# collabora/WhisperLive

Measured on AMD Instinct MI355X. Metric: real-time factor (xRT), Whisper-small 30 s window (p50 chunk latency in p50_chunk_latency_ms), higher is better.
Workload: dtype f16 (MFMA operands; f32 accumulate, f32 residual stream, f32 log-mel); 1 GPU; configs[1]: Whisper-small.en, 1 stream per GPU, one 30 s window per stream per step (480000 samples 16 kHz f32 resident in HBM -> log-mel -> encoder -> beam-5 decode, 64 generated tokens forced by suppressing EOT), seeded random weights; streams_per_gpu=1, beam_size=5, decode_steps=64

## Files before the change

### whisperlive_amd/csrc/decoder.h

```cpp
#pragma once
#include "kernels.h"

namespace wlx {

#define WLX_MAX_MT 4
#define WLX_MAX_DEC_ROWS 320
#define WLX_XSPLIT 8
#define WLX_MAX_CAND 32
#define WLX_MAX_HYP 32

struct RowTables {
    const int* token; const int* pos; const int* cache; const int* ancrow;
    const short* anc;
    int* intok;
};

void launch_dec_embed(const half_t* tok_emb, const float* pos_emb, int d, const RowTables& rt, int rows,
                      float* x, const int* done, hipStream_t s);

enum GemvIn : int { GEMV_IN_LN = 0, GEMV_IN_F16 = 1, GEMV_IN_XATTN = 2 };
enum GemvOut : int { GEMV_OUT_F16 = 0, GEMV_OUT_GELU_F16 = 1, GEMV_OUT_F32 = 2, GEMV_OUT_RESID = 3, GEMV_OUT_QKV = 4,
                     GEMV_OUT_SLAB = 5 };
enum GemvXsrc : int { GEMV_X_PLAIN = 0, GEMV_X_SLABS = 1, GEMV_X_EMBED = 2 };
#ifndef WLX_CQ_GB_LDS
#define WLX_CQ_GB_LDS 1
#endif
#ifndef WLX_CQ_SWAP
#define WLX_CQ_SWAP 1
#endif
#ifndef WLX_STAGE_WAVE
#define WLX_STAGE_WAVE 1
#endif
#ifndef WLX_XCOMB_WAVE
#define WLX_XCOMB_WAVE 1
#endif
#ifndef WLX_FC2_KS
#define WLX_FC2_KS 2
#endif

struct GemvParams {
    int in_mode, out_mode;
    int M;
    int Mtot;
    int chunk;
    int busy_device;
    int rt_nz, rt_tiles, rt_magic;
    int K, KT, N;
    int KTW;
    int NCH;
    int nwm;
    int xstage;
    const half_t* Wp; const float* bias;
    const float* X; long ldx; const float* gamma; const float* beta;
    const half_t* Xh; long ldxh;
    const half_t* part_o; const float* part_ml; int H; int R;
    half_t* Yh; long ldyh;
    float* Y; long ldy;
    float* Xres; long ldxres;
    int d; float qscale; half_t* Kc; half_t* Vc; long cache_row_stride;
    const int* row_cache; const int* row_pos;
    const int* done;
    int xsrc;
    float* slab; long slab_stride;
    int KTS;
    const half_t* tok_emb; const float* pos_emb; const int* emb_token; int* intok;
    WLX_TR_FIELD
};
#ifdef WLX_TRACE
extern unsigned long long* g_trace_buf;
extern int g_trace_seq;
extern const char* g_trace_names[512];
static inline WlxTrace trace_next(const char* name) {
    WlxTrace t{g_trace_buf, g_trace_seq};
    if (g_trace_seq < 512) g_trace_names[g_trace_seq] = name;
    ++g_trace_seq;
    return t;
}
#define WLX_TR_ARG(name) , trace_next(name)
#else
#define WLX_TR_ARG(name)
#endif
void launch_dec_gemv(const GemvParams& p, hipStream_t s);
const char* dec_gemv_kernel_name(const GemvParams& p);
extern bool g_decode_v1;
bool dec_gemv_is_lean(const GemvParams& p);
int dec_gemv_slab_split(int M, int K, int N);

void launch_dec_self_attn(const half_t* q, long ldq, const half_t* Kc, const half_t* Vc, long cache_row_stride,
                          int d, int H, const RowTables& rt, int rows, half_t* out, long ldo,
                          const int* done, bool ident_ancestry, hipStream_t s);
void launch_dec_cross_attn(const half_t* q, long ldq, const half_t* Kp, const half_t* Vp, long item_stride, int H, int R,
                           int groups, int rows, const int* group_item, half_t* part_o, float* part_ml, hipStream_t s);

bool dec_cq_cross_attn_eligible(int d, int H, int R);
void launch_dec_cq_cross_attn(const float* X, long ldx, const float* gamma, const float* beta, const half_t* Wp, const float* bias,
                              float qscale, int d, const half_t* Kp, const half_t* Vp, long item_stride, int H, int R, int groups,
                              int rows, const int* group_item, half_t* part_o, float* part_ml, hipStream_t s);
void launch_dec_xattn_combine(const half_t* part_o, const float* part_ml, int M, int H, int R, half_t* out, long ldo, hipStream_t s);
void launch_dec_align_scores(const half_t* q, long ldq, const half_t* Kp_item, int h, int rows, float* out, hipStream_t s);

struct SearchState {
    int* step;
    int* done;
    int* done_host;
    int* n_finished;
    int* item_done;
    int* plen;
    float* cum;
    int* row_done;
    float* cand_score; int* cand_tok;
    int* samp_tok; float* samp_lp;
    int* hyp_tokens;
    int* hyp_len;
    float* hyp_score;
    int* n_hyp;
    int* n_hyp_host;
    float* no_speech;
    int* nsp_row;
    int* token; int* pos; short* anc; int* intok;
    float* scan_stats;
    float* scan_cv; int* scan_ci;
    int* rule;
};
#define SC_THREADS 256
#define SC_NPT 8
#define SC_CHUNK (SC_THREADS * SC_NPT)
#define SC_MAXCH 27
#define SC_NSTAT 8
struct SearchParams {
    int V; long ldl;
    int items, R, rows;
    int sampling;
    int beam, ncand, max_cand_hyp , num_hyp;
    int allow_early_exit;
    float length_penalty, rep_penalty, temperature;
    int no_repeat_ngram, topk;
    int suppress_blank, apply_ts_rules, max_initial_ts;
    int sot, eot, no_timestamps, ts_begin, no_speech, blank;
    int max_length;
    unsigned long long seed;
    const unsigned* suppress_mask;
};
void launch_search_rows(const float* logits, const SearchParams* sp_dev, int rows, const SearchState& st, hipStream_t s);
void launch_search_update(const SearchParams* sp_dev, int items, const SearchState& st, hipStream_t s);
void launch_search_scan3(const float* logits, long ldl, int V, const SearchParams* sp_dev, int rows, const SearchState& st,
                         hipStream_t s);
void launch_search_merge_update3(const float* logits, long ldl, int V, const SearchParams* sp_dev, int items, int R,
                                 const SearchState& st, hipStream_t s);
void launch_search_reset(const SearchState& st, int items, int rows, hipStream_t s);
void launch_token_prob_rows(const float* logits, long ldl, int vlim, int rows, const int* toks, float* out, hipStream_t s);
void launch_token_prob(const float* logits, long ldl, int V, int rows, int tok, float* out, hipStream_t s);
void launch_lang_probs(const float* logits, long ldl, int rows, const int* ids, int n, float* probs, hipStream_t s);

}
```

### whisperlive_amd/csrc/decoder.hip

```cpp
#include "decoder.h"
#include <algorithm>
#include <cstdlib>
#include <cstdio>
#include <atomic>

namespace wlx {

__global__ __launch_bounds__(256) void dec_embed_kernel(const half_t* __restrict__ tok_emb,
                                                        const float* __restrict__ pos_emb, int d,
                                                        const int* __restrict__ token,
                                                        const int* __restrict__ pos,
                                                        const int* __restrict__ cache, int* __restrict__ intok,
                                                        float* __restrict__ x, const int* __restrict__ done WLX_TR_PARAM) {
    if (done && *done) return;
    WLX_TR_BEGIN();
    const int r = blockIdx.x;
    const int tok = token[r], p = pos[r];
    if (threadIdx.x == 0) intok[(long)cache[r] * WLX_T_TEXT + p] = tok;
    const half_t* te = tok_emb + (long)tok * d;
    const float* pe = pos_emb + (long)p * d;
    for (int i = threadIdx.x * 4; i < d; i += 256 * 4) {
        f16x4 t = ld_f16x4(te + i);
        float4 pv = *reinterpret_cast<const float4*>(pe + i);
        *reinterpret_cast<float4*>(x + (long)r * d + i) =
            make_float4((float)t[0] + pv.x, (float)t[1] + pv.y, (float)t[2] + pv.z, (float)t[3] + pv.w);
    }
    WLX_TR_END(trc);
}

void launch_dec_embed(const half_t* tok_emb, const float* pos_emb, int d, const RowTables& rt, int rows,
                      float* x, const int* done, hipStream_t s) {
    hipLaunchKernelGGL(dec_embed_kernel, dim3(rows), dim3(256), 0, s, tok_emb, pos_emb, d, rt.token, rt.pos,
                       rt.cache, rt.intok, x, done WLX_TR_ARG("embed"));
}

#define GV_CH 6

template <int MT, int NTB, int IN>
__global__ __launch_bounds__(512) void dec_gemv_kernel(GemvParams p) {
    if (p.done && *p.done) return;
    extern __shared__ __attribute__((aligned(16))) float smem[];
    const int tid = threadIdx.x, wave = tid >> 6, lane = tid & 63, c = lane & 15, g = lane >> 4;
    const int nw = blockDim.x >> 6;
    const int KT = p.KT;
    const int KTW = (KT + nw - 1) / nw;
    const int kt0 = wave * KTW;
    const int kt1 = (kt0 + KTW < KT) ? kt0 + KTW : KT;
    const int NT_total = (p.N + 15) >> 4;

    const half_t* wbase[NTB];
#pragma unroll
    for (int i = 0; i < NTB; ++i) {
        int nt = blockIdx.x * NTB + i;
// ... 337 lines not shown
            int u = lane + 64 * q;
            if (u >= total) u = (q == 0) ? total - 1 : (lane + 64 * (q - 1) < total ? lane + 64 * (q - 1) : total - 1);
            m_[q] = u / kv8; k_[q] = u - m_[q] * kv8;
            v_[q] = ld_f16x8(X + (long)m_[q] * ldx + k_[q] * 8);
        }
        after_first_loads();
#pragma unroll
        for (int q = 0; q < P; ++q) *reinterpret_cast<f16x8*>(xs + m_[q] * ldxs + k_[q] * 8) = v_[q];
    }
#pragma unroll 1
    for (int u0 = lane + 64 * P; u0 < total; u0 += 128) {
        const int u1 = u0 + 64;
        const int m0 = u0 / kv8, k0 = u0 - m0 * kv8;
        const int uc = (u1 < total) ? u1 : u0;
        const int m1 = uc / kv8, k1 = uc - m1 * kv8;
        const f16x8 v0 = ld_f16x8(X + (long)m0 * ldx + k0 * 8);
        const f16x8 v1 = ld_f16x8(X + (long)m1 * ldx + k1 * 8);
        *reinterpret_cast<f16x8*>(xs + m0 * ldxs + k0 * 8) = v0;
        *reinterpret_cast<f16x8*>(xs + m1 * ldxs + k1 * 8) = v1;
    }
}


template <int CH, int LNV, int IN, int OUT, int NTB, int MT, int XS>
__global__ __launch_bounds__((IN == GEMV_IN_LN || OUT == GEMV_OUT_SLAB || MT > 1 || CH > 6 || (IN == GEMV_IN_XATTN && WLX_XCOMB_WAVE != 0)) ? 512 : 1024) void dec_gemv2_kernel(GemvParams p_in) {
    GemvParams p = p_in;
    int tile = blockIdx.x;
    if (p_in.Mtot > 0) {
        int zc = (int)blockIdx.z;
        if (p_in.rt_nz > 0) {
            const int lin = (int)blockIdx.x, t = lin >> 3;
            const int tq = (int)(((unsigned)t * (unsigned)p_in.rt_magic) >> 16);
            zc = t - tq * p_in.rt_nz;
            tile = tq * 8 + (lin & 7);
            if (tile >= p_in.rt_tiles) return;
        }
        const int CHK = p_in.chunk;
        const int r0 = zc * CHK;
        p.M = (p_in.Mtot - r0 < CHK) ? p_in.Mtot - r0 : CHK;
        if (p.emb_token) p.emb_token += r0;
        if (p.X) p.X += (long)r0 * p.ldx;
        if (p.Xh) p.Xh += (long)r0 * p.ldxh;
        if (p.Yh) p.Yh += (long)r0 * p.ldyh;
        if (p.Y) p.Y += (long)r0 * p.ldy;
        if (p.Xres) p.Xres += (long)r0 * p.ldxres;
        if (p.slab) p.slab += (long)r0 * ((IN == GEMV_IN_LN) ? p.ldx : p.ldxres);
        if (p.row_cache) p.row_cache += r0;
        if (p.row_pos) p.row_pos += r0;
    }
    static_assert(XS == GEMV_X_PLAIN || IN == GEMV_IN_LN || (IN == GEMV_IN_F16 && OUT == GEMV_OUT_RESID && NTB == 1),
                  "slab / embedding sources: LayerNorm prologue or residual epilogue only");
    static_assert(OUT != GEMV_OUT_SLAB || (IN == GEMV_IN_F16 && NTB == 1), "K-split form: fp16 rows in");
    extern __shared__ __attribute__((aligned(16))) float smem[];
    const int tid = threadIdx.x, lane = tid & 63, c = lane & 15, g = lane >> 4;
    const int wave = __builtin_amdgcn_readfirstlane(tid >> 6);
    const int nw = p.nwm;
    WLX_TR_BEGIN();
    constexpr int NP = NTB * MT;
    constexpr bool LNT = (LNV == 15);
    constexpr int NV = LNT ? 2 : LNV;
    const bool tail_on = !LNT || lane < 32;
    const int tback = LNT ? (tail_on ? 0 : lane) : 0;
    (void)tail_on; (void)tback;
    float* accred = smem;
    half_t* xs = reinterpret_cast<half_t*>(smem + nw * NP * 256);

    const bool streams = (IN != GEMV_IN_XATTN) || wave < nw;
    const int kx0 = (streams ? wave : 0) * p.KTW;
    const int ks0 = (OUT == GEMV_OUT_SLAB) ? (int)blockIdx.y * p.KTS : 0;
    const int kw0 = ks0 + kx0;
    const half_t* wp = p.Wp + ((long)(tile * NTB) * p.KT + kw0) * 512 + lane * 8;
    const long wstep = (long)p.KT * 512;
    f16x8 wf[CH][NTB];
    auto load_weights = [&]() {
        asm volatile("" ::: "memory");
        const half_t* wq = streams ? wp : p.Wp + ((long)(tile * NTB) * p.KT + ks0) * 512 + lane * 8;
        const long js = streams ? 512 : 0, is = streams ? wstep : 0;
#pragma unroll
        for (int j = 0; j < CH; ++j)
#pragma unroll
            for (int i = 0; i < NTB; ++i) wf[j][i] = ld_nt_f16x8(wq + i * is + j * js);
    };
#ifndef WLX_X_FIRST
#define WLX_X_FIRST 1
#endif
    if (!WLX_X_FIRST) load_weights();

    int crow[MT];
#pragma unroll
    for (int mt = 0; mt < MT; ++mt) crow[mt] = (mt * 16 + c < p.M) ? mt * 16 + c : p.M - 1;
    const int pair0 = (wave < NP) ? wave : 0;
    const int nt_e = tile * NTB + pair0 / MT;
    const int n_e = nt_e * 16 + g * 4;
    int row_e = (pair0 % MT) * 16 + c;
    if (row_e >= p.M) row_e = p.M - 1;
    float4 bias_e = make_float4(0.f, 0.f, 0.f, 0.f), res_e = bias_e;
    int rc_e = 0, rp_e = 0;
    if constexpr (OUT != GEMV_OUT_F32) bias_e = *reinterpret_cast<const float4*>(p.bias + n_e);
    if constexpr (OUT == GEMV_OUT_RESID) res_e = *reinterpret_cast<const float4*>(p.Xres + (long)row_e * p.ldxres + n_e);
    if constexpr (OUT == GEMV_OUT_QKV) { rc_e = p.row_cache[row_e]; rp_e = p.row_pos[row_e]; }
    float4 slab_e[(OUT == GEMV_OUT_RESID && XS == GEMV_X_SLABS) ? WLX_FC2_KS : 1];
    if constexpr (OUT == GEMV_OUT_RESID && XS == GEMV_X_SLABS) {
#pragma unroll
        for (int sl = 0; sl < WLX_FC2_KS; ++sl)
            slab_e[sl] = *reinterpret_cast<const float4*>(p.slab + sl * p.slab_stride + (long)row_e * p.ldxres + n_e);
    }
    if constexpr (OUT == GEMV_OUT_SLAB) { if (blockIdx.y != 0) bias_e = make_float4(0.f, 0.f, 0.f, 0.f); }

    f32x4 acc[NTB][MT];
#pragma unroll
    for (int i = 0; i < NTB; ++i)
#pragma unroll
        for (int mt = 0; mt < MT; ++mt) acc[i][mt] = (f32x4){0.f, 0.f, 0.f, 0.f};
    f16x8 xf[CH][MT];

    if constexpr (IN == GEMV_IN_F16) {
        const half_t* xr[MT];
        int xstep;
        if (MT == 1 && p.xstage) {
            const int Ks = (OUT == GEMV_OUT_SLAB) ? p.KTS * 32 : p.K;
            const int ldxs = Ks + 8;
            if constexpr (WLX_STAGE_WAVE != 0) {
                stage_rows_f16_wave<(CH * 4 * 5 + 63) / 64>(p.Xh + (ks0 + kx0) * 32, p.ldxh, p.M, p.KTW * 32, xs + kx0 * 32, ldxs, lane, [&]() { if (WLX_X_FIRST) load_weights(); });
                WLX_TR_MARK(1);
                __builtin_amdgcn_fence(__ATOMIC_RELEASE, "wavefront");
                __builtin_amdgcn_wave_barrier();
                __builtin_amdgcn_fence(__ATOMIC_ACQUIRE, "wavefront");
            } else {
            stage_rows_f16(p.Xh + ks0 * 32, p.ldxh, p.M, Ks, xs, ldxs, [&]() { if (WLX_X_FIRST) load_weights(); });
            WLX_TR_MARK(1);
            __syncthreads();
            }
            xr[0] = xs + crow[0] * ldxs + kx0 * 32 + g * 8;
            xstep = 32;
        } else {
#pragma unroll
            for (int mt = 0; mt < MT; ++mt) xr[mt] = p.Xh + (long)crow[mt] * p.ldxh + kw0 * 32 + g * 8;
            xstep = 32;
        }
#pragma unroll
        for (int j = 0; j < CH; ++j)
#pragma unroll
            for (int mt = 0; mt < MT; ++mt) xf[j][mt] = *reinterpret_cast<const f16x8*>(xr[mt] + j * xstep);
        if (WLX_X_FIRST && !(MT == 1 && p.xstage)) load_weights();
#pragma unroll 1
        for (int ch = 1; ch < p.NCH; ++ch) {
            f16x8 wn[CH][NTB], xn[CH][MT];
#pragma unroll
            for (int j = 0; j < CH; ++j) {
#pragma unroll
                for (int i = 0; i < NTB; ++i) wn[j][i] = ld_nt_f16x8(wp + i * wstep + (ch * CH + j) * 512);
#pragma unroll
                for (int mt = 0; mt < MT; ++mt) xn[j][mt] = *reinterpret_cast<const f16x8*>(xr[mt] + (ch * CH + j) * xstep);
            }
#pragma unroll
            for (int j = 0; j < CH; ++j) {
#pragma unroll
                for (int i = 0; i < NTB; ++i) {
#pragma unroll
                    for (int mt = 0; mt < MT; ++mt) acc[i][mt] = mfma16(wf[j][i], xf[j][mt], acc[i][mt]);
                    wf[j][i] = wn[j][i];
                }
#pragma unroll
                for (int mt = 0; mt < MT; ++mt) xf[j][mt] = xn[j][mt];
            }
        }
    } else if constexpr (IN == GEMV_IN_LN && XS != GEMV_X_PLAIN) {
        const int nwl = nw;
        constexpr int NSL = (XS == GEMV_X_SLABS) ? WLX_FC2_KS : 1;
        float4 x[NV], sl[NSL][NV];
        f16x4 te[NV];
        int tok0 = 0, pos0 = 0;
        auto request_row = [&](int r, float4 (&x)[NV], float4 (&sl)[NSL][NV], f16x4 (&te)[NV], int& tok, int& pos) {
            if constexpr (XS == GEMV_X_EMBED) {
                tok = p.emb_token[r];
                pos = p.row_pos[r] | (p.row_cache[r] << 16);
                const half_t* tp = p.tok_emb + (long)tok * p.K + lane * 4;
                const float4* pp = reinterpret_cast<const float4*>(p.pos_emb + (long)(pos & 0xffff) * p.K) + lane;
#pragma unroll
                for (int j = 0; j < NV; ++j) { const int tb = (j == NV - 1) ? tback : 0; te[j] = ld_f16x4(tp + 256 * j - 4 * tb); x[j] = pp[64 * j - tb]; }
            } else {
                const float4* x4 = reinterpret_cast<const float4*>(p.X + (long)r * p.ldx) + lane;
#pragma unroll
                for (int j = 0; j < NV; ++j) x[j] = x4[64 * j - ((j == NV - 1) ? tback : 0)];
                if constexpr (XS == GEMV_X_SLABS) {
#pragma unroll
                    for (int q = 0; q < NSL; ++q) {
                        const float4* s4 = reinterpret_cast<const float4*>(p.slab + q * p.slab_stride + (long)r * p.ldx) + lane;
#pragma unroll
                        for (int j = 0; j < NV; ++j) sl[q][j] = s4[64 * j - ((j == NV - 1) ? tback : 0)];
                    }
                }
            }
        };
        auto combine_row = [&](int r, bool keep, float4 (&x)[NV], const float4 (&sl)[NSL][NV], const f16x4 (&te)[NV], int tok, int pos) {
            if constexpr (XS == GEMV_X_SLABS) {
#pragma unroll
                for (int q = 0; q < NSL; ++q)
#pragma unroll
                    for (int j = 0; j < NV; ++j) { x[j].x += sl[q][j].x; x[j].y += sl[q][j].y; x[j].z += sl[q][j].z; x[j].w += sl[q][j].w; }
            }
            if constexpr (XS == GEMV_X_EMBED) {
#pragma unroll
                for (int j = 0; j < NV; ++j) { x[j].x += (float)te[j][0]; x[j].y += (float)te[j][1]; x[j].z += (float)te[j][2]; x[j].w += (float)te[j][3]; }
                if (tile == 0 && keep) {
                    float4* o4 = reinterpret_cast<float4*>(p.Xres + (long)r * p.ldxres) + lane;
#pragma unroll
                    for (int j = 0; j < NV; ++j) if (j < NV - 1 || tail_on) o4[64 * j] = x[j];
                    if (lane == 0) p.intok[(long)(pos >> 16) * WLX_T_TEXT + (pos & 0xffff)] = tok;
                }
            }
        };
        const int ra = (wave < p.M) ? wave : p.M - 1;
        request_row(ra, x, sl, te, tok0, pos0);
        constexpr bool PF2 = MT == 1 && ((CH == 6 && LNV == 3) || (CH == 8 && LNV == 4) || (CH == 10 && LNV == 5));
        float4 xb[NV], slb[NSL][NV];
        f16x4 teb[NV];
        int tokb = 0, posb = 0;
        const int rb = (wave + nwl < p.M) ? wave + nwl : p.M - 1;
        if constexpr (PF2) request_row(rb, xb, slb, teb, tokb, posb);
        const float4* g4 = reinterpret_cast<const float4*>(p.gamma) + lane;
        const float4* b4 = reinterpret_cast<const float4*>(p.beta) + lane;
        float4 gq[NV], bq[NV];
#pragma unroll
        for (int j = 0; j < NV; ++j) { const int tb = (j == NV - 1) ? tback : 0; gq[j] = g4[64 * j - tb]; bq[j] = b4[64 * j - tb]; }
        if (WLX_X_FIRST) load_weights();
        const int ldxs = p.K + 8;
        constexpr float invK = LNT ? (1.0f / 384.0f) : 1.0f / (256.0f * NV);
        auto ln_row = [&](float4 (&x)[NV], int r, bool keep) {
            if constexpr (LNT) { if (!tail_on) x[NV - 1] = make_float4(0.f, 0.f, 0.f, 0.f); }
            float sm = 0.f;
#pragma unroll
            for (int j = 0; j < NV; ++j) sm += (x[j].x + x[j].y) + (x[j].z + x[j].w);
            const float mean = wave_sum_dpp(sm) * invK;
            float q = 0.f;
#pragma unroll
            for (int j = 0; j < NV; ++j) {
                x[j].x -= mean; x[j].y -= mean; x[j].z -= mean; x[j].w -= mean;
                if constexpr (LNT) { if (j == NV - 1 && !tail_on) x[j] = make_float4(0.f, 0.f, 0.f, 0.f); }
                q += (x[j].x * x[j].x + x[j].y * x[j].y) + (x[j].z * x[j].z + x[j].w * x[j].w);
            }
            const float rstd = rsqrtf(wave_sum_dpp(q) * invK + 1e-5f);
            half_t* dst = xs + (long)r * ldxs + lane * 4;
#pragma unroll
            for (int j = 0; j < NV; ++j) {
                const f16x4 hv = {(half_t)(x[j].x * rstd * gq[j].x + bq[j].x), (half_t)(x[j].y * rstd * gq[j].y + bq[j].y),
                                  (half_t)(x[j].z * rstd * gq[j].z + bq[j].z), (half_t)(x[j].w * rstd * gq[j].w + bq[j].w)};
                if (keep && (j < NV - 1 || tail_on)) *reinterpret_cast<f16x4*>(dst + 256 * j) = hv;
            }
        };
        combine_row(ra, wave < p.M, x, sl, te, tok0, pos0);
        ln_row(x, ra, wave < p.M);
        if constexpr (PF2) {
            combine_row(rb, wave + nwl < p.M, xb, slb, teb, tokb, posb);
            ln_row(xb, rb, wave + nwl < p.M);
        }
        if constexpr (MT == 1) {
#pragma unroll 1
            for (int r = wave + (PF2 ? 2 : 1) * nwl; r < p.M; r += nwl) {
                float4 x2[NV], sl2[NSL][NV];
                f16x4 te2[NV];
                int tok2 = 0, pos2 = 0;
                request_row(r, x2, sl2, te2, tok2, pos2);
                combine_row(r, true, x2, sl2, te2, tok2, pos2);
                ln_row(x2, r, true);
            }
        } else {
#pragma unroll 1
            for (int r = wave + nwl; r < p.M; r += 2 * nwl) {
                const int r1 = r + nwl;
                const bool has1 = r1 < p.M;
                float4 x2[NV], sl2[NSL][NV], x3[NV], sl3[NSL][NV];
                f16x4 te2[NV], te3[NV];
                int tok2 = 0, pos2 = 0, tok3 = 0, pos3 = 0;
                request_row(r, x2, sl2, te2, tok2, pos2);
                request_row(has1 ? r1 : r, x3, sl3, te3, tok3, pos3);
                combine_row(r, true, x2, sl2, te2, tok2, pos2);
                ln_row(x2, r, true);
                combine_row(has1 ? r1 : r, has1, x3, sl3, te3, tok3, pos3);
// ... 379 lines not shown
    const size_t xs_bytes = (size_t)p.M * (KTf * 32 + 8) * sizeof(half_t);
    if (c.NTB == 2 && p.out_mode == GEMV_OUT_GELU_F16 && c.shm + xs_bytes > WLX_G2_LDS_MAX) {
        c.NTB = 1;
        c.shm = sizeof(float) * (size_t)c.nw * c.NTB * c.MT * 256;
    }
    c.xstage = true;
    const size_t xstage_max = (p.Mtot > 0 && p.rt_nz > 0) ? (size_t)WLX_G2_LDS_MAX : (size_t)64 * 1024;
    if (p.in_mode == GEMV_IN_F16 && (c.MT > 1 || c.shm + xs_bytes > xstage_max)) c.xstage = false;
    if (c.xstage) c.shm += xs_bytes;
    if (c.shm > WLX_G2_LDS_MAX) return false;
    if (c.shm > 64 * 1024 && g_lds_optin_refused.load(std::memory_order_relaxed)) return false;
    return true;
}
static Gemv2Cfg gemv2_cfg(const GemvParams& p) {
    Gemv2Cfg c{};
    if (g_decode_v1 || p.M > 48 || p.M < 1) return c;
    if (p.bias ? (p.N & 15) != 0 : p.out_mode != GEMV_OUT_F32) return c;
    const bool combo = (p.in_mode == GEMV_IN_LN && (p.out_mode == GEMV_OUT_QKV || p.out_mode == GEMV_OUT_F16 ||
                                                    p.out_mode == GEMV_OUT_GELU_F16 || p.out_mode == GEMV_OUT_F32)) ||
                       (p.in_mode != GEMV_IN_LN && p.out_mode == GEMV_OUT_RESID) ||
                       (p.in_mode == GEMV_IN_F16 && p.out_mode == GEMV_OUT_SLAB);
    if (!combo || p.K != p.KT * 32) return c;
    if (p.xsrc != GEMV_X_PLAIN) {
        const bool ln_ok = p.in_mode == GEMV_IN_LN && p.out_mode == GEMV_OUT_QKV;
        const bool res_ok = p.in_mode == GEMV_IN_F16 && p.out_mode == GEMV_OUT_RESID && p.xsrc == GEMV_X_SLABS;
        if (!(ln_ok || res_ok)) return c;
    }
    int KTf = p.KT;
    if (p.out_mode == GEMV_OUT_SLAB) {
        if (p.KTS < 1 || p.KT % p.KTS || p.KT / p.KTS != WLX_FC2_KS) return c;
        KTf = p.KTS;
    }
    if (!gemv2_cfg_waves(p, KTf, c)) return c;
    c.NTB = gemv2_cfg_tiles(p);
    c.ok = gemv2_cfg_staging(p, KTf, c);
    return c;
}

template <int CH_, int LNV_, int IN_, int OUT_, int NTB_, int MT_, int XS_>
struct G2Args { static constexpr int CH = CH_, LNV = LNV_, IN = IN_, OUT = OUT_, NTB = NTB_, MT = MT_, XS = XS_; };
enum G2Rows { G2_LN_XS, G2_LN_PLAIN, G2_NO_LN };
template <int CH, int LNV, int OUT, int MT, int NTBMAX, class Leaf>
static bool gemv2_dispatch_ntb(const Gemv2Cfg& c, Leaf& leaf) {
    if (c.NTB == 1) return leaf(G2Args<CH, LNV, GEMV_IN_LN, OUT, 1, MT, GEMV_X_PLAIN>{});
    if constexpr (NTBMAX >= 2) { if (c.NTB == 2) return leaf(G2Args<CH, LNV, GEMV_IN_LN, OUT, 2, MT, GEMV_X_PLAIN>{}); }
    if constexpr (NTBMAX >= 4 && MT == 1) { if (c.NTB == 4) return leaf(G2Args<CH, LNV, GEMV_IN_LN, OUT, 4, 1, GEMV_X_PLAIN>{}); }
    return false;
}
template <int ROWS, int CH, int LNV, int MT, class Leaf>
static bool gemv2_dispatch_modes(const GemvParams& p, const Gemv2Cfg& c, Leaf& leaf) {
    if constexpr (ROWS == G2_LN_XS) {
        if (p.out_mode != GEMV_OUT_QKV || c.NTB != 1) return false;
        if (p.xsrc == GEMV_X_SLABS) return leaf(G2Args<CH, LNV, GEMV_IN_LN, GEMV_OUT_QKV, 1, MT, GEMV_X_SLABS>{});
        return p.xsrc == GEMV_X_EMBED && leaf(G2Args<CH, LNV, GEMV_IN_LN, GEMV_OUT_QKV, 1, MT, GEMV_X_EMBED>{});
    } else if constexpr (ROWS == G2_LN_PLAIN) {
        switch (p.out_mode) {
            case GEMV_OUT_QKV: return gemv2_dispatch_ntb<CH, LNV, GEMV_OUT_QKV, MT, 4>(c, leaf);
            case GEMV_OUT_F16: return gemv2_dispatch_ntb<CH, LNV, GEMV_OUT_F16, MT, 1>(c, leaf);
            case GEMV_OUT_GELU_F16: return gemv2_dispatch_ntb<CH, LNV, GEMV_OUT_GELU_F16, MT, 4>(c, leaf);
            case GEMV_OUT_F32: return gemv2_dispatch_ntb<CH, LNV, GEMV_OUT_F32, MT, 2>(c, leaf);
            default: return false;
        }
    } else {
        if (p.in_mode == GEMV_IN_XATTN) {
            if constexpr (CH <= 6) { if (p.out_mode == GEMV_OUT_RESID && p.xsrc == GEMV_X_PLAIN && c.NTB == 1) return leaf(G2Args<CH, 1, GEMV_IN_XATTN, GEMV_OUT_RESID, 1, MT, GEMV_X_PLAIN>{}); }
            return false;
        }
        if (p.in_mode != GEMV_IN_F16) return false;
        if (p.out_mode == GEMV_OUT_SLAB) return p.xsrc == GEMV_X_PLAIN && c.NTB == 1 && leaf(G2Args<CH, 1, GEMV_IN_F16, GEMV_OUT_SLAB, 1, MT, GEMV_X_PLAIN>{});
        if (p.out_mode != GEMV_OUT_RESID) return false;
        if (p.xsrc == GEMV_X_SLABS) return c.NTB == 1 && leaf(G2Args<CH, 1, GEMV_IN_F16, GEMV_OUT_RESID, 1, MT, GEMV_X_SLABS>{});
        if (p.xsrc != GEMV_X_PLAIN) return false;
        if (c.NTB == 1) return leaf(G2Args<CH, 1, GEMV_IN_F16, GEMV_OUT_RESID, 1, MT, GEMV_X_PLAIN>{});
        if constexpr (MT == 1) { if (c.NTB == 2) return leaf(G2Args<CH, 1, GEMV_IN_F16, GEMV_OUT_RESID, 2, 1, GEMV_X_PLAIN>{}); }
        return false;
    }
}
template <int ROWS, int CH, int LNV, int MTMAX, class Leaf>
static bool gemv2_dispatch_pair(const GemvParams& p, const Gemv2Cfg& c, Leaf& leaf) {
    if (c.CH != CH || c.LNV != LNV) return false;
    if (c.MT == 1) return gemv2_dispatch_modes<ROWS, CH, LNV, 1>(p, c, leaf);
    if constexpr (MTMAX == 3) return c.MT == 2 ? gemv2_dispatch_modes<ROWS, CH, LNV, 2>(p, c, leaf) : c.MT == 3 && gemv2_dispatch_modes<ROWS, CH, LNV, 3>(p, c, leaf);
    return false;
}
template <class Leaf>
static bool gemv2_dispatch(const GemvParams& p, const Gemv2Cfg& c, Leaf leaf) {
    if (p.in_mode == GEMV_IN_LN && p.xsrc != GEMV_X_PLAIN)
        return gemv2_dispatch_pair<G2_LN_XS, 4, 3, 3>(p, c, leaf) || gemv2_dispatch_pair<G2_LN_XS, 3, 3, 3>(p, c, leaf) || gemv2_dispatch_pair<G2_LN_XS, 2, 2, 3>(p, c, leaf) ||
               gemv2_dispatch_pair<G2_LN_XS, 4, 4, 3>(p, c, leaf) || gemv2_dispatch_pair<G2_LN_XS, 5, 5, 3>(p, c, leaf) || gemv2_dispatch_pair<G2_LN_XS, 2, 15, 1>(p, c, leaf) ||
               gemv2_dispatch_pair<G2_LN_XS, 6, 3, 1>(p, c, leaf) || gemv2_dispatch_pair<G2_LN_XS, 8, 4, 1>(p, c, leaf) || gemv2_dispatch_pair<G2_LN_XS, 10, 5, 1>(p, c, leaf);
    if (p.in_mode == GEMV_IN_LN)
        return gemv2_dispatch_pair<G2_LN_PLAIN, 6, 3, 3>(p, c, leaf) || gemv2_dispatch_pair<G2_LN_PLAIN, 5, 5, 3>(p, c, leaf) || gemv2_dispatch_pair<G2_LN_PLAIN, 4, 2, 3>(p, c, leaf) ||
               gemv2_dispatch_pair<G2_LN_PLAIN, 4, 4, 3>(p, c, leaf) || gemv2_dispatch_pair<G2_LN_PLAIN, 10, 5, 1>(p, c, leaf) || gemv2_dispatch_pair<G2_LN_PLAIN, 8, 4, 1>(p, c, leaf) ||
               gemv2_dispatch_pair<G2_LN_PLAIN, 2, 15, 1>(p, c, leaf);
    return gemv2_dispatch_pair<G2_NO_LN, 12, 1, 1>(p, c, leaf) || gemv2_dispatch_pair<G2_NO_LN, 10, 1, 1>(p, c, leaf) || gemv2_dispatch_pair<G2_NO_LN, 8, 1, 1>(p, c, leaf) ||
           gemv2_dispatch_pair<G2_NO_LN, 6, 1, 3>(p, c, leaf) || gemv2_dispatch_pair<G2_NO_LN, 5, 1, 3>(p, c, leaf) || gemv2_dispatch_pair<G2_NO_LN, 4, 1, 3>(p, c, leaf);
}
template __global__ void dec_gemv2_kernel<12, 1, GEMV_IN_XATTN, GEMV_OUT_RESID, 1, 1, GEMV_X_PLAIN>(GemvParams);
template __global__ void dec_gemv2_kernel<10, 1, GEMV_IN_XATTN, GEMV_OUT_RESID, 1, 1, GEMV_X_PLAIN>(GemvParams);
template __global__ void dec_gemv2_kernel<8, 1, GEMV_IN_XATTN, GEMV_OUT_RESID, 1, 1, GEMV_X_PLAIN>(GemvParams);

static bool gemv2_ok(const GemvParams& p, Gemv2Cfg* out) {
    const Gemv2Cfg c = gemv2_cfg(p);
    if (!c.ok || !gemv2_dispatch(p, c, [](auto) { return true; })) return false;
    if (out) *out = c;
    return true;
}
static void gemv2_launch(const GemvParams& p0, const Gemv2Cfg& c, hipStream_t s) {
    GemvParams p = p0;
    p.KTW = c.CH * c.NCH; p.NCH = c.NCH; p.xstage = c.xstage ? 1 : 0; p.nwm = c.nw;
#ifdef WLX_TRACE
    { static thread_local char nm[512][48]; const int q = g_trace_seq < 512 ? g_trace_seq : 511;
      snprintf(nm[q], 48, "gemv2<%d,%d,%d> N%d K%d", p.in_mode, p.out_mode, p.xsrc, p.N, p.K); p.trc = trace_next(nm[q]); }
#endif
    const int NT_total = (p.N + 15) / 16;
    if (p.Mtot > 0 && p.chunk <= 0) p.chunk = 48;
    dim3 grid((NT_total + c.NTB - 1) / c.NTB, p.out_mode == GEMV_OUT_SLAB ? p.KT / p.KTS : 1, p.Mtot > 0 ? (p.Mtot + p.chunk - 1) / p.chunk : 1), block(c.nw * 64);
    if (p.Mtot > 0 && p.rt_nz > 0) {
        p.rt_tiles = (int)grid.x;
        p.rt_magic = 65536 / p.rt_nz + 1;
        grid.x = ((grid.x + 7) / 8) * 8 * p.rt_nz;
        grid.z = 1;
    }
    if (p.in_mode == GEMV_IN_XATTN && !(WLX_XCOMB_WAVE != 0 && c.MT == 1)) {
        const int want = (p.M * p.H * 8 + 63) / 64;
        block.x = 64 * std::max(c.nw, std::min(c.MT > 1 ? 8 : 16, want));
    }
    const bool launched = gemv2_dispatch(p, c, [&](auto a) { using A = decltype(a); g2_launch<A::CH, A::LNV, A::IN, A::OUT, A::NTB, A::MT, A::XS>(grid, block, c.shm, s, p); return true; });
    if (!launched) dispatch_bug("dec_gemv2_kernel", s);
}
static GemvParams gemv_chunked(const GemvParams& p) {
    static const bool rt_on = [] { const char* e = wlx_ab("WLX_ROWTILE"); return !(e && e[0] == '0'); }();
    constexpr int rt_max = WLX_MAX_DEC_ROWS;
    static const int rt_chunk_env = [] { const char* e = wlx_ab("WLX_ROWTILE_CHUNK"); const int v = e ? atoi(e) : 0; return (v == 16 || v == 32 || v == 48) ? v : 0; }();
    int rt_chunk = 16;
    if (p.in_mode == GEMV_IN_F16 && p.out_mode == GEMV_OUT_RESID && p.xsrc == GEMV_X_PLAIN && !p.busy_device && p.M > 64) {
        static const int n_cu = [] { int dev = 0, n = 256; (void)hipGetDevice(&dev); hipDeviceProp_t pr; if (hipGetDeviceProperties(&pr, dev) == hipSuccess && pr.multiProcessorCount > 0) n = pr.multiProcessorCount; return n; }();
        const int tiles = (p.N + 15) / 16;
        double best = 1e300;
        for (int mt = 1; mt <= 3; ++mt) {
            const long wgs = (long)tiles * ((p.M + 16 * mt - 1) / (16 * mt));
            const double cost = (double)((wgs + n_cu - 1) / n_cu) * (1.0 + 0.35 * (mt - 1));
            if (cost < best - 1e-9) { best = cost; rt_chunk = 16 * mt; }
        }
    }
    if (rt_chunk_env) rt_chunk = rt_chunk_env;
    GemvParams q = p;
    if (p.Mtot != 0 || p.in_mode == GEMV_IN_XATTN) return q;
    const bool ln_wide4 = rt_chunk == 16 && p.M > 32 && p.in_mode == GEMV_IN_LN && p.xsrc == GEMV_X_PLAIN && (p.out_mode == GEMV_OUT_QKV || p.out_mode == GEMV_OUT_GELU_F16) &&
                          (p.N & 15) == 0 && ((p.N >> 4) & 3) == 0;
    const bool rt_shape = p.N <= 1536 || (long)p.N * p.K <= 3200000L || ln_wide4;
    if (rt_on && !g_decode_v1 && p.M > rt_chunk && p.M <= rt_max && rt_shape) { q.Mtot = p.M; q.M = rt_chunk; q.chunk = rt_chunk; q.rt_nz = (p.M + rt_chunk - 1) / rt_chunk; }
    else if (p.M > 48 && p.xsrc != GEMV_X_EMBED) { q.Mtot = p.M; q.M = 48; q.chunk = 48; }
    return q;
}

int dec_gemv_slab_split(int M, int K, int N) {
    if (WLX_FC2_KS < 2) return 0;
    if (g_decode_v1 || M < 1 || K % 32 || (K / 32) % WLX_FC2_KS || K < 2048) return 0;
    GemvParams p0{};
    p0.in_mode = GEMV_IN_F16; p0.out_mode = GEMV_OUT_SLAB; p0.M = M; p0.K = K; p0.KT = K / 32; p0.N = N; p0.KTS = p0.KT / WLX_FC2_KS;
    static const float dummy_bias = 0.f;
    p0.bias = &dummy_bias;
    const GemvParams p = gemv_chunked(p0);
    Gemv2Cfg c;
    if (!gemv2_ok(p, &c) || (p.M <= 16 && !c.xstage)) return 0;
    return WLX_FC2_KS;
}

struct VocabParams {
    const float* X; long ldx; const float* gamma; const float* beta;
    const half_t* Wp; int M, N, NT;
    float* Y; long ldy;
    const float* slab; long slab_stride;
    WLX_TR_FIELD
};
template <int KT, int KC, int MT, bool SLABS>
__global__ __launch_bounds__(512) void dec_vocab_kernel(VocabParams p) {
    static_assert(!SLABS || MT == 1, "slab rows: decode steps of one row tile");
    constexpr int K = KT * 32, LNV = (K + 255) / 256, NC = KT / KC, LDXS = K + 8;
    constexpr bool LNT = (K % 256) != 0;
    static_assert((K % 256 == 0 || K == 384) && KT % KC == 0 && NC % 2 == 0, "d_model a multiple of 256 (or 384); an even number of K chunks");
    constexpr int RPT = (MT == 1) ? 2 : 4;
    constexpr int NTRIP = (MT * 16 + 8 * RPT - 1) / (8 * RPT);
    extern __shared__ __attribute__((aligned(16))) half_t vxs[];
    const int tid = threadIdx.x, lane = tid & 63, c = lane & 15, g = lane >> 4;
    const int wave = __builtin_amdgcn_readfirstlane(tid >> 6);
    WLX_TR_BEGIN();
    const int pair = blockIdx.x * 8 + wave;
    const int t0 = (2 * pair < p.NT) ? 2 * pair : p.NT - 1, t1 = (2 * pair + 1 < p.NT) ? 2 * pair + 1 : p.NT - 1;
    const bool tail_on = !LNT || lane < 32;
    const int tback = LNT ? (tail_on ? 0 : lane) : 0;
    float4 x[RPT][LNV];
#pragma unroll
    for (int i = 0; i < RPT; ++i) {
        const int r = (wave + 8 * i < p.M) ? wave + 8 * i : p.M - 1;
        const float4* x4 = reinterpret_cast<const float4*>(p.X + (long)r * p.ldx) + lane;
#pragma unroll
        for (int j = 0; j < LNV; ++j) x[i][j] = x4[64 * j - ((j == LNV - 1) ? tback : 0)];
    }
    float4 xsl[SLABS ? WLX_FC2_KS : 1][RPT][LNV];
    if constexpr (SLABS) {
#pragma unroll
        for (int q = 0; q < WLX_FC2_KS; ++q)
#pragma unroll
            for (int i = 0; i < RPT; ++i) {
// ... 772 lines not shown
```

### whisperlive_amd/csrc/engine.h

```cpp
#pragma once
#include <hip/hip_runtime.h>
#include <map>
#include <mutex>
#include <string>
#include <vector>
#include "../../include/wlx.h"
#include "decoder.h"
#include "host.h"

namespace wlx {

struct StepGraphKey {
    int rows, R, groups;
    bool operator<(const StepGraphKey& o) const {
        if (rows != o.rows) return rows < o.rows;
        if (R != o.R) return R < o.R;
        return groups < o.groups;
    }
};

struct ProfRec { std::string name; double bytes; };
struct Prof { std::vector<ProfRec> recs; bool list_only = true; std::string only; int t = 0; };

struct Slot {
    std::mutex call_mu;
    int B = 0, R = 0, rows_cap = 0, cache_rows = 0, groups_cap = 0;
    hipStream_t stream = nullptr;
    bool dedicated_queue = false;
    int device_of = -1;
    bool counted = false;
    unsigned promote_epoch = 0;
    hipEvent_t ev0 = nullptr, ev1 = nullptr;
    hipEvent_t ev_lm0 = nullptr, ev_lm1 = nullptr;
    hipEvent_t ev_en0 = nullptr, ev_en1 = nullptr;
    bool en_pending = false;
    bool lm_pending = false;
    bool gen_pending = false;
    std::vector<int> lm_items;
    bool busy_variant = false;
    std::vector<void*> allocs, host_allocs;
    float* pcm = nullptr; size_t pcm_cap = 0;
    float* feats = nullptr; long feat_ld = 0;
    std::vector<int> nframes;
    std::vector<int64_t> npcm;
    unsigned* gmax = nullptr;
    ResampleStage rs{};
    bool rs_ready = false;
    long long* d_rng = nullptr;
    half_t *featT = nullptr, *h1 = nullptr, *ln = nullptr, *q = nullptr, *k = nullptr, *vt = nullptr,
           *attn = nullptr, *h2 = nullptr, *enc16 = nullptr;
    float *x = nullptr, *enc32 = nullptr;
    long featT_stride = 0, h1_stride = 0;
    half_t *ck = nullptr, *cvt = nullptr;
    int enc_batch = 0;
    half_t *kc = nullptr, *vc = nullptr;
    float* xd = nullptr; half_t *qd = nullptr, *attnd = nullptr, *hd = nullptr;
    float* slab = nullptr;
    half_t* part_o = nullptr;
    float *part_ml = nullptr, *logits = nullptr;
    long ldl = 0;
    int *d_token = nullptr, *d_pos = nullptr, *d_cache = nullptr, *d_ancrow = nullptr, *d_group_item = nullptr;
    struct DecBufs {
        float* xd; half_t *qd, *attnd, *hd; float* slab; int slab_rows; half_t* part_o; float* part_ml;
        int *d_token, *d_pos, *d_cache, *d_ancrow, *d_group_item;
    };
    DecBufs pf{};
    bool pf_one_pass = false;
    bool pf_ok = false;
    short* d_anc = nullptr; int* d_intok = nullptr;
    bool anc_ident = false;
    SearchState st{};
    SearchParams* d_sp = nullptr;
    unsigned* d_suppress = nullptr;
    int* d_lang_ids = nullptr; float* d_probs = nullptr; float* d_tokprob = nullptr;
    int* h_stage = nullptr; size_t h_stage_ints = 0;
    unsigned char* h_gen = nullptr; size_t h_gen_bytes = 0;
    int* h_pf = nullptr; bool h_pf_used = false;
    int* h_hyp = nullptr;
    int max_items = 0;
    std::vector<int> last_suppress; bool suppress_valid = false;
    std::map<StepGraphKey, hipGraphExec_t> graphs;
    wlx_timings tm{};
    Prof* prof = nullptr;
    struct AlignCapture { float* scores; const int32_t* heads; int n_heads, n_tok, row0, item; }* align = nullptr;
    float* align_scores = nullptr; size_t align_cap = 0;
    int* d_align_tgt = nullptr; float* d_align_prob = nullptr;
};

struct Ring {
    std::mutex mu;
    int device = 0;
    float* buf = nullptr; size_t cap = 0;
    int64_t base = 0, resident = 0;
    hipStream_t stream = nullptr;
    hipEvent_t last_read = nullptr; bool read_pending = false; hipStream_t last_read_stream = nullptr;
};

struct Engine {
    wlx_spec spec{};
    int device = 0;
    int H = 0;
    std::vector<void*> allocs;
    LogmelConsts lm{};
    half_t *conv1_w = nullptr, *conv2_w = nullptr;
    float *conv1_b = nullptr, *conv2_b = nullptr, *enc_pos = nullptr, *enc_ln_g = nullptr, *enc_ln_b = nullptr;
    int conv1_KT = 0;
    std::vector<LayerW> enc;
    half_t* Wckv = nullptr; float* bckv = nullptr;
    half_t *tok_emb16 = nullptr, *Wvocab = nullptr;
    float *dec_pos = nullptr, *dec_ln_g = nullptr, *dec_ln_b = nullptr;
    std::vector<LayerW> dec;
    std::mutex mu;
    std::vector<Slot*> slots;
    bool use_graph = true;
};

}

struct wlx_engine : public wlx::Engine {};
struct wlx_ring : public wlx::Ring {};
```

### whisperlive_amd/csrc/engine.hip

```cpp
#include "engine.h"
#include <sched.h>
#include <atomic>
#include <limits>
#include <algorithm>
#include <cmath>
#include <cstdio>
#include <cstdlib>
#include <cstring>
#include <chrono>
#include <thread>

using namespace wlx;

static inline void cpu_relax() {
#if defined(__x86_64__) || defined(__i386__)
    __builtin_ia32_pause();
#elif defined(__aarch64__)
    asm volatile("yield" ::: "memory");
#else
    asm volatile("" ::: "memory");
#endif
}
extern "C" int32_t wlx_abi_version(void) { return WLX_ABI_VERSION; }

// ... 74 lines not shown
    CKR(conv("model.encoder.conv2.weight", d, &e->conv2_w, &KT));
    CKR(ws.alloc_vec(A, "model.encoder.conv1.bias", d, &e->conv1_b, true));
    CKR(ws.alloc_vec(A, "model.encoder.conv2.bias", d, &e->conv2_b, true));
    CKR(positions("model.encoder.embed_positions.weight", sp.n_audio_ctx, &e->enc_pos));
    LayerOpts o{false, 1.f, true};
    e->enc.resize(sp.enc_layers);
    for (int l = 0; l < sp.enc_layers; ++l)
        CKR(load_layer(ws, A, "model.encoder.layers." + std::to_string(l) + ".", d, F, o, e->enc[l]));
    CKR(ws.alloc_vec(A, "model.encoder.layer_norm.weight", d, &e->enc_ln_g, true));
    CKR(ws.alloc_vec(A, "model.encoder.layer_norm.bias", d, &e->enc_ln_b, true));
    CKR(ws.need("model.decoder.embed_tokens.weight", {V, d}, &t));
    CKR(dalloc(A, &e->tok_emb16, (size_t)V * d, true));
    CKR(ws.device_f32(t, &src));
    launch_f32_to_f16(src, e->tok_emb16, (long)V * d, ws.st);
    CKR(alloc_packed(A, V, d, &e->Wvocab, &KT, true));
    launch_pack_linear(src, V, d, d, e->Wvocab, KT, 0, ws.st);
    CKR(positions("model.decoder.embed_positions.weight", sp.n_text_ctx, &e->dec_pos));
    CKR(alloc_packed(A, (int64_t)sp.dec_layers * 2 * d, d, &e->Wckv, nullptr, true));
    CKR(dalloc(A, &e->bckv, (size_t)sp.dec_layers * 2 * d, true));
    o.Wckv = e->Wckv; o.bckv = e->bckv;
    e->dec.resize(sp.dec_layers);
    for (o.l = 0; o.l < sp.dec_layers; ++o.l)
        CKR(load_layer(ws, A, "model.decoder.layers." + std::to_string(o.l) + ".", d, F, o, e->dec[o.l]));
    CKR(ws.alloc_vec(A, "model.decoder.layer_norm.weight", d, &e->dec_ln_g, true));
    CKR(ws.alloc_vec(A, "model.decoder.layer_norm.bias", d, &e->dec_ln_b, true));
    return ws.finish();
}

static std::atomic<bool> g_embedded_device_memory{false};
extern "C" int32_t wlx_engine_create(const wlx_spec* spec, const wlx_tensor* weights, int32_t n_weights,
                                     int32_t device, wlx_engine** out) {
    if (!spec || !weights || !out) return set_error(WLX_ERR_ARG, "null argument");
    if (spec->d_model % 64 || spec->d_model / 64 != spec->n_heads)
        return set_error(WLX_ERR_ARG, "d_model must be 64*n_heads");
    if (spec->d_model % 128 || spec->d_model > 1536) return set_error(WLX_ERR_ARG, "d_model must be a multiple of 128, <= 1536");
    if (spec->ffn % 128) return set_error(WLX_ERR_ARG, "ffn must be a multiple of 128");
    if (spec->n_mels != 80 && spec->n_mels != 128) return set_error(WLX_ERR_ARG, "n_mels must be 80 or 128");
    if (spec->n_audio_ctx != WLX_T_AUDIO || spec->n_text_ctx != WLX_T_TEXT)
        return set_error(WLX_ERR_ARG, "n_audio_ctx/n_text_ctx must be 1500/448");
    if (spec->vocab > 1024 * 52) return set_error(WLX_ERR_ARG, "vocab too large");
    int ndev = 0;
    CK(hipGetDeviceCount(&ndev));
    if (device < 0 || device >= ndev) return set_error(WLX_ERR_ARG, "device %d out of range (%d)", device, ndev);
    CK(hipSetDevice(device));
    if (int pe = gemm_prepare_device()) return set_error(WLX_ERR_HIP, "GEMM kernel set-up failed on device %d (hip error %d)", device, pe);
    wlx_engine* e = new wlx_engine();
    e->spec = *spec;
    e->device = device;
    e->H = spec->n_heads;
    for (int i = 0; i < n_weights; ++i)
        if (weights[i].on_device) { g_embedded_device_memory.store(true); break; }
    const char* ng = getenv("WLX_NO_GRAPH");
    e->use_graph = !(ng && ng[0] == '1');
    const char* v1 = wlx_ab("WLX_DECODE_V1");
    g_decode_v1 = (v1 && v1[0] == '1');
    int rc = engine_load(e, weights, n_weights);
    if (rc != WLX_OK) {
        for (void* p : e->allocs) (void)hipFree(p);
        delete e;
        return rc;
    }
    *out = e;
    return WLX_OK;
}

static int max_dedicated_queues() {
    static const int v = [] { const char* e = getenv("WLX_DEDICATED_QUEUES"); return e ? atoi(e) : 4; }();
    return v;
}
static std::atomic<int> g_dedicated_live[64];
static std::atomic<int> g_slots_live[64];
static std::atomic<bool> g_demote[64];
static std::atomic<unsigned> g_promote_epoch[64];
static void slot_free(Slot* s) {
    if (!s) return;
    if (s->device_of >= 0 && s->device_of < 64) {
        if (s->dedicated_queue) g_dedicated_live[s->device_of].fetch_sub(1);
        if (s->counted && g_slots_live[s->device_of].fetch_sub(1) - 1 <= max_dedicated_queues()) {
            if (g_demote[s->device_of].exchange(false)) g_promote_epoch[s->device_of].fetch_add(1);
        }
    }
    if (s->align_scores) (void)hipFree(s->align_scores);
    for (auto& kv : s->graphs) (void)hipGraphExecDestroy(kv.second);
    for (void* p : s->allocs) (void)hipFree(p);
    for (void* p : s->host_allocs) (void)hipHostFree(p);
    if (s->ev0) (void)hipEventDestroy(s->ev0);
    if (s->ev1) (void)hipEventDestroy(s->ev1);
    if (s->ev_lm0) (void)hipEventDestroy(s->ev_lm0);
    if (s->ev_lm1) (void)hipEventDestroy(s->ev_lm1);
    if (s->ev_en0) (void)hipEventDestroy(s->ev_en0);
    if (s->ev_en1) (void)hipEventDestroy(s->ev_en1);
    for (hipEvent_t ev : s->rs.copied) if (ev) (void)hipEventDestroy(ev);
    if (s->stream) (void)hipStreamDestroy(s->stream);
    delete s;
}

extern "C" void wlx_engine_destroy(wlx_engine* e) {
    if (!e) return;
    (void)hipSetDevice(e->device);
    (void)hipDeviceSynchronize();
    for (Slot* s : e->slots) slot_free(s);
    for (void* p : e->allocs) (void)hipFree(p);
    delete e;
}

extern "C" int32_t wlx_engine_spec(const wlx_engine* e, wlx_spec* out) {
// ... 201 lines not shown
            b.slab_rows = (int)PR;
            CKR(dalloc(s->allocs, &b.xd, PR * d, true)); CKR(dalloc(s->allocs, &b.qd, PR * d, true)); CKR(dalloc(s->allocs, &b.attnd, PR * d, true));
            CKR(dalloc(s->allocs, &b.hd, PR * F, true)); CKR(dalloc(s->allocs, &b.slab, (size_t)WLX_FC2_KS * PR * d, true));
            CKR(dalloc(s->allocs, &b.part_o, PG * e->H * WLX_XSPLIT * 16 * 64, true));
            CKR(dalloc(s->allocs, &b.part_ml, PG * e->H * WLX_XSPLIT * 16 * 2, true));
            CKR(dalloc(s->allocs, &b.d_token, PR, true)); CKR(dalloc(s->allocs, &b.d_pos, PR, true)); CKR(dalloc(s->allocs, &b.d_cache, PR, true));
            CKR(dalloc(s->allocs, &b.d_ancrow, PR, true)); CKR(dalloc(s->allocs, &b.d_group_item, PG, true));
            GemvParams q{};
            static const float dummy_bias = 0.f;
            q.M = 96; q.bias = &dummy_bias; q.xsrc = GEMV_X_PLAIN;
            auto lean = [&](int in, int out, int N, int K) { q.in_mode = in; q.out_mode = out; q.N = N; q.K = K; q.KT = K / 32; return dec_gemv_is_lean(q); };
            s->pf_ok = lean(GEMV_IN_LN, GEMV_OUT_QKV, 3 * d, d) && lean(GEMV_IN_F16, GEMV_OUT_RESID, d, d) && lean(GEMV_IN_LN, GEMV_OUT_F16, d, d) &&
                       lean(GEMV_IN_LN, GEMV_OUT_GELU_F16, F, d) && lean(GEMV_IN_F16, GEMV_OUT_RESID, d, F);
        }
        s->ldl = ((sp.vocab + 15) / 16) * 16;
        CKR(dalloc(s->allocs, &s->logits, (size_t)RC * s->ldl, true));
        CKR(dalloc(s->allocs, &s->d_token, (size_t)RC, true));
        CKR(dalloc(s->allocs, &s->d_pos, (size_t)RC, true));
        CKR(dalloc(s->allocs, &s->d_cache, (size_t)RC, true));
        CKR(dalloc(s->allocs, &s->d_ancrow, (size_t)RC, true));
        CKR(dalloc(s->allocs, &s->d_group_item, (size_t)RC, true));
        const int CR = std::max(s->cache_rows, RC);
        CKR(dalloc(s->allocs, &s->d_anc, (size_t)CR * WLX_T_TEXT, true));
        CKR(dalloc(s->allocs, &s->d_intok, (size_t)CR * WLX_T_TEXT, true));
        SearchState& st = s->st;
        CKR(dalloc(s->allocs, &st.step, 1, true)); CKR(dalloc(s->allocs, &st.done, 1, true)); CKR(dalloc(s->allocs, &st.n_finished, 1, true));
        CKR(dalloc(s->allocs, &st.item_done, (size_t)B, true)); CKR(dalloc(s->allocs, &st.plen, (size_t)B, true));
        CKR(dalloc(s->allocs, &st.cum, (size_t)RC, true)); CKR(dalloc(s->allocs, &st.row_done, (size_t)RC, true));
        CKR(dalloc(s->allocs, &st.cand_score, (size_t)RC * WLX_MAX_CAND, true));
        CKR(dalloc(s->allocs, &st.cand_tok, (size_t)RC * WLX_MAX_CAND, true));
        CKR(dalloc(s->allocs, &st.samp_tok, (size_t)RC, true)); CKR(dalloc(s->allocs, &st.samp_lp, (size_t)RC, true));
        {
            const size_t ints = (size_t)B * (2 + 2 * WLX_MAX_HYP + (size_t)WLX_MAX_HYP * WLX_T_TEXT);
            CKR(halloc(s->host_allocs, &s->h_hyp, ints));
            memset(s->h_hyp, 0, ints * sizeof(int));
            s->max_items = B;
            CKR(halloc(s->host_allocs, &s->h_pf, (size_t)(5 * WLX_T_TEXT + 64)));
            st.n_hyp_host = s->h_hyp;
            st.hyp_len = st.n_hyp_host + B;
            st.hyp_score = reinterpret_cast<float*>(st.hyp_len + (size_t)B * WLX_MAX_HYP);
            st.no_speech = st.hyp_score + (size_t)B * WLX_MAX_HYP;
            st.hyp_tokens = reinterpret_cast<int*>(st.no_speech + B);
        }
        CKR(dalloc(s->allocs, &st.n_hyp, (size_t)B, true));
        CKR(dalloc(s->allocs, &st.nsp_row, (size_t)RC, true));
        st.token = s->d_token; st.pos = s->d_pos; st.anc = s->d_anc; st.intok = s->d_intok;
        CKR(dalloc(s->allocs, &st.scan_stats, (size_t)RC * SC_MAXCH * SC_NSTAT, true));
        CKR(dalloc(s->allocs, &st.scan_cv, (size_t)RC * (SC_MAXCH + 1) * WLX_MAX_CAND, true));
        CKR(dalloc(s->allocs, &st.scan_ci, (size_t)RC * (SC_MAXCH + 1) * WLX_MAX_CAND, true));
        CKR(dalloc(s->allocs, &st.rule, (size_t)RC * 4, true));
        CKR(dalloc(s->allocs, &s->d_align_tgt, (size_t)WLX_T_TEXT, true));
        CKR(dalloc(s->allocs, &s->d_align_prob, (size_t)WLX_T_TEXT, true));
        CKR(dalloc(s->allocs, &s->d_sp, 1, true));
        CKR(dalloc(s->allocs, &s->d_suppress, (size_t)(1024 * 52 / 32), true));
        CKR(dalloc(s->allocs, &s->d_lang_ids, 256, true));
        CKR(dalloc(s->allocs, &s->d_probs, (size_t)B * 256, true));
        CKR(dalloc(s->allocs, &s->d_tokprob, (size_t)RC, true));
        s->h_stage_ints = 1 << 16;
        CKR(halloc(s->host_allocs, &s->h_stage, s->h_stage_ints));
        s->st.done_host = s->h_stage + (s->h_stage_ints - 4);
        s->h_gen_bytes = 4096 + (size_t)RC * (4 + 16 + 4) + (size_t)B * 4 + (size_t)RC * WLX_T_TEXT * 2 + 256 + ((size_t)RC * 4 + B) * 4 + 128 +
                         (size_t)B * (4 + WLX_MAX_HYP * 8 + 4) + 64 + (size_t)B * WLX_MAX_HYP * WLX_T_TEXT * 4;
        CKR(halloc(s->host_allocs, &s->h_gen, s->h_gen_bytes));
        CK(hipStreamSynchronize(s->stream));
        return WLX_OK;
    }();
    if (rc != WLX_OK) { slot_free(s); return rc; }
    std::lock_guard<std::mutex> g(e->mu);
    e->slots.push_back(s);
    const int id = (int)e->slots.size() - 1;
    *slot_out = id;
    return WLX_OK;
}

extern "C" int32_t wlx_slot_destroy(wlx_engine* e, int32_t slot) {
    if (!e) return set_error(WLX_ERR_ARG, "null engine");
    Slot* s = nullptr;
    for (;;) {
        {
            std::lock_guard<std::mutex> g(e->mu);
            if (slot < 0 || slot >= (int)e->slots.size() || !e->slots[slot]) return set_error(WLX_ERR_ARG, "bad slot %d", slot);
            if (e->slots[slot]->call_mu.try_lock()) {
                s = e->slots[slot];
                e->slots[slot] = nullptr;
                break;
            }
        }
        std::this_thread::sleep_for(std::chrono::milliseconds(1));
    }
    s->call_mu.unlock();
    (void)hipSetDevice(e->device);
    (void)hipStreamSynchronize(s->stream);
    slot_free(s);
    return WLX_OK;
}

static int flush_logmel(Engine* e, Slot* s) {
    if (s->lm_items.empty()) return WLX_OK;
    CK(hipSetDevice(e->device));
    CK(hipEventRecord(s->ev_lm0, s->stream));
    for (size_t i0 = 0; i0 < s->lm_items.size(); i0 += WLX_LM_MAXB) {
        LogmelBatch lb{};
        for (size_t i = i0; i < s->lm_items.size() && i < i0 + WLX_LM_MAXB; ++i) {
            const int item = s->lm_items[i], k = lb.n_items++;
            const int64_t n = s->npcm[item];
            lb.pcm[k] = s->pcm + (size_t)item * s->pcm_cap; lb.n[k] = (long)n;
// ... 341 lines not shown
        g.A = s->ln; g.lda = d; g.Wp = w.Wqkv; g.KT = d / 32; g.M = M; g.N = 3 * d; g.mode = GEMM_QKV; g.bias = w.bqkv;
        g.C = s->q; g.ldc = d; g.d = d; g.qscale = 0.125f; g.Kout = s->k; g.ldk = d; g.Vt = s->vt; g.ldvt = WLX_T_AUDIO_PAD;
        g.rows_per_item = T; g.kv_item_stride_k = (long)WLX_T_AUDIO_PAD * d; g.kv_item_stride_v = (long)d * WLX_T_AUDIO_PAD;
        launch_gemm(g, 1, st);
        launch_attn_encoder(s->q, d, s->k, d, s->vt, WLX_T_AUDIO_PAD, s->attn, d, T, H, batch, (long)T * d,
                            (long)WLX_T_AUDIO_PAD * d, (long)d * WLX_T_AUDIO_PAD, (long)T * d, st);
        g = GemmParams{};
        g.A = s->attn; g.lda = d; g.Wp = w.Wo; g.KT = d / 32; g.M = M; g.N = d; g.mode = GEMM_RESID_F32; g.bias = w.bo;
        g.X = s->x; g.ldx = d;
        launch_gemm(g, 1, st);
        launch_layernorm_f16(s->x, d, w.ln3_g, w.ln3_b, s->ln, d, M, d, st);
        g = GemmParams{};
        g.A = s->ln; g.lda = d; g.Wp = w.W1; g.KT = d / 32; g.M = M; g.N = F; g.mode = GEMM_GELU_F16; g.bias = w.b1;
        g.C = s->h2; g.ldc = F;
        launch_gemm(g, 1, st);
        g = GemmParams{};
        g.A = s->h2; g.lda = F; g.Wp = w.W2; g.KT = F / 32; g.M = M; g.N = d; g.mode = GEMM_RESID_F32; g.bias = w.b2;
        g.X = s->x; g.ldx = d;
        launch_gemm(g, 1, st);
    }
    launch_layernorm_f16_f32(s->x, d, e->enc_ln_g, e->enc_ln_b, s->enc16, s->enc32, d, M, d, st);
    g = GemmParams{};
    g.A = s->enc16; g.lda = d; g.Wp = e->Wckv; g.KT = d / 32; g.M = M; g.N = sp.dec_layers * 2 * d; g.mode = GEMM_CROSS_KV;
    g.bias = e->bckv; g.d = d; g.Kout = s->ck; g.ldk = d; g.Vt = s->cvt; g.ldvt = WLX_T_AUDIO_PAD; g.rows_per_item = T;
    g.kv_item_stride_k = (long)WLX_T_AUDIO_PAD * d; g.kv_item_stride_v = (long)d * WLX_T_AUDIO_PAD;
    g.kv_layer_stride_k = (long)s->B * WLX_T_AUDIO_PAD * d; g.kv_layer_stride_v = (long)s->B * d * WLX_T_AUDIO_PAD;
    launch_gemm(g, 1, st);
    CK(hipGetLastError());
    CK(hipEventRecord(s->ev_en1, st));
    s->en_pending = true;
    s->enc_batch = batch;
    return WLX_OK;
}

extern "C" int32_t wlx_encoder_output_get(wlx_engine* e, int32_t slot, int32_t item, float* out, int64_t cap_floats) {
    SlotGuard sg_;
    CKR(slot_acquire(e, slot, sg_));
    Slot* s = sg_.s;
    if (item < 0 || item >= s->enc_batch) return set_error(WLX_ERR_STATE, "item %d not encoded", item);
    const size_t n = (size_t)WLX_T_AUDIO * e->spec.d_model;
    if (!out || (int64_t)n > cap_floats) return set_error(WLX_ERR_ARG, "output buffer too small");
    CK(hipSetDevice(e->device));
    CK(hipMemcpyAsync(out, s->enc32 + (size_t)item * n, n * 4, hipMemcpyDeviceToHost, s->stream));
    CK(hipStreamSynchronize(s->stream));
    return WLX_OK;
}

template <class F>
static inline void plaunch(Slot* s, const char* name, double bytes, F&& f) {
    if (!s->prof) { f(); return; }
    if (s->prof->list_only) { s->prof->recs.push_back(ProfRec{name, bytes}); return; }
    if (s->prof->only == name) f();
}
static double gemv_bytes(const GemvParams& p) { return 2.0 * (double)p.N * (double)p.K + (p.bias ? 4.0 * p.N : 0.0); }
static bool device_is_busy(const Slot* s) {
    return s->device_of >= 0 && s->device_of < 64 && g_slots_live[s->device_of].load(std::memory_order_relaxed) >= 3;
}
static void pgemv(Slot* s, const GemvParams& p0) {
    GemvParams p = p0;
    p.busy_device = s->busy_variant ? 1 : 0;
    if (!s->prof) { launch_dec_gemv(p, s->stream); return; }
    const std::string nm = dec_gemv_kernel_name(p);
    plaunch(s, nm.c_str(), gemv_bytes(p), [&] { launch_dec_gemv(p, s->stream); });
}

static void decoder_pass(Engine* e, Slot* s_, int rows, int R, int groups, bool with_logits, bool check_done, const Slot::DecBufs* alt = nullptr) {
    const wlx_spec& sp = e->spec;
    const int d = sp.d_model, F = sp.ffn, H = e->H;
    struct View {
        Slot* base; float* xd; half_t *qd, *attnd, *hd; float* slab; long slab_rows; half_t* part_o; float* part_ml;
        int *d_token, *d_pos, *d_cache, *d_ancrow, *d_group_item;
        Slot* operator->() const { return base; }
    } s{s_, alt ? alt->xd : s_->xd, alt ? alt->qd : s_->qd, alt ? alt->attnd : s_->attnd, alt ? alt->hd : s_->hd,
        alt ? alt->slab : s_->slab, alt ? (long)alt->slab_rows : (long)s_->rows_cap, alt ? alt->part_o : s_->part_o, alt ? alt->part_ml : s_->part_ml,
        alt ? alt->d_token : s_->d_token, alt ? alt->d_pos : s_->d_pos, alt ? alt->d_cache : s_->d_cache,
        alt ? alt->d_ancrow : s_->d_ancrow, alt ? alt->d_group_item : s_->d_group_item};
    hipStream_t st = s->stream;
    const int* done = (check_done && g_decode_v1) ? s->st.done : nullptr;
    RowTables rt{s.d_token, s.d_pos, s.d_cache, s.d_ancrow, s->d_anc, s->d_intok};
    const long crs = (long)WLX_T_TEXT * d;
    auto qkv_params = [&](int l, int xsrc) {
        const LayerW& w = e->dec[l];
        GemvParams p{};
        p.in_mode = GEMV_IN_LN; p.out_mode = GEMV_OUT_QKV; p.M = rows; p.K = d; p.KT = d / 32; p.N = 3 * d;
        p.Wp = w.Wqkv; p.bias = w.bqkv; p.X = s.xd; p.ldx = d; p.gamma = w.ln1_g; p.beta = w.ln1_b;
        p.Yh = s.qd; p.ldyh = d; p.d = d; p.qscale = 0.125f;
        p.Kc = s->kc + (size_t)l * s->cache_rows * crs; p.Vc = s->vc + (size_t)l * s->cache_rows * crs; p.cache_row_stride = crs;
        p.row_cache = s.d_cache; p.row_pos = s.d_pos; p.done = done;
        p.xsrc = xsrc; p.slab = s.slab; p.slab_stride = s.slab_rows * d;
        if (xsrc == GEMV_X_EMBED) {
            p.tok_emb = e->tok_emb16; p.pos_emb = e->dec_pos; p.emb_token = s.d_token; p.intok = s->d_intok;
            p.Xres = s.xd; p.ldxres = d;
        }
        return p;
    };
    auto oproj_params = [&](int l, int xsrc) {
        const LayerW& w = e->dec[l];
        GemvParams p{};
        p.in_mode = GEMV_IN_F16; p.out_mode = GEMV_OUT_RESID; p.M = rows; p.K = d; p.KT = d / 32; p.N = d;
        p.Wp = w.Wo; p.bias = w.bo; p.Xh = s.attnd; p.ldxh = d; p.Xres = s.xd; p.ldxres = d; p.qscale = 1.f; p.done = done;
        p.xsrc = xsrc; p.slab = s.slab; p.slab_stride = s.slab_rows * d;
        return p;
    };
    auto vocab_params = [&](int xsrc) {
        GemvParams p{};
        p.in_mode = GEMV_IN_LN; p.out_mode = GEMV_OUT_F32; p.M = rows; p.K = d; p.KT = d / 32; p.N = sp.vocab;
        p.Wp = e->Wvocab; p.bias = nullptr; p.X = s.xd; p.ldx = d; p.gamma = e->dec_ln_g; p.beta = e->dec_ln_b;
        p.Y = s->logits; p.ldy = s->ldl; p.qscale = 1.f; p.done = done;
        p.xsrc = xsrc; p.slab = s.slab; p.slab_stride = s.slab_rows * d;
        return p;
    };
    int KS = dec_gemv_slab_split(rows, F, d);
    if (rows > s.slab_rows) KS = 0;
    if (rows > 16 && !alt) KS = 0;
    if (alt && s->pf_one_pass) KS = 0;
    if (KS && !(dec_gemv_is_lean(qkv_params(0, GEMV_X_SLABS)) && dec_gemv_is_lean(oproj_params(0, GEMV_X_SLABS)))) KS = 0;
    const bool fold_embed = (rows <= 16 || (alt != nullptr && rows <= 64)) && dec_gemv_is_lean(qkv_params(0, GEMV_X_EMBED));
    if (!fold_embed)
        plaunch(s.base, "dec_embed_kernel", (double)rows * d * (2 + 4), [&] { launch_dec_embed(e->tok_emb16, e->dec_pos, d, rt, rows, s.xd, done, st); });
    bool slabs_pending = false;
    for (int l = 0; l < sp.dec_layers; ++l) {
        const LayerW& w = e->dec[l];
        half_t* kc = s->kc + (size_t)l * s->cache_rows * crs;
        half_t* vc = s->vc + (size_t)l * s->cache_rows * crs;
        {
            GemvParams pq = qkv_params(l, (l == 0 && fold_embed) ? GEMV_X_EMBED : (slabs_pending ? GEMV_X_SLABS : GEMV_X_PLAIN));
            pgemv(s.base, pq);
        }
        plaunch(s.base, "dec_self_attn2_kernel", 4.0 * rows * d * (s->prof ? s->prof->t + 1 : 1), [&] { launch_dec_self_attn(s.qd, d, kc, vc, crs, d, H, rt, rows, s.attnd, d, done, s->anc_ident, st); });
        pgemv(s.base, oproj_params(l, slabs_pending ? GEMV_X_SLABS : GEMV_X_PLAIN));
        slabs_pending = false;
        GemvParams p{};
        const half_t* ckl = s->ck + (size_t)l * s->B * WLX_T_AUDIO_PAD * d;
        const half_t* cvl = s->cvt + (size_t)l * s->B * d * WLX_T_AUDIO_PAD;
        const bool fused = !s->align && rows <= 48 && dec_cq_cross_attn_eligible(d, H, R);
        if (fused)
            plaunch(s.base, "dec_cq_cross_attn_kernel", 2.0 * d * d + 4.0 * groups * WLX_T_AUDIO * d, [&] {
                launch_dec_cq_cross_attn(s.xd, d, w.ln2_g, w.ln2_b, w.Wcq, w.bcq, 0.125f, d, ckl, cvl, (long)WLX_T_AUDIO_PAD * d, H, R,
                                         groups, rows, s.d_group_item, s.part_o, s.part_ml, st);
            });
        if (!fused) {
            p = GemvParams{};
            p.in_mode = GEMV_IN_LN; p.out_mode = GEMV_OUT_F16; p.M = rows; p.K = d; p.KT = d / 32; p.N = d;
            p.Wp = w.Wcq; p.bias = w.bcq; p.X = s.xd; p.ldx = d; p.gamma = w.ln2_g; p.beta = w.ln2_b;
            p.Yh = s.qd; p.ldyh = d; p.qscale = 0.125f; p.done = done;
            pgemv(s.base, p);
            if (s->align) {
                const Slot::AlignCapture& a = *s->align;
                for (int hi = 0; hi < a.n_heads; ++hi)
                    if (a.heads[2 * hi] == l)
                        launch_dec_align_scores(s.qd, d, s->ck + ((size_t)l * s->B + a.item) * WLX_T_AUDIO_PAD * d, a.heads[2 * hi + 1], rows,
                                                a.scores + ((size_t)hi * a.n_tok + a.row0) * WLX_T_AUDIO_PAD, st);
            }
            plaunch(s.base, "dec_cross_attn_kernel", 4.0 * groups * WLX_T_AUDIO * d, [&] {
                launch_dec_cross_attn(s.qd, d, ckl, cvl, (long)WLX_T_AUDIO_PAD * d, H, R, groups, rows, s.d_group_item, s.part_o, s.part_ml, st);
            });
        }
        p = GemvParams{};
        p.in_mode = GEMV_IN_XATTN; p.out_mode = GEMV_OUT_RESID; p.M = rows; p.K = d; p.KT = d / 32; p.N = d;
        p.Wp = w.Wco; p.bias = w.bco; p.part_o = s.part_o; p.part_ml = s.part_ml; p.H = H; p.R = R;
        p.Xres = s.xd; p.ldxres = d; p.qscale = 1.f; p.done = done;
        if (rows > 16) {
            plaunch(s.base, "dec_xattn_combine_kernel", 0.0, [&] { launch_dec_xattn_combine(s.part_o, s.part_ml, rows, H, R, s.attnd, d, st); });
            p.in_mode = GEMV_IN_F16; p.Xh = s.attnd; p.ldxh = d;
        }
        pgemv(s.base, p);
        p = GemvParams{};
        p.in_mode = GEMV_IN_LN; p.out_mode = GEMV_OUT_GELU_F16; p.M = rows; p.K = d; p.KT = d / 32; p.N = F;
        p.Wp = w.W1; p.bias = w.b1; p.X = s.xd; p.ldx = d; p.gamma = w.ln3_g; p.beta = w.ln3_b;
        p.Yh = s.hd; p.ldyh = F; p.qscale = 1.f; p.done = done;
        pgemv(s.base, p);
        p = GemvParams{};
        p.in_mode = GEMV_IN_F16; p.out_mode = GEMV_OUT_RESID; p.M = rows; p.K = F; p.KT = F / 32; p.N = d;
        p.Wp = w.W2; p.bias = w.b2; p.Xh = s.hd; p.ldxh = F; p.Xres = s.xd; p.ldxres = d; p.qscale = 1.f; p.done = done;
        const bool last_split = with_logits && dec_gemv_is_lean(vocab_params(GEMV_X_SLABS));
        if (KS && (l + 1 < sp.dec_layers || last_split)) {
            p.out_mode = GEMV_OUT_SLAB; p.KTS = p.KT / KS; p.slab = s.slab; p.slab_stride = s.slab_rows * d;
            slabs_pending = true;
        }
// ... 37 lines not shown
        CK(hipMemcpyAsync(b.d_pos, h + rows, rows * 4, hipMemcpyHostToDevice, s->stream));
        CK(hipMemcpyAsync(b.d_cache, h + 2 * rows, rows * 4, hipMemcpyHostToDevice, s->stream));
        CK(hipMemcpyAsync(b.d_ancrow, h + 3 * rows, rows * 4, hipMemcpyHostToDevice, s->stream));
        CK(hipMemcpyAsync(b.d_group_item, h + 4 * rows, groups * 4, hipMemcpyHostToDevice, s->stream));
        s->anc_ident = false;
        s->pf_one_pass = true;
        decoder_pass(e, s, rows, 16, groups, false, false, &b);
        s->pf_one_pass = false;
        CK(hipGetLastError());
        if (nsp_index >= 0 && nsp_index < rows) {
            const int d = e->spec.d_model;
            GemvParams p{};
            p.in_mode = GEMV_IN_LN; p.out_mode = GEMV_OUT_F32; p.M = 1; p.K = d; p.KT = d / 32; p.N = e->spec.vocab;
            p.Wp = e->Wvocab; p.bias = nullptr; p.X = b.xd + (size_t)nsp_index * d; p.ldx = d; p.gamma = e->dec_ln_g; p.beta = e->dec_ln_b;
            p.Y = s->logits; p.ldy = s->ldl; p.qscale = 1.f; p.xsrc = GEMV_X_PLAIN;
            launch_dec_gemv(p, s->stream);
            launch_token_prob(s->logits, s->ldl, e->spec.vocab, 1, nsp_token, s->d_tokprob, s->stream);
            CK(hipMemcpyAsync(nsp_out, s->d_tokprob, 4, hipMemcpyDefault, s->stream));
            CK(hipGetLastError());
        }
        return WLX_OK;
    }
    const int chunk = std::min(s->rows_cap, [] { const char* v = getenv("WLX_PREFILL_ROWS"); const int c = v ? atoi(v) : 48; return (c >= 16 && c <= WLX_MAX_DEC_ROWS) ? c : 48; }());
    for (int c0 = 0; c0 < n; c0 += chunk) {
        const int rows = std::min(chunk, n - c0);
        const int groups = (rows + 15) / 16;
        std::vector<int> tk(rows), ps(rows), ca(rows, crow), an(rows, crow), gi(groups, item);
        for (int i = 0; i < rows; ++i) { tk[i] = tokens[c0 + i]; ps[i] = pos0 + c0 + i; }
        CKR(upload_rows(s, tk, ps, ca, an, gi));
        const bool want_nsp = nsp_index >= c0 && nsp_index < c0 + rows;
        const bool lg = (logits_host != nullptr) || want_nsp;
        decoder_pass(e, s, rows, 16, groups, lg, false);
        CK(hipGetLastError());
        if (logits_host) {
            CK(hipMemcpy2DAsync(logits_host + (size_t)c0 * e->spec.vocab, (size_t)e->spec.vocab * 4, s->logits,
                                (size_t)s->ldl * 4, (size_t)e->spec.vocab * 4, rows, hipMemcpyDeviceToHost, s->stream));
        }
        if (want_nsp) {
            launch_token_prob(s->logits + (size_t)(nsp_index - c0) * s->ldl, s->ldl, e->spec.vocab, 1, nsp_token,
                              s->d_tokprob, s->stream);
            CK(hipMemcpyAsync(nsp_out, s->d_tokprob, 4, hipMemcpyDeviceToDevice, s->stream));
        }
    }
    return WLX_OK;
}

static int set_anc_rows(Slot* s, const std::vector<short>& anc_host, int first_row, int nrows) {
    CK(hipMemcpyAsync(s->d_anc + (size_t)first_row * WLX_T_TEXT, anc_host.data(), (size_t)nrows * WLX_T_TEXT * sizeof(short),
                      hipMemcpyHostToDevice, s->stream));
    CK(hipStreamSynchronize(s->stream));
    return WLX_OK;
}

static void launch_search(Engine* e, Slot* s, int rows, int R, int groups, bool sampling) {
    if (sampling || g_decode_v1) {
        launch_search_rows(s->logits, s->d_sp, rows, s->st, s->stream);
        launch_search_update(s->d_sp, groups, s->st, s->stream);
    } else {
        launch_search_scan3(s->logits, s->ldl, e->spec.vocab, s->d_sp, rows, s->st, s->stream);
        launch_search_merge_update3(s->logits, s->ldl, e->spec.vocab, s->d_sp, groups, R, s->st, s->stream);
    }
}

static int graph_steps_for(const Slot* s, int rows) {
    static const int env = [] { const char* v = wlx_ab("WLX_GRAPH_STEPS"); const int n = v ? atoi(v) : 2; return (n == 1 || n == 2) ? n : 2; }();
    if (env == 1 || rows > 16) return 1;
    const bool alone = s->device_of >= 0 && s->device_of < 64 && g_slots_live[s->device_of].load(std::memory_order_relaxed) <= 1;
    return alone ? 2 : 1;
}

static int get_step_graph(Engine* e, Slot* s, int rows, int R, int groups, bool sampling, int nsteps, hipGraphExec_t* out) {
    s->busy_variant = device_is_busy(s);
    StepGraphKey key{rows, R, groups * 8 + (nsteps == 2 ? 4 : 0) + (s->busy_variant ? 2 : 0) + (sampling ? 1 : 0)};
    auto it = s->graphs.find(key);
    if (it != s->graphs.end()) { *out = it->second; return WLX_OK; }
    hipGraph_t graph;
    decoder_pass(e, s, rows, R, groups, true, true);
    CK(hipGetLastError());
    CK(hipStreamBeginCapture(s->stream, hipStreamCaptureModeThreadLocal));
    for (int k = 0; k < nsteps; ++k) {
        decoder_pass(e, s, rows, R, groups, true, true);
        launch_search(e, s, rows, R, groups, sampling);
    }
    const hipError_t ce = hipStreamEndCapture(s->stream, &graph);
    if (ce != hipSuccess) {
        (void)hipGetLastError();
        hipStream_t ns = nullptr;
        bool ded = false;
        if (s->dedicated_queue) { g_dedicated_live[e->device].fetch_sub(1); s->dedicated_queue = false; }
        if (create_slot_stream(e->device, &ns, &ded) == WLX_OK) {
            s->dedicated_queue = ded;
            (void)hipStreamDestroy(s->stream);
            s->stream = ns;
        }
        return set_error(WLX_ERR_HIP, "decode-step graph capture failed: %s (slot stream replaced)", hipGetErrorString(ce));
    }
    hipGraphExec_t exec;
    CK(hipGraphInstantiate(&exec, graph, nullptr, nullptr, 0));
    CK(hipGraphDestroy(graph));
    s->graphs[key] = exec;
    *out = exec;
    return WLX_OK;
}

static int run_step(Engine* e, Slot* s, int rows, int R, int groups, bool sampling, int nsteps = 1) {
    if (e->use_graph) {
        hipGraphExec_t exec;
        CKR(get_step_graph(e, s, rows, R, groups, sampling, nsteps, &exec));
        CK(hipGraphLaunch(exec, s->stream));
    } else {
        s->busy_variant = device_is_busy(s);
        for (int k = 0; k < nsteps; ++k) {
            decoder_pass(e, s, rows, R, groups, true, true);
            launch_search(e, s, rows, R, groups, sampling);
        }
        CK(hipGetLastError());
    }
    return WLX_OK;
}

static int fill_search_params(Engine* e, Slot* s, int batch, int R, const wlx_gen_opts* o, bool apply_ts, SearchParams* sp) {
    memset(sp, 0, sizeof(*sp));
    sp->V = e->spec.vocab; sp->ldl = s->ldl; sp->items = batch; sp->R = R; sp->rows = batch * R;
    sp->sampling = (o->sampling_temperature > 0.f || o->beam_size <= 1) ? 1 : 0;
    sp->beam = sp->sampling ? 1 : o->beam_size;
    sp->ncand = sp->sampling ? 1 : 2 * o->beam_size;
    sp->max_cand_hyp = std::max(1, (int)std::lround((double)o->beam_size * (double)o->patience));
    sp->num_hyp = std::max(1, o->num_hypotheses);
    sp->allow_early_exit = (o->length_penalty == 0.f) ? 1 : 0;
    sp->length_penalty = o->length_penalty; sp->rep_penalty = (o->repetition_penalty > 0.f) ? o->repetition_penalty : 1.f;
    sp->temperature = o->sampling_temperature; sp->no_repeat_ngram = o->no_repeat_ngram_size;
    sp->topk = (o->sampling_temperature > 0.f) ? o->sampling_topk : 1;
    sp->suppress_blank = o->suppress_blank; sp->apply_ts_rules = apply_ts ? 1 : 0;
    sp->max_initial_ts = o->max_initial_timestamp_index;
    sp->sot = o->ids.sot; sp->eot = o->ids.eot; sp->no_timestamps = o->ids.no_timestamps; sp->ts_begin = o->ids.timestamp_begin;
    sp->no_speech = o->ids.no_speech; sp->blank = o->ids.blank;
    sp->max_length = o->max_length; sp->seed = o->seed; sp->suppress_mask = s->d_suppress;
    return WLX_OK;
}

static int validate_opts(Engine* e, Slot* s, int batch, const wlx_gen_opts* o) {
    if (!o) return set_error(WLX_ERR_ARG, "null opts");
    const int V = e->spec.vocab;
    auto bad = [&](int id) { return id < 0 || id >= V; };
    if (bad(o->ids.sot) || bad(o->ids.eot) || bad(o->ids.no_timestamps) || bad(o->ids.timestamp_begin) || bad(o->ids.no_speech))
        return set_error(WLX_ERR_ARG, "token ids out of vocabulary");
    if (o->max_length < 2 || o->max_length > WLX_T_TEXT) return set_error(WLX_ERR_ARG, "max_length must be 2..448");
    const bool sampling = (o->sampling_temperature > 0.f || o->beam_size <= 1);
    const int R = sampling ? std::max(1, o->num_hypotheses) : o->beam_size;
    if (R < 1 || R > s->R) return set_error(WLX_ERR_ARG, "beam_size/num_hypotheses %d exceeds slot rows per item %d", R, s->R);
    if (!sampling && o->num_hypotheses > o->beam_size) return set_error(WLX_ERR_ARG, "num_hypotheses > beam_size");
    if (!sampling && 2 * o->beam_size > WLX_MAX_CAND) return set_error(WLX_ERR_ARG, "beam_size too large");
    if (batch * R > s->rows_cap) return set_error(WLX_ERR_ARG, "too many decoder rows");
    if (o->n_suppress_tokens < 0 || (o->n_suppress_tokens > 0 && !o->suppress_tokens)) return set_error(WLX_ERR_ARG, "bad suppress_tokens");
    return WLX_OK;
}

static int upload_suppress(Engine* e, Slot* s, const wlx_gen_opts* o) {
    const int V = e->spec.vocab, words = (V + 31) / 32;
    if (s->suppress_valid && (int)s->last_suppress.size() == o->n_suppress_tokens &&
        (o->n_suppress_tokens == 0 || memcmp(s->last_suppress.data(), o->suppress_tokens, (size_t)o->n_suppress_tokens * 4) == 0))
        return WLX_OK;
    s->suppress_valid = false;
    std::vector<unsigned> mask(words, 0u);
    for (int i = 0; i < o->n_suppress_tokens; ++i) {
        const int id = o->suppress_tokens[i];
        if (id >= 0 && id < V) mask[id >> 5] |= 1u << (id & 31);
// ... 89 lines not shown
                for (int bi = 0; bi < nb; ++bi) {
                    const int b = b0 + bi;
                    const int32_t* pr = prompts + (size_t)b * pstride;
                    const int np_ = pl[b] - 1;
                    for (int i = 0; i < 16; ++i) {
                        const int j = np_ > 0 ? std::min(i, np_ - 1) : 0;
                        h[bi * 16 + i] = pr[j]; h[prow + bi * 16 + i] = j; h[2 * prow + bi * 16 + i] = b * R; h[3 * prow + bi * 16 + i] = b * R;
                    }
                    h[4 * prow + bi] = enc_items ? enc_items[b] : b;
                }
                CK(hipMemcpyAsync(pb.d_token, h, prow * 4, hipMemcpyHostToDevice, st));
                CK(hipMemcpyAsync(pb.d_pos, h + prow, prow * 4, hipMemcpyHostToDevice, st));
                CK(hipMemcpyAsync(pb.d_cache, h + 2 * prow, prow * 4, hipMemcpyHostToDevice, st));
                CK(hipMemcpyAsync(pb.d_ancrow, h + 3 * prow, prow * 4, hipMemcpyHostToDevice, st));
                CK(hipMemcpyAsync(pb.d_group_item, h + 4 * prow, nb * 4, hipMemcpyHostToDevice, st));
                s->anc_ident = false;
                decoder_pass(e, s, prow, 16, nb, false, false, &pb);
                CK(hipGetLastError());
                for (int bi = 0; bi < nb; ++bi) {
                    const int b = b0 + bi;
                    if (!(sot_at[b] >= 0 && sot_at[b] < pl[b] - 1)) continue;
                    GemvParams p{};
                    p.in_mode = GEMV_IN_LN; p.out_mode = GEMV_OUT_F32; p.M = 1; p.K = d; p.KT = d / 32; p.N = V;
                    p.Wp = e->Wvocab; p.bias = nullptr; p.X = pb.xd + (size_t)(bi * 16 + sot_at[b]) * d; p.ldx = d; p.gamma = e->dec_ln_g; p.beta = e->dec_ln_b;
                    p.Y = s->logits; p.ldy = s->ldl; p.qscale = 1.f; p.xsrc = GEMV_X_PLAIN;
                    launch_dec_gemv(p, st);
                    launch_token_prob(s->logits, s->ldl, V, 1, o->ids.no_speech, s->d_tokprob, st);
                    CK(hipMemcpyAsync(S.no_speech + b, s->d_tokprob, 4, hipMemcpyDefault, st));
                }
                CK(hipGetLastError());
            }
        } else {
            for (int b = 0; b < batch; ++b) {
                const int32_t* pr = prompts + (size_t)b * pstride;
                if (pl[b] > 1)
                    CKR(prefill_tokens(e, s, enc_items ? enc_items[b] : b, b * R, pr, 0, pl[b] - 1, nullptr, (sot_at[b] >= 0 && sot_at[b] < pl[b] - 1) ? sot_at[b] : -1,
                                       o->ids.no_speech, S.no_speech + b));
            }
        }
    }
    {
        std::vector<int> tk(rows), ps(rows), ca(rows), an(rows), gi(batch);
        for (int b = 0; b < batch; ++b) {
            gi[b] = enc_items ? enc_items[b] : b;
            for (int r = 0; r < R; ++r) {
                const int row = b * R + r;
                tk[row] = prompts[(size_t)b * pstride + pl[b] - 1]; ps[row] = pl[b] - 1; ca[row] = row; an[row] = row;
            }
        }
        CKR(upload_rows(s, tk, ps, ca, an, gi, h_rows));
        memcpy(h_nsp, nsp.data(), (size_t)rows * 4);
        CK(hipMemcpyAsync(S.nsp_row, h_nsp, rows * 4, hipMemcpyHostToDevice, st));
    }
    volatile int* h_done = s->h_stage + (s->h_stage_ints - 4);
    h_done[0] = 0;
    h_done[1] = 0;
    const double tg1 = now_us();
    int steps_run = 0;
    bool finished = false;
    const int gsteps = (injected_logits || !e->use_graph) ? 1 : graph_steps_for(s, rows);
    for (int step = 0; step < max_steps && !finished;) {
        int n_this = 1;
        if (injected_logits) {
            if (step >= inj_steps) break;
            RowTables rt{s->d_token, s->d_pos, s->d_cache, s->d_ancrow, s->d_anc, s->d_intok};
            launch_dec_embed(e->tok_emb16, e->dec_pos, e->spec.d_model, rt, rows, s->xd, nullptr, st);
            CK(hipMemcpy2DAsync(s->logits, (size_t)s->ldl * 4, inj + (size_t)step * rows * V, (size_t)V * 4, (size_t)V * 4, rows,
                                hipMemcpyHostToDevice, st));
            launch_search(e, s, rows, R, batch, sampling);
            CK(hipGetLastError());
        } else {
            const double ta = gen_trace ? now_us() : 0.0;
            n_this = std::min(gsteps, max_steps - step);
            CKR(run_step(e, s, rows, R, batch, sampling, n_this));
            if (gen_trace) tg_launch += now_us() - ta;
        }
        steps_run += n_this;
        step += n_this;
        if (injected_logits) {
            CK(hipStreamSynchronize(st));
            finished = h_done[0] != 0;
        } else if (step >= 2) {
            const double ta = gen_trace ? now_us() : 0.0;
            int spins = 0, rounds = 0;
            while (h_done[1] < step - 1 && h_done[0] == 0) {
                if (rounds == 0 && spins < 4096) cpu_relax(); else sched_yield();
                if (++spins >= (1 << 16)) {
                    spins = 0; ++rounds;
                    const hipError_t q = hipStreamQuery(st);
                    if (q == hipSuccess) break;
                    if (q != hipErrorNotReady) return set_error(WLX_ERR_HIP, "decode loop: %s", hipGetErrorString(q));
                }
            }
            if (gen_trace) tg_wait += now_us() - ta;
            finished = h_done[0] != 0;
        }
    }
    const double tg2 = now_us();
    if (gen_trace) CK(hipStreamSynchronize(st));
    const double tg3 = now_us();
    CK(hipEventRecord(s->ev1, st));
    s->gen_pending = true;
    if (h_done[0] == 0 || gen_trace) CK(hipStreamSynchronize(st));
    std::atomic_thread_fence(std::memory_order_acquire);
    const int MB = s->max_items;
    const int* n_hyp = S.n_hyp_host;
    const int* hyp_len = S.hyp_len;
    const float* hyp_score = S.hyp_score;
    const float* nspv = S.no_speech;
    const int* hyp_tok = S.hyp_tokens;
    (void)MB; (void)h_res;
    const int NH = std::max(1, o->num_hypotheses);
    for (int b = 0; b < batch; ++b) {
        std::vector<int> order(std::min(n_hyp[b], WLX_MAX_HYP));
        for (size_t i = 0; i < order.size(); ++i) order[i] = (int)i;
        std::stable_sort(order.begin(), order.end(), [&](int a, int c) {
            return hyp_score[(size_t)b * WLX_MAX_HYP + a] > hyp_score[(size_t)b * WLX_MAX_HYP + c];
        });
        for (int h = 0; h < NH; ++h) {
            int32_t* dst = tokens_out + ((size_t)b * NH + h) * tstride;
            if (h < (int)order.size()) {
                const int src = order[h];
                int len = hyp_len[(size_t)b * WLX_MAX_HYP + src];
                if (len > tstride) len = tstride;
                memcpy(dst, &hyp_tok[((size_t)b * WLX_MAX_HYP + src) * WLX_T_TEXT], (size_t)len * 4);
                n_tokens_out[b * NH + h] = len;
                scores_out[b * NH + h] = hyp_score[(size_t)b * WLX_MAX_HYP + src];
            } else {
                n_tokens_out[b * NH + h] = 0;
                scores_out[b * NH + h] = -INFINITY;
            }
        }
        if (nsp_out) nsp_out[b] = nspv[b];
    }
    if (gen_trace) {
        float gms = 0.f;
        CK(hipEventElapsedTime(&gms, s->ev0, s->ev1));
        fprintf(stderr, "[wlx gen] steps %d: setup %.0f us | loop %.0f us (graph launch calls %.0f, event waits %.0f) | drain %.0f us | readback %.0f us | device %.0f us\n",
                steps_run, tg1 - tg0, tg2 - tg1, tg_launch, tg_wait, tg3 - tg2, now_us() - tg3, 1e3 * gms);
    }
    return WLX_OK;
}

extern "C" int32_t wlx_generate_ex(wlx_engine* e, int32_t slot, int32_t batch, const int32_t* enc_items,
                                   const int32_t* prompts, const int32_t* prompt_lens, int32_t prompt_stride,
                                   const wlx_gen_opts* opts, int32_t* tokens_out, int32_t tokens_stride,
                                   int32_t* n_tokens_out, float* scores_out, float* no_speech_prob_out) {
    SlotGuard sg_;
    CKR(slot_acquire(e, slot, sg_));
// ... 406 lines not shown
```

### whisperlive_amd/csrc/search.hip

```cpp
#include "decoder.h"

namespace wlx {

#define SR_THREADS 1024
#define SR_NPT 52

__device__ __forceinline__ float block_max(float v, float* scratch) {
    v = wave_max(v);
    __syncthreads();
    if ((threadIdx.x & 63) == 0) scratch[threadIdx.x >> 6] = v;
    __syncthreads();
    float r = scratch[0];
#pragma unroll
    for (int w = 1; w < SR_THREADS / 64; ++w) r = fmaxf(r, scratch[w]);
    return r;
}
__device__ __forceinline__ float block_sum(float v, float* scratch) {
    v = wave_sum(v);
    __syncthreads();
    if ((threadIdx.x & 63) == 0) scratch[threadIdx.x >> 6] = v;
    __syncthreads();
    float r = 0.f;
#pragma unroll
    for (int w = 0; w < SR_THREADS / 64; ++w) r += scratch[w];
    return r;
}

__device__ __forceinline__ unsigned long long splitmix64(unsigned long long x) {
    x += 0x9E3779B97F4A7C15ull;
    x = (x ^ (x >> 30)) * 0xBF58476D1CE4E5B9ull;
    x = (x ^ (x >> 27)) * 0x94D049BB133111EBull;
    return x ^ (x >> 31);
}

__global__ __launch_bounds__(SR_THREADS) void search_rows_kernel(const float* __restrict__ logits,
                                                                 const SearchParams* __restrict__ spp, SearchState st) {
    if (*st.done) return;
    const SearchParams sp = *spp;
    const int r = blockIdx.x;
    const int item = r / sp.R;
    const int rb = r - item * sp.R;
    if (st.item_done[item]) return;
    if (sp.sampling) { if (rb >= sp.num_hyp || st.row_done[r]) return; }
    else if (rb >= sp.beam) return;

    __shared__ int hist[WLX_T_TEXT];
    __shared__ unsigned seen[(SR_THREADS * SR_NPT + 31) / 32];
    __shared__ float fs[16];
    __shared__ int is_[16];
    __shared__ int last_ts_idx;
    __shared__ float chunk_sum[SR_THREADS];

    const int tid = threadIdx.x;
// ... 194 lines not shown
            float gv = fs[0]; int gi = is_[0];
#pragma unroll
            for (int w = 1; w < SR_THREADS / 64; ++w)
                if (fs[w] > gv || (fs[w] == gv && is_[w] < gi)) { gv = fs[w]; gi = is_[w]; }
            chosen = gi;
            if (tid == 0) { st.samp_tok[r] = gi; st.samp_lp[r] = gv - lse_sel; }
        } else {
            float* wrow = const_cast<float*>(lrow);
#pragma unroll
            for (int i = 0; i < SR_NPT; ++i) {
                const int id = tid + i * SR_THREADS;
                if (id < V) wrow[id] = v[i];
            }
            __syncthreads();
            const float invT = 1.0f / sp.temperature;
            float cs = 0.f;
            for (int q = 0; q < SR_NPT; ++q) {
                const int id = tid * SR_NPT + q;
                if (id < V) cs += __expf((wrow[id] - mx_sel) * invT);
            }
            chunk_sum[tid] = cs;
            __syncthreads();
            if (tid == 0) {
                float total = 0.f;
                for (int t2 = 0; t2 < SR_THREADS; ++t2) total += chunk_sum[t2];
                const unsigned long long h = splitmix64(sp.seed ^ splitmix64(((unsigned long long)r << 32) | (unsigned)p));
                const float u = (float)(h >> 40) * (1.0f / 16777216.0f);
                const float target = u * total;
                float run = 0.f; int ch = 0;
                for (; ch < SR_THREADS - 1; ++ch) { if (run + chunk_sum[ch] > target) break; run += chunk_sum[ch]; }
                int pick = -1, lastvalid = -1;
                for (int q = 0; q < SR_NPT; ++q) {
                    const int id = ch * SR_NPT + q;
                    if (id >= V) break;
                    const float e = __expf((wrow[id] - mx_sel) * invT);
                    if (e > 0.f) lastvalid = id;
                    run += e;
                    if (run > target && e > 0.f) { pick = id; break; }
                }
                if (pick < 0) pick = (lastvalid >= 0) ? lastvalid : sp.eot;
                st.samp_tok[r] = pick;
                st.samp_lp[r] = wrow[pick] - lse_sel;
                is_[0] = pick;
            }
            __syncthreads();
            chosen = is_[0];
        }
        (void)chosen;
    }
}

void launch_search_rows(const float* logits, const SearchParams* sp_dev, int rows, const SearchState& st, hipStream_t s) {
    hipLaunchKernelGGL(search_rows_kernel, dim3(rows), dim3(SR_THREADS), 0, s, logits, sp_dev, st);
}

__device__ __forceinline__ void step_mirror(const SearchState& st, int step_no) {
    __hip_atomic_store(st.done_host + 1, step_no, __ATOMIC_RELEASE, __HIP_MEMORY_SCOPE_SYSTEM);
}
__device__ __forceinline__ void finish_item(const SearchState& st, int item, int items) {
    st.item_done[item] = 1;
    __threadfence_system();
    const int nf = atomicAdd(st.n_finished, 1) + 1;
    if (nf >= items) {
        __threadfence_system();
        *st.done = 1;
        __hip_atomic_store(st.done_host, 1, __ATOMIC_RELEASE, __HIP_MEMORY_SCOPE_SYSTEM);
    }
}

__global__ __launch_bounds__(256) void search_update_kernel(const SearchParams* __restrict__ spp, SearchState st) {
    if (*st.done) return;
    const SearchParams sp = *spp;
    const int item = blockIdx.x;
    const int tid = threadIdx.x;
    int step_no = 0;
    if (item == 0 && tid == 0) step_no = atomicAdd(st.step, 1) + 1;
    if (st.item_done[item]) { if (step_no) step_mirror(st, step_no); return; }
    const int r0 = item * sp.R;
    const int plen = st.plen[item];

    __shared__ short anc_s[16 * WLX_T_TEXT];
    __shared__ int parent[16], newtok[16];
    __shared__ float newcum[16];
    __shared__ int hyp_src[16], hyp_extra[16], hyp_slot[16], hyp_n;
    __shared__ int n_active_s, finished_s;

    if (!sp.sampling) {
        const int p = st.pos[r0];
        const int ngen = p + 1 - plen;
        const int max_new = sp.max_length - plen;
        const bool is_last = (ngen + 1 >= max_new);
        if (tid == 0) {
            bool used[16 * WLX_MAX_CAND];
            for (int i = 0; i < sp.beam * sp.ncand; ++i) used[i] = false;
            int n_active = 0, nh_new = 0, n_hyp = st.n_hyp[item];
            bool top_beam_finished = false;
            for (int k = 0; k < sp.ncand; ++k) {
                float bs = WLX_NEG_INF; int bb = -1, bj = -1;
                for (int b = 0; b < sp.beam; ++b)
                    for (int j = 0; j < sp.ncand; ++j) {
                        if (used[b * sp.ncand + j]) continue;
                        const float sc = st.cand_score[(long)(r0 + b) * WLX_MAX_CAND + j];
                        if (bb < 0 || sc > bs) { bs = sc; bb = b; bj = j; }
                        break;
                    }
                if (bb < 0) break;
                used[bb * sp.ncand + bj] = true;
                const int tok = st.cand_tok[(long)(r0 + bb) * WLX_MAX_CAND + bj];
                if (tok == sp.eot || is_last) {
                    if (k >= sp.beam) continue;
                    if (n_hyp + nh_new < WLX_MAX_HYP && nh_new < 16) {
                        const int len = ngen + ((tok == sp.eot) ? 0 : 1);
                        const int slot = n_hyp + nh_new;
                        hyp_src[nh_new] = bb;
                        hyp_extra[nh_new] = (tok == sp.eot) ? -1 : tok;
                        hyp_slot[nh_new] = slot;
                        st.hyp_len[item * WLX_MAX_HYP + slot] = len;
                        const float denom = powf((float)(len > 0 ? len : 1), sp.length_penalty);
                        st.hyp_score[item * WLX_MAX_HYP + slot] = bs / denom;
                        ++nh_new;
// ... 52 lines not shown
            }
            st.pos[r0 + j] = p + 1;
            st.nsp_row[r0 + j] = 0;
        }
    } else {
        __shared__ int alive;
        if (tid == 0) alive = 0;
        __syncthreads();
        for (int b = 0; b < sp.num_hyp; ++b) {
            const int r = r0 + b;
            if (st.row_done[r]) continue;
            const int p = st.pos[r];
            const int ngen = p + 1 - plen;
            const bool is_last = (ngen + 1 >= sp.max_length - plen);
            const int tok = st.samp_tok[r];
            const float cum = st.cum[r] + st.samp_lp[r];
            const bool fin = (tok == sp.eot) || is_last;
            if (fin) {
                int* dst = st.hyp_tokens + ((long)item * WLX_MAX_HYP + b) * WLX_T_TEXT;
                const short* ar = st.anc + (long)r * WLX_T_TEXT;
                for (int j = tid; j < ngen; j += 256) dst[j] = st.intok[(long)ar[plen + j] * WLX_T_TEXT + plen + j];
                if (tid == 0) {
                    const int len = ngen + ((tok == sp.eot) ? 0 : 1);
                    if (tok != sp.eot) dst[ngen] = tok;
                    st.hyp_len[item * WLX_MAX_HYP + b] = len;
                    st.hyp_score[item * WLX_MAX_HYP + b] = cum / powf((float)(len > 0 ? len : 1), sp.length_penalty);
                    st.row_done[r] = 1;
                    st.cum[r] = cum;
                }
            } else if (tid == 0) {
                st.cum[r] = cum;
                st.token[r] = tok;
                st.pos[r] = p + 1;
                st.anc[(long)r * WLX_T_TEXT + p + 1] = (short)r;
                st.nsp_row[r] = 0;
                alive = 1;
            }
            __syncthreads();
        }
        __syncthreads();
        if (tid == 0 && !alive) {
            st.n_hyp[item] = sp.num_hyp; st.n_hyp_host[item] = sp.num_hyp;
            finish_item(st, item, sp.items);
        }
    }
    if (step_no) step_mirror(st, step_no);
}

void launch_search_update(const SearchParams* sp_dev, int items, const SearchState& st, hipStream_t s) {
    hipLaunchKernelGGL(search_update_kernel, dim3(items), dim3(256), 0, s, sp_dev, st);
}


__device__ __forceinline__ float s3_wave_sum(float v) { return dpp_wave_sum(v); }
__device__ __forceinline__ float s3_wave_max(float v) { return dpp_wave_max(v); }
__device__ __forceinline__ void s3_wave_argmax(float& v, int& i) {
    const float m = dpp_wave_max(v);
    const unsigned long long hit = __ballot(v == m);
    int id;
    if (__builtin_popcountll(hit) == 1) id = __builtin_amdgcn_readlane(i, (int)__builtin_ctzll(hit));
    else id = dpp_wave_min_i32((v == m) ? i : 0x7fffffff);
    i = id;
    v = m;
}
__device__ __forceinline__ void s3_row_argmax(float& v, int& i) {
    float m = v;
    WLX_DPP_REDUCE_ROW("v_max_f32_dpp", m);
    int t = (v == m) ? i : 0x7fffffff;
    WLX_DPP_REDUCE_ROW("v_min_i32_dpp", t);
    v = m; i = t;
}

__device__ __forceinline__ void s3_chunk(int chunk, int ts_begin, int V, int& id0, int& lim, int& nct, int& nch) {
    nct = (ts_begin + SC_CHUNK - 1) / SC_CHUNK;
    nch = nct + (V - ts_begin + SC_CHUNK - 1) / SC_CHUNK;
    const bool is_ts = chunk >= nct;
    id0 = is_ts ? ts_begin + (chunk - nct) * SC_CHUNK : chunk * SC_CHUNK;
    lim = is_ts ? V : ts_begin;
}

__global__ __launch_bounds__(SC_THREADS) void search_scan3_kernel(const float* __restrict__ logits, long ldl, int V,
                                                                  const SearchParams* __restrict__ spp, SearchState st WLX_TR_PARAM) {
    const int chunk = blockIdx.x, r = blockIdx.y, tid = threadIdx.x, lane = tid & 63;
    const int wave = __builtin_amdgcn_readfirstlane(tid >> 6);
    WLX_TR_BEGIN();
    const SearchParams sp = *spp;
    int id0, lim, nct, nch_;
    s3_chunk(chunk, sp.ts_begin, V, id0, lim, nct, nch_);
    if (chunk >= nch_) return;
    const float* lrow = logits + (long)r * ldl + id0 + tid;
    float v[SC_NPT];
#pragma unroll
    for (int i = 0; i < SC_NPT; ++i) v[i] = (id0 + i * SC_THREADS + tid < lim) ? lrow[i * SC_THREADS] : WLX_NEG_INF;
    const int item = r / sp.R;
    const int rb = r - item * sp.R;
    const int4 rule = *reinterpret_cast<const int4*>(st.rule + 4 * r);
    const int p = st.pos[r], plen = st.plen[item], nsp = st.nsp_row[r];
    if (st.item_done[item] || rb >= sp.beam) return;
    const int ngen = p + 1 - plen;

    __shared__ float fs[6][4];
    __shared__ float wv_s[4][WLX_MAX_CAND];
    __shared__ int wi_s[4][WLX_MAX_CAND];

    if (sp.rep_penalty != 1.0f || sp.no_repeat_ngram > 0) {
        __shared__ int hist[WLX_T_TEXT];
        const short* ar = st.anc + (long)r * WLX_T_TEXT;
        for (int j = tid; j < ngen; j += SC_THREADS) hist[j] = st.intok[(long)ar[plen + j] * WLX_T_TEXT + plen + j];
        __syncthreads();
        if (sp.rep_penalty != 1.0f) {
#pragma unroll
            for (int i = 0; i < SC_NPT; ++i) {
                const int id = id0 + i * SC_THREADS + tid;
                bool hit = false;
                for (int j = 0; j < ngen; ++j) hit = hit || (hist[j] == id);
                if (hit && id < lim) v[i] = (v[i] < 0.f) ? v[i] * sp.rep_penalty : v[i] / sp.rep_penalty;
            }
        }
        if (sp.no_repeat_ngram > 0 && ngen >= sp.no_repeat_ngram - 1) {
            const int n = sp.no_repeat_ngram;
            for (int j = 0; j + n - 1 < ngen; ++j) {
                bool match = true;
                for (int q = 0; q < n - 1; ++q) match = match && (hist[j + q] == hist[ngen - (n - 1) + q]);
                if (match) {
                    const int banned = hist[j + n - 1];
#pragma unroll
                    for (int i = 0; i < SC_NPT; ++i)
                        if (id0 + i * SC_THREADS + tid == banned) v[i] = WLX_NEG_INF;
                }
            }
        }
    }
// ... 91 lines not shown
#pragma unroll
                        for (int i = 0; i + stp < SC_NPT; i += 2 * stp)
                            if (tv[i + stp] > tv[i]) { tv[i] = tv[i + stp]; ti_[i] = ti_[i + stp]; }
                    bv = tv[0]; bi = ti_[0];
                }
                ++won;
            }
        }
        WLX_TR_MARK(3);
        __syncthreads();
        WLX_TR_MARK(4);
        if (wave == 0) {
            if (lane == 0) {
                float* so = st.scan_stats + ((long)r * SC_MAXCH + chunk) * SC_NSTAT;
                const float ssum = fs[3][0] + fs[3][1] + fs[3][2] + fs[3][3];
                so[0] = ts_chunk ? WLX_NEG_INF : mx; so[1] = ts_chunk ? 0.f : ssum;
                so[2] = ts_chunk ? mx : WLX_NEG_INF; so[3] = ts_chunk ? ssum : 0.f;
                so[4] = raw_m;   so[5] = fs[5][0] + fs[5][1] + fs[5][2] + fs[5][3];
            }
            const int nc = sp.ncand;
            const int e0 = lane, e1 = lane + 64;
            float x0 = WLX_NEG_INF, x1 = WLX_NEG_INF; int i0 = 0x7fffffff, i1 = 0x7fffffff;
            if (e0 < 4 * nc) { const int q = e0 / nc, k = e0 - q * nc; x0 = wv_s[q][k]; i0 = wi_s[q][k]; }
            if (e1 < 4 * nc) { const int q = e1 / nc, k = e1 - q * nc; x1 = wv_s[q][k]; i1 = wi_s[q][k]; }
#pragma unroll 1
            for (int k = 0; k < nc; ++k) {
                const bool f1 = (x1 > x0) || (x1 == x0 && i1 < i0);
                float gv = f1 ? x1 : x0; int gi = f1 ? i1 : i0;
                s3_wave_argmax(gv, gi);
                if (lane == 0) { cv[k] = gv; ci[k] = gi; }
                if (gi != 0x7fffffff) {
                    if (i0 == gi) { x0 = WLX_NEG_INF; i0 = 0x7fffffff; }
                    if (i1 == gi) { x1 = WLX_NEG_INF; i1 = 0x7fffffff; }
                }
            }
        }
    }
    WLX_TR_MARK(5);
    WLX_TR_END(trc);
}

void launch_search_scan3(const float* logits, long ldl, int V, const SearchParams* sp_dev, int rows, const SearchState& st,
                         hipStream_t s) {
    hipLaunchKernelGGL(search_scan3_kernel, dim3(SC_MAXCH, rows), dim3(SC_THREADS), 0, s, logits, ldl, V, sp_dev, st WLX_TR_ARG("search_scan3"));
}

#define MU3_THREADS 384
__global__ __launch_bounds__(MU3_THREADS) void search_merge_update3_kernel(const float* __restrict__ logits, long ldl, int V,
                                                                           const SearchParams* __restrict__ spp, SearchState st, int R WLX_TR_PARAM) {
    const int item = blockIdx.x;
    const int tid = threadIdx.x, lane = tid & 63;
    const int wave = __builtin_amdgcn_readfirstlane(tid >> 6);
    constexpr int NW = MU3_THREADS / 64;
    constexpr int PQ = 3;
    const int r0 = item * R;
    const int done_v = *st.done;
    const int idone = st.item_done[item];
    const int plen = st.plen[item];
    const int p = st.pos[r0];
    const int n_hyp0 = st.n_hyp[item];
    const int rp = r0 + (wave < R ? wave : R - 1);
    const int lc = lane < SC_MAXCH ? lane : SC_MAXCH - 1;
    const float4* pso = reinterpret_cast<const float4*>(st.scan_stats + ((long)rp * SC_MAXCH + lc) * SC_NSTAT);
    const float4 ps0 = pso[0], ps1 = pso[1];
    const float4* pcv = reinterpret_cast<const float4*>(st.scan_cv + ((long)rp * (SC_MAXCH + 1) + lc) * WLX_MAX_CAND);
    const int4* pci = reinterpret_cast<const int4*>(st.scan_ci + ((long)rp * (SC_MAXCH + 1) + lc) * WLX_MAX_CAND);
    float4 pa[PQ]; int4 pb[PQ];
#pragma unroll
    for (int k = 0; k < PQ; ++k) { pa[k] = pcv[k]; pb[k] = pci[k]; }
    const float pcum = st.cum[rp];
    const int pnsp = st.nsp_row[rp];
    const SearchParams sp = *spp;
    if (done_v) return;
    WLX_TR_BEGIN();
    int step_no = 0;
    if (item == 0 && tid == 0) step_no = atomicAdd(st.step, 1) + 1;
    if (idone) { if (step_no) step_mirror(st, step_no); return; }
    int id0_, lim_, nct, nch;
    s3_chunk(0, sp.ts_begin, V, id0_, lim_, nct, nch);

    __shared__ float cand_s[16][WLX_MAX_CAND];
    __shared__ int cand_t[16][WLX_MAX_CAND];
    __shared__ float lv[NW][SC_MAXCH + 1][WLX_MAX_CAND];
    __shared__ int li[NW][SC_MAXCH + 1][WLX_MAX_CAND];
    __shared__ short anc_s[16 * WLX_T_TEXT];
    __shared__ int parent[16], newtok[16];
    __shared__ float newcum[16];
    __shared__ int hyp_src[16], hyp_extra[16], hyp_slot[16], hyp_n;
    __shared__ int n_active_s, finished_s;
    __shared__ int ord_b[WLX_MAX_CAND], ord_t[WLX_MAX_CAND];
    __shared__ float ord_s[WLX_MAX_CAND];
    __shared__ int4 rule_old[16];

    for (int i = tid; i < sp.beam * (p + 1); i += MU3_THREADS) {
        const int b = i / (p + 1), q = i - b * (p + 1);
        anc_s[b * WLX_T_TEXT + q] = st.anc[(long)(r0 + b) * WLX_T_TEXT + q];
    }
    if (tid < sp.beam) rule_old[tid] = *reinterpret_cast<const int4*>(st.rule + 4 * (r0 + tid));

    const bool ts = sp.apply_ts_rules != 0;
    const int nc4 = (sp.ncand + 3) >> 2;
#pragma unroll 1
    for (int rb = wave; rb < sp.beam; rb += NW) {
        const int r = r0 + rb;
        const bool first = rb == wave;
        const bool have = lane < nch;
        float4 s0 = make_float4(WLX_NEG_INF, 0.f, WLX_NEG_INF, 0.f), s1 = make_float4(WLX_NEG_INF, 0.f, 0.f, 0.f);
        float cum_r; int nsp_r;
        {
            const float4* cv = reinterpret_cast<const float4*>(st.scan_cv + ((long)r * (SC_MAXCH + 1) + lc) * WLX_MAX_CAND);
            const int4* ci = reinterpret_cast<const int4*>(st.scan_ci + ((long)r * (SC_MAXCH + 1) + lc) * WLX_MAX_CAND);
            float4 a[WLX_MAX_CAND / 4]; int4 b[WLX_MAX_CAND / 4];
            if (first) {
#pragma unroll
                for (int k = 0; k < PQ; ++k) { a[k] = pa[k]; b[k] = pb[k]; }
#pragma unroll
                for (int k = PQ; k < WLX_MAX_CAND / 4; ++k)
                    if (k < nc4) { a[k] = cv[k]; b[k] = ci[k]; }
                if (have) { s0 = ps0; s1 = ps1; }
                cum_r = pcum; nsp_r = pnsp;
            } else {
#pragma unroll
                for (int k = 0; k < WLX_MAX_CAND / 4; ++k)
                    if (k < nc4) { a[k] = cv[k]; b[k] = ci[k]; }
                const float4* so = reinterpret_cast<const float4*>(st.scan_stats + ((long)r * SC_MAXCH + lc) * SC_NSTAT);
                const float4 t0 = so[0], t1 = so[1];
                if (have) { s0 = t0; s1 = t1; }
                cum_r = st.cum[r]; nsp_r = st.nsp_row[r];
            }
#pragma unroll
            for (int k = 0; k < WLX_MAX_CAND / 4; ++k)
                if (k < nc4 && have) {
                    *reinterpret_cast<float4*>(&lv[wave][lane][4 * k]) = have ? a[k] : make_float4(WLX_NEG_INF, WLX_NEG_INF, WLX_NEG_INF, WLX_NEG_INF);
                    *reinterpret_cast<int4*>(&li[wave][lane][4 * k]) = have ? b[k] : make_int4(0x7fffffff, 0x7fffffff, 0x7fffffff, 0x7fffffff);
                }
        }
        const float mt = s0.x, st_ = s0.y, mts = s0.z, sts = s0.w, rm = s1.x, rs = s1.y;
        const float Mtext = s3_wave_max(mt), Mts = s3_wave_max(mts);
        if (nsp_r > 0) {
            const float RM = s3_wave_max(rm);
            const float RS = s3_wave_sum((rm > WLX_NEG_INF) ? rs * __expf(rm - RM) : 0.f);
            if (lane == 0) st.no_speech[item] = __expf(logits[(long)r * ldl + sp.no_speech] - RM) / RS;
        }
        const float S_ts = s3_wave_sum((mts > WLX_NEG_INF) ? sts * __expf(mts - Mts) : 0.f);
        const float lse_ts = (Mts > WLX_NEG_INF) ? Mts + __logf(S_ts) : WLX_NEG_INF;
        const bool text_masked = ts && (lse_ts > Mtext);
        float lse_sel;
        if (text_masked) {
            lse_sel = lse_ts;
        } else {
            const float mx_all = fmaxf(Mtext, Mts);
            const float a = ((mt > WLX_NEG_INF) ? st_ * __expf(mt - mx_all) : 0.f) +
                            ((mts > WLX_NEG_INF) ? sts * __expf(mts - mx_all) : 0.f);
            lse_sel = mx_all + __logf(s3_wave_sum(a));
        }
        const bool usable = (lane < nch) && (!text_masked || lane >= nct);
        const float base = cum_r - lse_sel;
        int hp = 0;
        float hv = usable ? lv[wave][lane][0] : WLX_NEG_INF;
        int hi = usable ? li[wave][lane][0] : 0x7fffffff;
#pragma unroll 1
        for (int k = 0; k < sp.ncand; ++k) {
            float gv = hv; int gi = hi;
            s3_wave_argmax(gv, gi);
            if (lane == 0) {
                cand_s[rb][k] = (gi < V) ? gv + base : WLX_NEG_INF;
                cand_t[rb][k] = (gi < V) ? gi : sp.eot;
            }
            if (usable && gi != 0x7fffffff && hi == gi) {
                ++hp;
                hv = (hp < sp.ncand) ? lv[wave][lane][hp] : WLX_NEG_INF;
                hi = (hp < sp.ncand) ? li[wave][lane][hp] : 0x7fffffff;
            }
        }
    }
    __syncthreads();
    WLX_TR_MARK(1);

    const int ngen = p + 1 - plen;
    const int max_new = sp.max_length - plen;
    const bool is_last = (ngen + 1 >= max_new);
    if (wave == 0) {
        const int b = lane;
        const bool own = b < sp.beam;
        int hp = 0;
#pragma unroll 1
        for (int k = 0; k < sp.ncand; ++k) {
            const bool alive = own && hp < sp.ncand;
            float kv = alive ? cand_s[b][hp] : WLX_NEG_INF;
            int kb = alive ? b : 0x7fffffff;
            s3_row_argmax(kv, kb);
            if (lane == 0) ord_b[k] = (kb == 0x7fffffff) ? -1 : kb;
            if (alive && b == kb) { ord_s[k] = cand_s[b][hp]; ord_t[k] = cand_t[b][hp]; ++hp; }
        }
        const int k = lane;
        const bool in_list = k < sp.ncand;
        const int bb = in_list ? ord_b[k] : -1;
        const float bs = in_list ? ord_s[k] : 0.f;
        const int tok = in_list ? ord_t[k] : 0;
        const unsigned long long stop = __ballot(!in_list || bb < 0);
        const bool live = k < (int)__builtin_ctzll(stop);
        const bool fin_k = live && (tok == sp.eot || is_last);
        const bool act_k = live && !fin_k;
        const unsigned long long below = (1ull << k) - 1ull;
        const unsigned long long finm = __ballot(fin_k && k < sp.beam);
        const unsigned long long actm = __ballot(act_k);
        int cap = WLX_MAX_HYP - n_hyp0; cap = cap < 16 ? cap : 16; cap = cap > 0 ? cap : 0;
        const int hidx = __builtin_popcountll(finm & below), aidx = __builtin_popcountll(actm & below);
        if (fin_k && k < sp.beam && hidx < cap) {
            const int len = ngen + ((tok == sp.eot) ? 0 : 1);
            const int slot = n_hyp0 + hidx;
            hyp_src[hidx] = bb;
            hyp_extra[hidx] = (tok == sp.eot) ? -1 : tok;
            hyp_slot[hidx] = slot;
            st.hyp_len[item * WLX_MAX_HYP + slot] = len;
            const float flen = (float)(len > 0 ? len : 1);
            const float denom = (sp.length_penalty == 1.0f) ? flen : powf(flen, sp.length_penalty);
            st.hyp_score[item * WLX_MAX_HYP + slot] = bs / denom;
        }
        if (act_k && aidx < sp.beam) { parent[aidx] = bb; newtok[aidx] = tok; newcum[aidx] = bs; }
        if (lane == 0) {
            int nh_new = __builtin_popcountll(finm); nh_new = nh_new < cap ? nh_new : cap;
            int n_active = __builtin_popcountll(actm); n_active = n_active < sp.beam ? n_active : sp.beam;
            const bool top_beam_finished = fin_k;
            const int n_hyp = n_hyp0 + nh_new;
            st.n_hyp[item] = n_hyp; st.n_hyp_host[item] = n_hyp;
            hyp_n = nh_new;
            n_active_s = n_active;
            bool fin = is_last || n_active == 0;
            if (sp.allow_early_exit) fin = fin || (top_beam_finished && n_hyp >= sp.num_hyp);
            else fin = fin || (n_hyp >= sp.max_cand_hyp);
            finished_s = fin ? 1 : 0;
        }
    }
    __syncthreads();
    WLX_TR_MARK(2);
    for (int hh = 0; hh < hyp_n; ++hh) {
        const int b = hyp_src[hh];
        int* dst = st.hyp_tokens + ((long)item * WLX_MAX_HYP + hyp_slot[hh]) * WLX_T_TEXT;
        for (int j = tid; j < ngen; j += MU3_THREADS)
            dst[j] = st.intok[(long)anc_s[b * WLX_T_TEXT + plen + j] * WLX_T_TEXT + plen + j];
        if (tid == 0 && hyp_extra[hh] >= 0) dst[ngen] = hyp_extra[hh];
    }
    if (finished_s) {
        __syncthreads();
        if (tid == 0) {
            if (step_no) step_mirror(st, step_no);
            finish_item(st, item, sp.items);
        }
        return;
    }
    const int na = n_active_s;
    for (int i = tid; i < na * (p + 1); i += MU3_THREADS) {
        const int j = i / (p + 1), q = i - j * (p + 1);
        st.anc[(long)(r0 + j) * WLX_T_TEXT + q] = anc_s[parent[j] * WLX_T_TEXT + q];
    }
    if (tid < sp.beam) {
        const int j = tid;
        st.anc[(long)(r0 + j) * WLX_T_TEXT + p + 1] = (short)(r0 + j);
        int4 ru = make_int4(0, 1, -1, 0);
        if (j < na) {
            const int tok = newtok[j];
            const int4 po = rule_old[parent[j]];
            const int is_ts = tok >= sp.ts_begin ? 1 : 0;
            ru.x = is_ts;
            ru.y = (ngen + 1 < 2) ? 1 : po.x;
            ru.z = is_ts ? tok : po.z;
            st.token[r0 + j] = tok; st.cum[r0 + j] = newcum[j];
        } else { st.token[r0 + j] = sp.eot; st.cum[r0 + j] = WLX_NEG_INF; }
        *reinterpret_cast<int4*>(st.rule + 4 * (r0 + j)) = ru;
        st.pos[r0 + j] = p + 1;
        st.nsp_row[r0 + j] = 0;
    }
    if (step_no) step_mirror(st, step_no);
    WLX_TR_END(trc);
}

void launch_search_merge_update3(const float* logits, long ldl, int V, const SearchParams* sp_dev, int items, int R,
                                 const SearchState& st, hipStream_t s) {
    hipLaunchKernelGGL(search_merge_update3_kernel, dim3(items), dim3(MU3_THREADS), 0, s, logits, ldl, V, sp_dev, st, R WLX_TR_ARG("search_merge_update3"));
}

__global__ __launch_bounds__(256) void search_reset_kernel(SearchState st, int items, int rows) {
    const int t = threadIdx.x;
    if (t == 0) { *st.step = 0; *st.done = 0; *st.n_finished = 0; step_mirror(st, 0); }
    for (int i = t; i < items; i += 256) { st.item_done[i] = 0; st.n_hyp[i] = 0; st.n_hyp_host[i] = 0; st.no_speech[i] = 0.f; }
    for (int i = t; i < rows; i += 256) st.row_done[i] = 0;
    for (int i = t; i < items * WLX_MAX_HYP; i += 256) st.hyp_len[i] = 0;
}
void launch_search_reset(const SearchState& st, int items, int rows, hipStream_t s) {
    hipLaunchKernelGGL(search_reset_kernel, dim3(1), dim3(256), 0, s, st, items, rows);
}

__global__ __launch_bounds__(SR_THREADS) void token_prob_kernel(const float* __restrict__ logits, long ldl, int V,
                                                               int tok, float* __restrict__ out) {
    __shared__ float fs[16];
    const float* lrow = logits + (long)blockIdx.x * ldl;
    float mx = WLX_NEG_INF;
    for (int i = threadIdx.x; i < V; i += SR_THREADS) mx = fmaxf(mx, lrow[i]);
    mx = block_max(mx, fs);
    float sm = 0.f;
    for (int i = threadIdx.x; i < V; i += SR_THREADS) sm += __expf(lrow[i] - mx);
    sm = block_sum(sm, fs);
    if (threadIdx.x == 0) out[blockIdx.x] = __expf(lrow[tok] - mx) / sm;
}
__global__ __launch_bounds__(SR_THREADS) void token_prob_rows_kernel(const float* __restrict__ logits, long ldl, int vlim,
                                                                     const int* __restrict__ toks, float* __restrict__ out) {
    __shared__ float fs[16];
    const int r = blockIdx.x, tid = threadIdx.x;
    const float* lrow = logits + (long)r * ldl;
    float mx = WLX_NEG_INF;
    for (int i = tid; i < vlim; i += SR_THREADS) mx = fmaxf(mx, lrow[i]);
    mx = block_max(mx, fs);
    float sm = 0.f;
    for (int i = tid; i < vlim; i += SR_THREADS) sm += __expf(lrow[i] - mx);
    sm = block_sum(sm, fs);
    if (tid == 0) { const int t = toks[r]; out[r] = (t >= 0 && t < vlim) ? __expf(lrow[t] - mx) / sm : 0.f; }
}
void launch_token_prob_rows(const float* logits, long ldl, int vlim, int rows, const int* toks, float* out, hipStream_t s) {
    hipLaunchKernelGGL(token_prob_rows_kernel, dim3(rows), dim3(SR_THREADS), 0, s, logits, ldl, vlim, toks, out);
}

void launch_token_prob(const float* logits, long ldl, int V, int rows, int tok, float* out, hipStream_t s) {
    hipLaunchKernelGGL(token_prob_kernel, dim3(rows), dim3(SR_THREADS), 0, s, logits, ldl, V, tok, out);
}

__global__ __launch_bounds__(256) void lang_probs_kernel(const float* __restrict__ logits, long ldl,
                                                         const int* __restrict__ ids, int n, float* __restrict__ probs) {
    __shared__ float red[4];
    const float* lrow = logits + (long)blockIdx.x * ldl;
    float mx = WLX_NEG_INF;
    for (int i = threadIdx.x; i < n; i += 256) mx = fmaxf(mx, lrow[ids[i]]);
    mx = wave_max(mx);
// ... 18 lines not shown
```

Before: 1154 xRT (audio s / wall s).

## Fold beam-search merge/update into next step's first-layer QKV GEMV kernel

Removes the separate search_merge_update3 launch in the greedy/beam path by folding the merge work into the layer-0 embed+LN+QKV GEMV kernel. An extra block 0 does the bookkeeping (hypothesis commit, ancestry, rule state), while every other block redundantly recomputes the beam winners from the scan partials so it knows which tokens to embed. Winner state is passed between steps through a double-buffered fold scratch array. This saves one kernel launch and one serial dependency per decode step. In exchange, each GEMV block does extra merge work, and the change adds new graph variants and a single-item, rows-at-most-16 restriction.

```diff
diff --git a/whisperlive_amd/csrc/decoder.h b/whisperlive_amd/csrc/decoder.h
--- a/whisperlive_amd/csrc/decoder.h
+++ b/whisperlive_amd/csrc/decoder.h
@@ -21,7 +21,31 @@
 enum GemvIn : int { GEMV_IN_LN = 0, GEMV_IN_F16 = 1, GEMV_IN_XATTN = 2 };
 enum GemvOut : int { GEMV_OUT_F16 = 0, GEMV_OUT_GELU_F16 = 1, GEMV_OUT_F32 = 2, GEMV_OUT_RESID = 3, GEMV_OUT_QKV = 4,
                      GEMV_OUT_SLAB = 5 };
-enum GemvXsrc : int { GEMV_X_PLAIN = 0, GEMV_X_SLABS = 1, GEMV_X_EMBED = 2 };
+enum GemvXsrc : int { GEMV_X_PLAIN = 0, GEMV_X_SLABS = 1, GEMV_X_EMBED = 2, GEMV_X_FOLD = 3 };
+struct SearchParams;
+struct SearchState {
+    int* step;
+    int* done;
+    int* done_host;
+    int* n_finished;
+    int* item_done;
+    int* plen;
+    float* cum;
+    int* row_done;
+    float* cand_score; int* cand_tok;
+    int* samp_tok; float* samp_lp;
+    int* hyp_tokens;
+    int* hyp_len;
+    float* hyp_score;
+    int* n_hyp;
+    int* n_hyp_host;
+    float* no_speech;
+    int* nsp_row;
+    int* token; int* pos; short* anc; int* intok;
+    float* scan_stats;
+    float* scan_cv; int* scan_ci;
+    int* rule;
+};
 #ifndef WLX_CQ_GB_LDS
 #define WLX_CQ_GB_LDS 1
 #endif
@@ -64,6 +88,9 @@
     float* slab; long slab_stride;
     int KTS;
     const half_t* tok_emb; const float* pos_emb; const int* emb_token; int* intok;
+    const SearchParams* fold_sp; SearchState fold_st;
+    const int* fold_in; int* fold_out;
+    const float* fold_logits; long fold_ldl; int fold_V;
     WLX_TR_FIELD
 };
 #ifdef WLX_TRACE
@@ -99,29 +126,6 @@
 void launch_dec_xattn_combine(const half_t* part_o, const float* part_ml, int M, int H, int R, half_t* out, long ldo, hipStream_t s);
 void launch_dec_align_scores(const half_t* q, long ldq, const half_t* Kp_item, int h, int rows, float* out, hipStream_t s);
 
-struct SearchState {
-    int* step;
-    int* done;
-    int* done_host;
-    int* n_finished;
-    int* item_done;
-    int* plen;
-    float* cum;
-    int* row_done;
-    float* cand_score; int* cand_tok;
-    int* samp_tok; float* samp_lp;
-    int* hyp_tokens;
-    int* hyp_len;
-    float* hyp_score;
-    int* n_hyp;
-    int* n_hyp_host;
-    float* no_speech;
-    int* nsp_row;
-    int* token; int* pos; short* anc; int* intok;
-    float* scan_stats;
-    float* scan_cv; int* scan_ci;
-    int* rule;
-};
 #define SC_THREADS 256
 #define SC_NPT 8
 #define SC_CHUNK (SC_THREADS * SC_NPT)
@@ -147,6 +151,8 @@
                          hipStream_t s);
 void launch_search_merge_update3(const float* logits, long ldl, int V, const SearchParams* sp_dev, int items, int R,
                                  const SearchState& st, hipStream_t s);
+void launch_search_fold_seed(const SearchState& st, int* fold, int rows, hipStream_t s);
+#define WLX_FOLD_WORDS 64
 void launch_search_reset(const SearchState& st, int items, int rows, hipStream_t s);
 void launch_token_prob_rows(const float* logits, long ldl, int vlim, int rows, const int* toks, float* out, hipStream_t s);
 void launch_token_prob(const float* logits, long ldl, int V, int rows, int tok, float* out, hipStream_t s);
diff --git a/whisperlive_amd/csrc/decoder.hip b/whisperlive_amd/csrc/decoder.hip
--- a/whisperlive_amd/csrc/decoder.hip
+++ b/whisperlive_amd/csrc/decoder.hip
@@ -1,4 +1,5 @@
 #include "decoder.h"
+#include "search_merge.h"
 #include <algorithm>
 #include <cstdlib>
 #include <cstdio>
@@ -442,6 +443,14 @@
                   "slab / embedding sources: LayerNorm prologue or residual epilogue only");
     static_assert(OUT != GEMV_OUT_SLAB || (IN == GEMV_IN_F16 && NTB == 1), "K-split form: fp16 rows in");
     extern __shared__ __attribute__((aligned(16))) float smem[];
+    if constexpr (XS == GEMV_X_FOLD) {
+        if (blockIdx.x == 0) {
+            s3_fold_bookkeep(p.fold_logits, p.fold_ldl, p.fold_V, p.fold_sp, p.fold_st, p.M, p.fold_in, p.fold_out, (int)threadIdx.x, (int)blockDim.x,
+                             *reinterpret_cast<S3FoldLds*>(smem));
+            return;
+        }
+        tile -= 1;
+    }
     const int tid = threadIdx.x, lane = tid & 63, c = lane & 15, g = lane >> 4;
     const int wave = __builtin_amdgcn_readfirstlane(tid >> 6);
     const int nw = p.nwm;
@@ -475,6 +484,14 @@
 #define WLX_X_FIRST 1
 #endif
     if (!WLX_X_FIRST) load_weights();
+    __shared__ int fold_tok_s[XS == GEMV_X_FOLD ? 16 : 1];
+    __shared__ int fold_pos_s;
+    int fold_pos = 0;
+    if constexpr (XS == GEMV_X_FOLD) {
+        s3_fold_winners(p.fold_sp, p.fold_st, p.fold_in, p.fold_V, p.M, tid, (int)(blockDim.x >> 6), reinterpret_cast<S3FoldLds*>(smem)->L, fold_tok_s, &fold_pos_s,
+                        [&]() { if (WLX_X_FIRST) load_weights(); });
+        fold_pos = __builtin_amdgcn_readfirstlane(fold_pos_s);
+    }
 
     int crow[MT];
 #pragma unroll
@@ -488,7 +505,7 @@
     int rc_e = 0, rp_e = 0;
     if constexpr (OUT != GEMV_OUT_F32) bias_e = *reinterpret_cast<const float4*>(p.bias + n_e);
     if constexpr (OUT == GEMV_OUT_RESID) res_e = *reinterpret_cast<const float4*>(p.Xres + (long)row_e * p.ldxres + n_e);
-    if constexpr (OUT == GEMV_OUT_QKV) { rc_e = p.row_cache[row_e]; rp_e = p.row_pos[row_e]; }
+    if constexpr (OUT == GEMV_OUT_QKV) { rc_e = p.row_cache[row_e]; rp_e = (XS == GEMV_X_FOLD) ? fold_pos : p.row_pos[row_e]; }
     float4 slab_e[(OUT == GEMV_OUT_RESID && XS == GEMV_X_SLABS) ? WLX_FC2_KS : 1];
     if constexpr (OUT == GEMV_OUT_RESID && XS == GEMV_X_SLABS) {
 #pragma unroll
@@ -562,9 +579,14 @@
         f16x4 te[NV];
         int tok0 = 0, pos0 = 0;
         auto request_row = [&](int r, float4 (&x)[NV], float4 (&sl)[NSL][NV], f16x4 (&te)[NV], int& tok, int& pos) {
-            if constexpr (XS == GEMV_X_EMBED) {
+            if constexpr (XS == GEMV_X_FOLD) {
+                tok = __builtin_amdgcn_readfirstlane(fold_tok_s[r]);
+                pos = fold_pos | (p.row_cache[r] << 16);
+            } else if constexpr (XS == GEMV_X_EMBED) {
                 tok = p.emb_token[r];
                 pos = p.row_pos[r] | (p.row_cache[r] << 16);
+            }
+            if constexpr (XS == GEMV_X_EMBED || XS == GEMV_X_FOLD) {
                 const half_t* tp = p.tok_emb + (long)tok * p.K + lane * 4;
                 const float4* pp = reinterpret_cast<const float4*>(p.pos_emb + (long)(pos & 0xffff) * p.K) + lane;
 #pragma unroll
@@ -590,7 +612,7 @@
 #pragma unroll
                     for (int j = 0; j < NV; ++j) { x[j].x += sl[q][j].x; x[j].y += sl[q][j].y; x[j].z += sl[q][j].z; x[j].w += sl[q][j].w; }
             }
-            if constexpr (XS == GEMV_X_EMBED) {
+            if constexpr (XS == GEMV_X_EMBED || XS == GEMV_X_FOLD) {
 #pragma unroll
                 for (int j = 0; j < NV; ++j) { x[j].x += (float)te[j][0]; x[j].y += (float)te[j][1]; x[j].z += (float)te[j][2]; x[j].w += (float)te[j][3]; }
                 if (tile == 0 && keep) {
@@ -614,7 +636,7 @@
         float4 gq[NV], bq[NV];
 #pragma unroll
         for (int j = 0; j < NV; ++j) { const int tb = (j == NV - 1) ? tback : 0; gq[j] = g4[64 * j - tb]; bq[j] = b4[64 * j - tb]; }
-        if (WLX_X_FIRST) load_weights();
+        if (WLX_X_FIRST && XS != GEMV_X_FOLD) load_weights();
         const int ldxs = p.K + 8;
         constexpr float invK = LNT ? (1.0f / 384.0f) : 1.0f / (256.0f * NV);
         auto ln_row = [&](float4 (&x)[NV], int r, bool keep) {
@@ -1100,6 +1122,7 @@
     if constexpr (ROWS == G2_LN_XS) {
         if (p.out_mode != GEMV_OUT_QKV || c.NTB != 1) return false;
         if (p.xsrc == GEMV_X_SLABS) return leaf(G2Args<CH, LNV, GEMV_IN_LN, GEMV_OUT_QKV, 1, MT, GEMV_X_SLABS>{});
+        if constexpr (MT == 1) { if (p.xsrc == GEMV_X_FOLD) return p.M <= 16 && p.Mtot == 0 && leaf(G2Args<CH, LNV, GEMV_IN_LN, GEMV_OUT_QKV, 1, 1, GEMV_X_FOLD>{}); }
         return p.xsrc == GEMV_X_EMBED && leaf(G2Args<CH, LNV, GEMV_IN_LN, GEMV_OUT_QKV, 1, MT, GEMV_X_EMBED>{});
     } else if constexpr (ROWS == G2_LN_PLAIN) {
         switch (p.out_mode) {
@@ -1174,7 +1197,9 @@
         const int want = (p.M * p.H * 8 + 63) / 64;
         block.x = 64 * std::max(c.nw, std::min(c.MT > 1 ? 8 : 16, want));
     }
-    const bool launched = gemv2_dispatch(p, c, [&](auto a) { using A = decltype(a); g2_launch<A::CH, A::LNV, A::IN, A::OUT, A::NTB, A::MT, A::XS>(grid, block, c.shm, s, p); return true; });
+    size_t shm = c.shm;
+    if (p.xsrc == GEMV_X_FOLD) { grid.x += 1; shm = std::max(shm, sizeof(S3FoldLds)); }
+    const bool launched = gemv2_dispatch(p, c, [&](auto a) { using A = decltype(a); g2_launch<A::CH, A::LNV, A::IN, A::OUT, A::NTB, A::MT, A::XS>(grid, block, shm, s, p); return true; });
     if (!launched) dispatch_bug("dec_gemv2_kernel", s);
 }
 static GemvParams gemv_chunked(const GemvParams& p) {
@@ -1199,7 +1224,7 @@
                           (p.N & 15) == 0 && ((p.N >> 4) & 3) == 0;
     const bool rt_shape = p.N <= 1536 || (long)p.N * p.K <= 3200000L || ln_wide4;
     if (rt_on && !g_decode_v1 && p.M > rt_chunk && p.M <= rt_max && rt_shape) { q.Mtot = p.M; q.M = rt_chunk; q.chunk = rt_chunk; q.rt_nz = (p.M + rt_chunk - 1) / rt_chunk; }
-    else if (p.M > 48 && p.xsrc != GEMV_X_EMBED) { q.Mtot = p.M; q.M = 48; q.chunk = 48; }
+    else if (p.M > 48 && p.xsrc != GEMV_X_EMBED && p.xsrc != GEMV_X_FOLD) { q.Mtot = p.M; q.M = 48; q.chunk = 48; }
     return q;
 }
 
diff --git a/whisperlive_amd/csrc/engine.h b/whisperlive_amd/csrc/engine.h
--- a/whisperlive_amd/csrc/engine.h
+++ b/whisperlive_amd/csrc/engine.h
@@ -71,6 +71,7 @@
     bool anc_ident = false;
     SearchState st{};
     SearchParams* d_sp = nullptr;
+    int* d_fold = nullptr;
     unsigned* d_suppress = nullptr;
     int* d_lang_ids = nullptr; float* d_probs = nullptr; float* d_tokprob = nullptr;
     int* h_stage = nullptr; size_t h_stage_ints = 0;
@@ -113,6 +114,7 @@
     std::mutex mu;
     std::vector<Slot*> slots;
     bool use_graph = true;
+    bool merge_fold = true;
 };
 
 }
diff --git a/whisperlive_amd/csrc/engine.hip b/whisperlive_amd/csrc/engine.hip
--- a/whisperlive_amd/csrc/engine.hip
+++ b/whisperlive_amd/csrc/engine.hip
@@ -150,6 +150,8 @@
         if (weights[i].on_device) { g_embedded_device_memory.store(true); break; }
     const char* ng = getenv("WLX_NO_GRAPH");
     e->use_graph = !(ng && ng[0] == '1');
+    const char* mf = getenv("WLX_MERGE_FOLD");
+    e->merge_fold = !(mf && mf[0] == '0');
     const char* v1 = wlx_ab("WLX_DECODE_V1");
     g_decode_v1 = (v1 && v1[0] == '1');
     int rc = engine_load(e, weights, n_weights);
@@ -457,6 +459,7 @@
         CKR(dalloc(s->allocs, &s->d_align_tgt, (size_t)WLX_T_TEXT, true));
         CKR(dalloc(s->allocs, &s->d_align_prob, (size_t)WLX_T_TEXT, true));
         CKR(dalloc(s->allocs, &s->d_sp, 1, true));
+        CKR(dalloc(s->allocs, &s->d_fold, (size_t)2 * WLX_FOLD_WORDS, true));
         CKR(dalloc(s->allocs, &s->d_suppress, (size_t)(1024 * 52 / 32), true));
         CKR(dalloc(s->allocs, &s->d_lang_ids, 256, true));
         CKR(dalloc(s->allocs, &s->d_probs, (size_t)B * 256, true));
@@ -904,7 +907,11 @@
     if (s->prof->list_only) { s->prof->recs.push_back(ProfRec{name, bytes}); return; }
     if (s->prof->only == name) f();
 }
-static double gemv_bytes(const GemvParams& p) { return 2.0 * (double)p.N * (double)p.K + (p.bias ? 4.0 * p.N : 0.0); }
+static double gemv_bytes(const GemvParams& p) {
+    double b = 2.0 * (double)p.N * (double)p.K + (p.bias ? 4.0 * p.N : 0.0);
+    if (p.xsrc == GEMV_X_FOLD) b += (double)p.M * SC_MAXCH * (SC_NSTAT * 4.0 + 2.0 * WLX_MAX_CAND * 4.0);
+    return b;
+}
 static bool device_is_busy(const Slot* s) {
     return s->device_of >= 0 && s->device_of < 64 && g_slots_live[s->device_of].load(std::memory_order_relaxed) >= 3;
 }
@@ -916,7 +923,7 @@
     plaunch(s, nm.c_str(), gemv_bytes(p), [&] { launch_dec_gemv(p, s->stream); });
 }
 
-static void decoder_pass(Engine* e, Slot* s_, int rows, int R, int groups, bool with_logits, bool check_done, const Slot::DecBufs* alt = nullptr) {
+static void decoder_pass(Engine* e, Slot* s_, int rows, int R, int groups, bool with_logits, bool check_done, const Slot::DecBufs* alt = nullptr, int fold_copy = -1) {
     const wlx_spec& sp = e->spec;
     const int d = sp.d_model, F = sp.ffn, H = e->H;
     struct View {
@@ -940,9 +947,15 @@
         p.Kc = s->kc + (size_t)l * s->cache_rows * crs; p.Vc = s->vc + (size_t)l * s->cache_rows * crs; p.cache_row_stride = crs;
         p.row_cache = s.d_cache; p.row_pos = s.d_pos; p.done = done;
         p.xsrc = xsrc; p.slab = s.slab; p.slab_stride = s.slab_rows * d;
-        if (xsrc == GEMV_X_EMBED) {
+        if (xsrc == GEMV_X_EMBED || xsrc == GEMV_X_FOLD) {
             p.tok_emb = e->tok_emb16; p.pos_emb = e->dec_pos; p.emb_token = s.d_token; p.intok = s->d_intok;
             p.Xres = s.xd; p.ldxres = d;
+        }
+        if (xsrc == GEMV_X_FOLD) {
+            const SearchState& S = s->st;
+            p.fold_sp = s->d_sp; p.fold_st = S;
+            p.fold_in = s->d_fold + (size_t)(fold_copy & 1) * WLX_FOLD_WORDS; p.fold_out = s->d_fold + (size_t)((fold_copy & 1) ^ 1) * WLX_FOLD_WORDS;
+            p.fold_logits = s->logits; p.fold_ldl = s->ldl; p.fold_V = sp.vocab;
         }
         return p;
     };
@@ -976,7 +989,7 @@
         half_t* kc = s->kc + (size_t)l * s->cache_rows * crs;
         half_t* vc = s->vc + (size_t)l * s->cache_rows * crs;
         {
-            GemvParams pq = qkv_params(l, (l == 0 && fold_embed) ? GEMV_X_EMBED : (slabs_pending ? GEMV_X_SLABS : GEMV_X_PLAIN));
+            GemvParams pq = qkv_params(l, (l == 0 && fold_embed) ? (fold_copy >= 0 ? GEMV_X_FOLD : GEMV_X_EMBED) : (slabs_pending ? GEMV_X_SLABS : GEMV_X_PLAIN));
             pgemv(s.base, pq);
         }
         plaunch(s.base, "dec_self_attn2_kernel", 4.0 * rows * d * (s->prof ? s->prof->t + 1 : 1), [&] { launch_dec_self_attn(s.qd, d, kc, vc, crs, d, H, rt, rows, s.attnd, d, done, s->anc_ident, st); });
@@ -1120,14 +1133,22 @@
     return WLX_OK;
 }
 
-static void launch_search(Engine* e, Slot* s, int rows, int R, int groups, bool sampling) {
+static void launch_search(Engine* e, Slot* s, int rows, int R, int groups, bool sampling, bool merge = true) {
     if (sampling || g_decode_v1) {
         launch_search_rows(s->logits, s->d_sp, rows, s->st, s->stream);
         launch_search_update(s->d_sp, groups, s->st, s->stream);
     } else {
         launch_search_scan3(s->logits, s->ldl, e->spec.vocab, s->d_sp, rows, s->st, s->stream);
-        launch_search_merge_update3(s->logits, s->ldl, e->spec.vocab, s->d_sp, groups, R, s->st, s->stream);
-    }
+        if (merge) launch_search_merge_update3(s->logits, s->ldl, e->spec.vocab, s->d_sp, groups, R, s->st, s->stream);
+    }
+}
+static int fold_copy_of(int fold_step0, int k) { return (fold_step0 < 0 || fold_step0 + k == 0) ? -1 : ((fold_step0 + k - 1) & 1); }
+static bool fold_form_ok(Engine* e, int rows) {
+    static const float dummy_bias = 0.f;
+    const int d = e->spec.d_model;
+    GemvParams p{};
+    p.in_mode = GEMV_IN_LN; p.out_mode = GEMV_OUT_QKV; p.M = rows; p.K = d; p.KT = d / 32; p.N = 3 * d; p.bias = &dummy_bias; p.xsrc = GEMV_X_FOLD;
+    return rows <= 16 && dec_gemv_is_lean(p);
 }
 
 static int graph_steps_for(const Slot* s, int rows) {
@@ -1137,9 +1158,10 @@
     return alone ? 2 : 1;
 }
 
-static int get_step_graph(Engine* e, Slot* s, int rows, int R, int groups, bool sampling, int nsteps, hipGraphExec_t* out) {
+static int get_step_graph(Engine* e, Slot* s, int rows, int R, int groups, bool sampling, int nsteps, int fold_step0, hipGraphExec_t* out) {
     s->busy_variant = device_is_busy(s);
-    StepGraphKey key{rows, R, groups * 8 + (nsteps == 2 ? 4 : 0) + (s->busy_variant ? 2 : 0) + (sampling ? 1 : 0)};
+    const int fold_mode = fold_step0 < 0 ? 0 : (fold_step0 == 0 ? 1 : 2 + ((fold_step0 - 1) & 1));
+    StepGraphKey key{rows, R, groups * 32 + fold_mode * 8 + (nsteps == 2 ? 4 : 0) + (s->busy_variant ? 2 : 0) + (sampling ? 1 : 0)};
     auto it = s->graphs.find(key);
     if (it != s->graphs.end()) { *out = it->second; return WLX_OK; }
     hipGraph_t graph;
@@ -1147,8 +1169,8 @@
     CK(hipGetLastError());
     CK(hipStreamBeginCapture(s->stream, hipStreamCaptureModeThreadLocal));
     for (int k = 0; k < nsteps; ++k) {
-        decoder_pass(e, s, rows, R, groups, true, true);
-        launch_search(e, s, rows, R, groups, sampling);
+        decoder_pass(e, s, rows, R, groups, true, true, nullptr, fold_copy_of(fold_step0, k));
+        launch_search(e, s, rows, R, groups, sampling, fold_step0 < 0);
     }
     const hipError_t ce = hipStreamEndCapture(s->stream, &graph);
     if (ce != hipSuccess) {
@@ -1171,16 +1193,16 @@
     return WLX_OK;
 }
 
-static int run_step(Engine* e, Slot* s, int rows, int R, int groups, bool sampling, int nsteps = 1) {
+static int run_step(Engine* e, Slot* s, int rows, int R, int groups, bool sampling, int nsteps = 1, int fold_step0 = -1) {
     if (e->use_graph) {
         hipGraphExec_t exec;
-        CKR(get_step_graph(e, s, rows, R, groups, sampling, nsteps, &exec));
+        CKR(get_step_graph(e, s, rows, R, groups, sampling, nsteps, fold_step0, &exec));
         CK(hipGraphLaunch(exec, s->stream));
     } else {
         s->busy_variant = device_is_busy(s);
         for (int k = 0; k < nsteps; ++k) {
-            decoder_pass(e, s, rows, R, groups, true, true);
-            launch_search(e, s, rows, R, groups, sampling);
+            decoder_pass(e, s, rows, R, groups, true, true, nullptr, fold_copy_of(fold_step0, k));
+            launch_search(e, s, rows, R, groups, sampling, fold_step0 < 0);
         }
         CK(hipGetLastError());
     }
@@ -1376,6 +1398,9 @@
         memcpy(h_nsp, nsp.data(), (size_t)rows * 4);
         CK(hipMemcpyAsync(S.nsp_row, h_nsp, rows * 4, hipMemcpyHostToDevice, st));
     }
+    const bool fold = e->merge_fold && !sampling && !injected_logits && batch == 1 && !g_decode_v1 && !s->prof && !s->align &&
+                      h_sp->rep_penalty == 1.f && h_sp->no_repeat_ngram <= 0 && fold_form_ok(e, rows);
+    if (fold) launch_search_fold_seed(S, s->d_fold, rows, st);
     volatile int* h_done = s->h_stage + (s->h_stage_ints - 4);
     h_done[0] = 0;
     h_done[1] = 0;
@@ -1396,7 +1421,7 @@
         } else {
             const double ta = gen_trace ? now_us() : 0.0;
             n_this = std::min(gsteps, max_steps - step);
-            CKR(run_step(e, s, rows, R, batch, sampling, n_this));
+            CKR(run_step(e, s, rows, R, batch, sampling, n_this, fold ? step : -1));
             if (gen_trace) tg_launch += now_us() - ta;
         }
         steps_run += n_this;
@@ -1419,6 +1444,10 @@
             if (gen_trace) tg_wait += now_us() - ta;
             finished = h_done[0] != 0;
         }
+    }
+    if (fold && steps_run > 0 && !finished) {
+        launch_search_merge_update3(s->logits, s->ldl, V, s->d_sp, batch, R, S, st);
+        CK(hipGetLastError());
     }
     const double tg2 = now_us();
     if (gen_trace) CK(hipStreamSynchronize(st));
diff --git a/whisperlive_amd/csrc/search.hip b/whisperlive_amd/csrc/search.hip
--- a/whisperlive_amd/csrc/search.hip
+++ b/whisperlive_amd/csrc/search.hip
@@ -1,4 +1,5 @@
 #include "decoder.h"
+#include "search_merge.h"
 
 namespace wlx {
 
@@ -299,20 +300,6 @@
 
 void launch_search_rows(const float* logits, const SearchParams* sp_dev, int rows, const SearchState& st, hipStream_t s) {
     hipLaunchKernelGGL(search_rows_kernel, dim3(rows), dim3(SR_THREADS), 0, s, logits, sp_dev, st);
-}
-
-__device__ __forceinline__ void step_mirror(const SearchState& st, int step_no) {
-    __hip_atomic_store(st.done_host + 1, step_no, __ATOMIC_RELEASE, __HIP_MEMORY_SCOPE_SYSTEM);
-}
-__device__ __forceinline__ void finish_item(const SearchState& st, int item, int items) {
-    st.item_done[item] = 1;
-    __threadfence_system();
-    const int nf = atomicAdd(st.n_finished, 1) + 1;
-    if (nf >= items) {
-        __threadfence_system();
-        *st.done = 1;
-        __hip_atomic_store(st.done_host, 1, __ATOMIC_RELEASE, __HIP_MEMORY_SCOPE_SYSTEM);
-    }
 }
 
 __global__ __launch_bounds__(256) void search_update_kernel(const SearchParams* __restrict__ spp, SearchState st) {
@@ -471,32 +458,6 @@
 }
 
 
-__device__ __forceinline__ float s3_wave_sum(float v) { return dpp_wave_sum(v); }
-__device__ __forceinline__ float s3_wave_max(float v) { return dpp_wave_max(v); }
-__device__ __forceinline__ void s3_wave_argmax(float& v, int& i) {
-    const float m = dpp_wave_max(v);
-    const unsigned long long hit = __ballot(v == m);
-    int id;
-    if (__builtin_popcountll(hit) == 1) id = __builtin_amdgcn_readlane(i, (int)__builtin_ctzll(hit));
-    else id = dpp_wave_min_i32((v == m) ? i : 0x7fffffff);
-    i = id;
-    v = m;
-}
-__device__ __forceinline__ void s3_row_argmax(float& v, int& i) {
-    float m = v;
-    WLX_DPP_REDUCE_ROW("v_max_f32_dpp", m);
-    int t = (v == m) ? i : 0x7fffffff;
-    WLX_DPP_REDUCE_ROW("v_min_i32_dpp", t);
-    v = m; i = t;
-}
-
-__device__ __forceinline__ void s3_chunk(int chunk, int ts_begin, int V, int& id0, int& lim, int& nct, int& nch) {
-    nct = (ts_begin + SC_CHUNK - 1) / SC_CHUNK;
-    nch = nct + (V - ts_begin + SC_CHUNK - 1) / SC_CHUNK;
-    const bool is_ts = chunk >= nct;
-    id0 = is_ts ? ts_begin + (chunk - nct) * SC_CHUNK : chunk * SC_CHUNK;
-    lim = is_ts ? V : ts_begin;
-}
 
 __global__ __launch_bounds__(SC_THREADS) void search_scan3_kernel(const float* __restrict__ logits, long ldl, int V,
                                                                   const SearchParams* __restrict__ spp, SearchState st WLX_TR_PARAM) {
@@ -694,7 +655,6 @@
     const int tid = threadIdx.x, lane = tid & 63;
     const int wave = __builtin_amdgcn_readfirstlane(tid >> 6);
     constexpr int NW = MU3_THREADS / 64;
-    constexpr int PQ = 3;
     const int r0 = item * R;
     const int done_v = *st.done;
     const int idone = st.item_done[item];
@@ -703,15 +663,8 @@
     const int n_hyp0 = st.n_hyp[item];
     const int rp = r0 + (wave < R ? wave : R - 1);
     const int lc = lane < SC_MAXCH ? lane : SC_MAXCH - 1;
-    const float4* pso = reinterpret_cast<const float4*>(st.scan_stats + ((long)rp * SC_MAXCH + lc) * SC_NSTAT);
-    const float4 ps0 = pso[0], ps1 = pso[1];
-    const float4* pcv = reinterpret_cast<const float4*>(st.scan_cv + ((long)rp * (SC_MAXCH + 1) + lc) * WLX_MAX_CAND);
-    const int4* pci = reinterpret_cast<const int4*>(st.scan_ci + ((long)rp * (SC_MAXCH + 1) + lc) * WLX_MAX_CAND);
-    float4 pa[PQ]; int4 pb[PQ];
-#pragma unroll
-    for (int k = 0; k < PQ; ++k) { pa[k] = pcv[k]; pb[k] = pci[k]; }
-    const float pcum = st.cum[rp];
-    const int pnsp = st.nsp_row[rp];
+    S3RowFetch pf;
+    s3_merge_request(st, st.cum, true, rp, lc, pf);
     const SearchParams sp = *spp;
     if (done_v) return;
     WLX_TR_BEGIN();
@@ -721,101 +674,12 @@
     int id0_, lim_, nct, nch;
     s3_chunk(0, sp.ts_begin, V, id0_, lim_, nct, nch);
 
-    __shared__ float cand_s[16][WLX_MAX_CAND];
-    __shared__ int cand_t[16][WLX_MAX_CAND];
-    __shared__ float lv[NW][SC_MAXCH + 1][WLX_MAX_CAND];
-    __shared__ int li[NW][SC_MAXCH + 1][WLX_MAX_CAND];
-    __shared__ short anc_s[16 * WLX_T_TEXT];
-    __shared__ int parent[16], newtok[16];
-    __shared__ float newcum[16];
-    __shared__ int hyp_src[16], hyp_extra[16], hyp_slot[16], hyp_n;
-    __shared__ int n_active_s, finished_s;
-    __shared__ int ord_b[WLX_MAX_CAND], ord_t[WLX_MAX_CAND];
-    __shared__ float ord_s[WLX_MAX_CAND];
-    __shared__ int4 rule_old[16];
-
-    for (int i = tid; i < sp.beam * (p + 1); i += MU3_THREADS) {
-        const int b = i / (p + 1), q = i - b * (p + 1);
-        anc_s[b * WLX_T_TEXT + q] = st.anc[(long)(r0 + b) * WLX_T_TEXT + q];
-    }
-    if (tid < sp.beam) rule_old[tid] = *reinterpret_cast<const int4*>(st.rule + 4 * (r0 + tid));
-
-    const bool ts = sp.apply_ts_rules != 0;
-    const int nc4 = (sp.ncand + 3) >> 2;
-#pragma unroll 1
-    for (int rb = wave; rb < sp.beam; rb += NW) {
-        const int r = r0 + rb;
-        const bool first = rb == wave;
-        const bool have = lane < nch;
-        float4 s0 = make_float4(WLX_NEG_INF, 0.f, WLX_NEG_INF, 0.f), s1 = make_float4(WLX_NEG_INF, 0.f, 0.f, 0.f);
-        float cum_r; int nsp_r;
-        {
-            const float4* cv = reinterpret_cast<const float4*>(st.scan_cv + ((long)r * (SC_MAXCH + 1) + lc) * WLX_MAX_CAND);
-            const int4* ci = reinterpret_cast<const int4*>(st.scan_ci + ((long)r * (SC_MAXCH + 1) + lc) * WLX_MAX_CAND);
-            float4 a[WLX_MAX_CAND / 4]; int4 b[WLX_MAX_CAND / 4];
-            if (first) {
-#pragma unroll
-                for (int k = 0; k < PQ; ++k) { a[k] = pa[k]; b[k] = pb[k]; }
-#pragma unroll
-                for (int k = PQ; k < WLX_MAX_CAND / 4; ++k)
-                    if (k < nc4) { a[k] = cv[k]; b[k] = ci[k]; }
-                if (have) { s0 = ps0; s1 = ps1; }
-                cum_r = pcum; nsp_r = pnsp;
-            } else {
-#pragma unroll
-                for (int k = 0; k < WLX_MAX_CAND / 4; ++k)
-                    if (k < nc4) { a[k] = cv[k]; b[k] = ci[k]; }
-                const float4* so = reinterpret_cast<const float4*>(st.scan_stats + ((long)r * SC_MAXCH + lc) * SC_NSTAT);
-                const float4 t0 = so[0], t1 = so[1];
-                if (have) { s0 = t0; s1 = t1; }
-                cum_r = st.cum[r]; nsp_r = st.nsp_row[r];
-            }
-#pragma unroll
-            for (int k = 0; k < WLX_MAX_CAND / 4; ++k)
-                if (k < nc4 && have) {
-                    *reinterpret_cast<float4*>(&lv[wave][lane][4 * k]) = have ? a[k] : make_float4(WLX_NEG_INF, WLX_NEG_INF, WLX_NEG_INF, WLX_NEG_INF);
-                    *reinterpret_cast<int4*>(&li[wave][lane][4 * k]) = have ? b[k] : make_int4(0x7fffffff, 0x7fffffff, 0x7fffffff, 0x7fffffff);
-                }
-        }
-        const float mt = s0.x, st_ = s0.y, mts = s0.z, sts = s0.w, rm = s1.x, rs = s1.y;
-        const float Mtext = s3_wave_max(mt), Mts = s3_wave_max(mts);
-        if (nsp_r > 0) {
-            const float RM = s3_wave_max(rm);
-            const float RS = s3_wave_sum((rm > WLX_NEG_INF) ? rs * __expf(rm - RM) : 0.f);
-            if (lane == 0) st.no_speech[item] = __expf(logits[(long)r * ldl + sp.no_speech] - RM) / RS;
-        }
-        const float S_ts = s3_wave_sum((mts > WLX_NEG_INF) ? sts * __expf(mts - Mts) : 0.f);
-        const float lse_ts = (Mts > WLX_NEG_INF) ? Mts + __logf(S_ts) : WLX_NEG_INF;
-        const bool text_masked = ts && (lse_ts > Mtext);
-        float lse_sel;
-        if (text_masked) {
-            lse_sel = lse_ts;
-        } else {
-            const float mx_all = fmaxf(Mtext, Mts);
-            const float a = ((mt > WLX_NEG_INF) ? st_ * __expf(mt - mx_all) : 0.f) +
-                            ((mts > WLX_NEG_INF) ? sts * __expf(mts - mx_all) : 0.f);
-            lse_sel = mx_all + __logf(s3_wave_sum(a));
-        }
-        const bool usable = (lane < nch) && (!text_masked || lane >= nct);
-        const float base = cum_r - lse_sel;
-        int hp = 0;
-        float hv = usable ? lv[wave][lane][0] : WLX_NEG_INF;
-        int hi = usable ? li[wave][lane][0] : 0x7fffffff;
-#pragma unroll 1
-        for (int k = 0; k < sp.ncand; ++k) {
-            float gv = hv; int gi = hi;
-            s3_wave_argmax(gv, gi);
-            if (lane == 0) {
-                cand_s[rb][k] = (gi < V) ? gv + base : WLX_NEG_INF;
-                cand_t[rb][k] = (gi < V) ? gi : sp.eot;
-            }
-            if (usable && gi != 0x7fffffff && hi == gi) {
-                ++hp;
-                hv = (hp < sp.ncand) ? lv[wave][lane][hp] : WLX_NEG_INF;
-                hi = (hp < sp.ncand) ? li[wave][lane][hp] : 0x7fffffff;
-            }
-        }
-    }
+    __shared__ S3MergeLds<NW> L;
+    __shared__ S3BookLds B;
+
+    s3_book_stage(sp, st, r0, p, tid, MU3_THREADS, B);
+
+    s3_merge_rows<NW>(logits, ldl, V, sp, st, st.cum, item, r0, wave, NW, lane, lc, nct, nch, pf, true, L);
     __syncthreads();
     WLX_TR_MARK(1);
 
@@ -823,104 +687,34 @@
     const int max_new = sp.max_length - plen;
     const bool is_last = (ngen + 1 >= max_new);
     if (wave == 0) {
-        const int b = lane;
-        const bool own = b < sp.beam;
-        int hp = 0;
-#pragma unroll 1
-        for (int k = 0; k < sp.ncand; ++k) {
-            const bool alive = own && hp < sp.ncand;
-            float kv = alive ? cand_s[b][hp] : WLX_NEG_INF;
-            int kb = alive ? b : 0x7fffffff;
-            s3_row_argmax(kv, kb);
-            if (lane == 0) ord_b[k] = (kb == 0x7fffffff) ? -1 : kb;
-            if (alive && b == kb) { ord_s[k] = cand_s[b][hp]; ord_t[k] = cand_t[b][hp]; ++hp; }
-        }
-        const int k = lane;
-        const bool in_list = k < sp.ncand;
-        const int bb = in_list ? ord_b[k] : -1;
-        const float bs = in_list ? ord_s[k] : 0.f;
-        const int tok = in_list ? ord_t[k] : 0;
-        const unsigned long long stop = __ballot(!in_list || bb < 0);
-        const bool live = k < (int)__builtin_ctzll(stop);
-        const bool fin_k = live && (tok == sp.eot || is_last);
-        const bool act_k = live && !fin_k;
-        const unsigned long long below = (1ull << k) - 1ull;
-        const unsigned long long finm = __ballot(fin_k && k < sp.beam);
-        const unsigned long long actm = __ballot(act_k);
-        int cap = WLX_MAX_HYP - n_hyp0; cap = cap < 16 ? cap : 16; cap = cap > 0 ? cap : 0;
-        const int hidx = __builtin_popcountll(finm & below), aidx = __builtin_popcountll(actm & below);
-        if (fin_k && k < sp.beam && hidx < cap) {
-            const int len = ngen + ((tok == sp.eot) ? 0 : 1);
-            const int slot = n_hyp0 + hidx;
-            hyp_src[hidx] = bb;
-            hyp_extra[hidx] = (tok == sp.eot) ? -1 : tok;
-            hyp_slot[hidx] = slot;
-            st.hyp_len[item * WLX_MAX_HYP + slot] = len;
-            const float flen = (float)(len > 0 ? len : 1);
-            const float denom = (sp.length_penalty == 1.0f) ? flen : powf(flen, sp.length_penalty);
-            st.hyp_score[item * WLX_MAX_HYP + slot] = bs / denom;
-        }
-        if (act_k && aidx < sp.beam) { parent[aidx] = bb; newtok[aidx] = tok; newcum[aidx] = bs; }
-        if (lane == 0) {
-            int nh_new = __builtin_popcountll(finm); nh_new = nh_new < cap ? nh_new : cap;
-            int n_active = __builtin_popcountll(actm); n_active = n_active < sp.beam ? n_active : sp.beam;
-            const bool top_beam_finished = fin_k;
-            const int n_hyp = n_hyp0 + nh_new;
-            st.n_hyp[item] = n_hyp; st.n_hyp_host[item] = n_hyp;
-            hyp_n = nh_new;
-            n_active_s = n_active;
-            bool fin = is_last || n_active == 0;
-            if (sp.allow_early_exit) fin = fin || (top_beam_finished && n_hyp >= sp.num_hyp);
-            else fin = fin || (n_hyp >= sp.max_cand_hyp);
-            finished_s = fin ? 1 : 0;
-        }
+        s3_merge_beams<NW>(sp, lane, L);
+        s3_book_select<NW>(sp, st, item, lane, n_hyp0, ngen, is_last, L, B);
     }
     __syncthreads();
     WLX_TR_MARK(2);
-    for (int hh = 0; hh < hyp_n; ++hh) {
-        const int b = hyp_src[hh];
-        int* dst = st.hyp_tokens + ((long)item * WLX_MAX_HYP + hyp_slot[hh]) * WLX_T_TEXT;
-        for (int j = tid; j < ngen; j += MU3_THREADS)
-            dst[j] = st.intok[(long)anc_s[b * WLX_T_TEXT + plen + j] * WLX_T_TEXT + plen + j];
-        if (tid == 0 && hyp_extra[hh] >= 0) dst[ngen] = hyp_extra[hh];
-    }
-    if (finished_s) {
-        __syncthreads();
-        if (tid == 0) {
-            if (step_no) step_mirror(st, step_no);
-            finish_item(st, item, sp.items);
-        }
-        return;
-    }
-    const int na = n_active_s;
-    for (int i = tid; i < na * (p + 1); i += MU3_THREADS) {
-        const int j = i / (p + 1), q = i - j * (p + 1);
-        st.anc[(long)(r0 + j) * WLX_T_TEXT + q] = anc_s[parent[j] * WLX_T_TEXT + q];
-    }
-    if (tid < sp.beam) {
-        const int j = tid;
-        st.anc[(long)(r0 + j) * WLX_T_TEXT + p + 1] = (short)(r0 + j);
-        int4 ru = make_int4(0, 1, -1, 0);
-        if (j < na) {
-            const int tok = newtok[j];
-            const int4 po = rule_old[parent[j]];
-            const int is_ts = tok >= sp.ts_begin ? 1 : 0;
-            ru.x = is_ts;
-            ru.y = (ngen + 1 < 2) ? 1 : po.x;
-            ru.z = is_ts ? tok : po.z;
-            st.token[r0 + j] = tok; st.cum[r0 + j] = newcum[j];
-        } else { st.token[r0 + j] = sp.eot; st.cum[r0 + j] = WLX_NEG_INF; }
-        *reinterpret_cast<int4*>(st.rule + 4 * (r0 + j)) = ru;
-        st.pos[r0 + j] = p + 1;
-        st.nsp_row[r0 + j] = 0;
-    }
-    if (step_no) step_mirror(st, step_no);
+    if (s3_book_commit(sp, st, item, r0, p, plen, ngen, step_no, tid, MU3_THREADS, B)) return;
     WLX_TR_END(trc);
 }
 
 void launch_search_merge_update3(const float* logits, long ldl, int V, const SearchParams* sp_dev, int items, int R,
                                  const SearchState& st, hipStream_t s) {
     hipLaunchKernelGGL(search_merge_update3_kernel, dim3(items), dim3(MU3_THREADS), 0, s, logits, ldl, V, sp_dev, st, R WLX_TR_ARG("search_merge_update3"));
+}
+
+__global__ __launch_bounds__(S3_FOLD_WORDS) void search_fold_seed_kernel(SearchState st, int* __restrict__ fold, int rows) {
+    static_assert(S3_FOLD_WORDS == WLX_FOLD_WORDS, "fold copy size");
+    const int t = threadIdx.x;
+    int v = 0;
+    if (t == S3_FOLD_DONE) v = *st.done;
+    if (t == S3_FOLD_IDONE) v = st.item_done[0];
+    if (t == S3_FOLD_POS) v = st.pos[0];
+    if (t == S3_FOLD_NHYP) v = st.n_hyp[0];
+    if (t >= S3_FOLD_CUM && t < S3_FOLD_CUM + 16 && t - S3_FOLD_CUM < rows) v = __float_as_int(st.cum[t - S3_FOLD_CUM]);
+    if (t >= S3_FOLD_TOK && t < S3_FOLD_TOK + 16 && t - S3_FOLD_TOK < rows) v = st.token[t - S3_FOLD_TOK];
+    fold[t] = v;
+}
+void launch_search_fold_seed(const SearchState& st, int* fold, int rows, hipStream_t s) {
+    hipLaunchKernelGGL(search_fold_seed_kernel, dim3(1), dim3(S3_FOLD_WORDS), 0, s, st, fold, rows);
 }
 
 __global__ __launch_bounds__(256) void search_reset_kernel(SearchState st, int items, int rows) {
diff --git a/whisperlive_amd/csrc/search_merge.h b/whisperlive_amd/csrc/search_merge.h
--- /dev/null
+++ b/whisperlive_amd/csrc/search_merge.h
@@ -0,0 +1,401 @@
+#pragma once
+#include "decoder.h"
+
+namespace wlx {
+
+__device__ __forceinline__ void step_mirror(const SearchState& st, int step_no) {
+    __hip_atomic_store(st.done_host + 1, step_no, __ATOMIC_RELEASE, __HIP_MEMORY_SCOPE_SYSTEM);
+}
+__device__ __forceinline__ void finish_item(const SearchState& st, int item, int items) {
+    st.item_done[item] = 1;
+    __threadfence_system();
+    const int nf = atomicAdd(st.n_finished, 1) + 1;
+    if (nf >= items) {
+        __threadfence_system();
+        *st.done = 1;
+        __hip_atomic_store(st.done_host, 1, __ATOMIC_RELEASE, __HIP_MEMORY_SCOPE_SYSTEM);
+    }
+}
+
+__device__ __forceinline__ float s3_wave_sum(float v) { return dpp_wave_sum(v); }
+__device__ __forceinline__ float s3_wave_max(float v) { return dpp_wave_max(v); }
+__device__ __forceinline__ void s3_wave_argmax(float& v, int& i) {
+    const float m = dpp_wave_max(v);
+    const unsigned long long hit = __ballot(v == m);
+    int id;
+    if (__builtin_popcountll(hit) == 1) id = __builtin_amdgcn_readlane(i, (int)__builtin_ctzll(hit));
+    else id = dpp_wave_min_i32((v == m) ? i : 0x7fffffff);
+    i = id;
+    v = m;
+}
+__device__ __forceinline__ void s3_row_argmax(float& v, int& i) {
+    float m = v;
+    WLX_DPP_REDUCE_ROW("v_max_f32_dpp", m);
+    int t = (v == m) ? i : 0x7fffffff;
+    WLX_DPP_REDUCE_ROW("v_min_i32_dpp", t);
+    v = m; i = t;
+}
+
+__device__ __forceinline__ void s3_chunk(int chunk, int ts_begin, int V, int& id0, int& lim, int& nct, int& nch) {
+    nct = (ts_begin + SC_CHUNK - 1) / SC_CHUNK;
+    nch = nct + (V - ts_begin + SC_CHUNK - 1) / SC_CHUNK;
+    const bool is_ts = chunk >= nct;
+    id0 = is_ts ? ts_begin + (chunk - nct) * SC_CHUNK : chunk * SC_CHUNK;
+    lim = is_ts ? V : ts_begin;
+}
+
+#define S3_PQ 3
+template <int NW>
+struct alignas(16) S3MergeLds {
+    float lv[NW][SC_MAXCH + 1][WLX_MAX_CAND];
+    int li[NW][SC_MAXCH + 1][WLX_MAX_CAND];
+    float cand_s[16][WLX_MAX_CAND];
+    int cand_t[16][WLX_MAX_CAND];
+    int ord_b[WLX_MAX_CAND], ord_t[WLX_MAX_CAND];
+    float ord_s[WLX_MAX_CAND];
+};
+struct S3RowFetch {
+    float4 ps0, ps1;
+    float4 pa[S3_PQ]; int4 pb[S3_PQ];
+    float pcum; int pnsp;
+};
+__device__ __forceinline__ void s3_merge_request(const SearchState& st, const float* __restrict__ cum, bool publish, int rp, int lc, S3RowFetch& f) {
+    const float4* pso = reinterpret_cast<const float4*>(st.scan_stats + ((long)rp * SC_MAXCH + lc) * SC_NSTAT);
+    f.ps0 = pso[0]; f.ps1 = pso[1];
+    const float4* pcv = reinterpret_cast<const float4*>(st.scan_cv + ((long)rp * (SC_MAXCH + 1) + lc) * WLX_MAX_CAND);
+    const int4* pci = reinterpret_cast<const int4*>(st.scan_ci + ((long)rp * (SC_MAXCH + 1) + lc) * WLX_MAX_CAND);
+#pragma unroll
+    for (int k = 0; k < S3_PQ; ++k) { f.pa[k] = pcv[k]; f.pb[k] = pci[k]; }
+    f.pcum = cum[rp];
+    f.pnsp = publish ? st.nsp_row[rp] : 0;
+}
+
+template <int NW>
+__device__ __forceinline__ void s3_merge_rows(const float* __restrict__ logits, long ldl, int V, const SearchParams& sp, const SearchState& st,
+                                              const float* __restrict__ cum, int item, int r0, int wave, int nwv, int lane, int lc, int nct, int nch,
+                                              const S3RowFetch& f, bool publish, S3MergeLds<NW>& L) {
+    const bool ts = sp.apply_ts_rules != 0;
+    const int nc4 = (sp.ncand + 3) >> 2;
+#pragma unroll 1
+    for (int rb = wave; rb < sp.beam; rb += nwv) {
+        const int r = r0 + rb;
+        const bool first = rb == wave;
+        const bool have = lane < nch;
+        float4 s0 = make_float4(WLX_NEG_INF, 0.f, WLX_NEG_INF, 0.f), s1 = make_float4(WLX_NEG_INF, 0.f, 0.f, 0.f);
+        float cum_r; int nsp_r;
+        {
+            const float4* cv = reinterpret_cast<const float4*>(st.scan_cv + ((long)r * (SC_MAXCH + 1) + lc) * WLX_MAX_CAND);
+            const int4* ci = reinterpret_cast<const int4*>(st.scan_ci + ((long)r * (SC_MAXCH + 1) + lc) * WLX_MAX_CAND);
+            float4 a[WLX_MAX_CAND / 4]; int4 b[WLX_MAX_CAND / 4];
+            if (first) {
+#pragma unroll
+                for (int k = 0; k < S3_PQ; ++k) { a[k] = f.pa[k]; b[k] = f.pb[k]; }
+#pragma unroll
+                for (int k = S3_PQ; k < WLX_MAX_CAND / 4; ++k)
+                    if (k < nc4) { a[k] = cv[k]; b[k] = ci[k]; }
+                if (have) { s0 = f.ps0; s1 = f.ps1; }
+                cum_r = f.pcum; nsp_r = f.pnsp;
+            } else {
+#pragma unroll
+                for (int k = 0; k < WLX_MAX_CAND / 4; ++k)
+                    if (k < nc4) { a[k] = cv[k]; b[k] = ci[k]; }
+                const float4* so = reinterpret_cast<const float4*>(st.scan_stats + ((long)r * SC_MAXCH + lc) * SC_NSTAT);
+                const float4 t0 = so[0], t1 = so[1];
+                if (have) { s0 = t0; s1 = t1; }
+                cum_r = cum[r]; nsp_r = publish ? st.nsp_row[r] : 0;
+            }
+#pragma unroll
+            for (int k = 0; k < WLX_MAX_CAND / 4; ++k)
+                if (k < nc4 && have) {
+                    *reinterpret_cast<float4*>(&L.lv[wave][lane][4 * k]) = have ? a[k] : make_float4(WLX_NEG_INF, WLX_NEG_INF, WLX_NEG_INF, WLX_NEG_INF);
+                    *reinterpret_cast<int4*>(&L.li[wave][lane][4 * k]) = have ? b[k] : make_int4(0x7fffffff, 0x7fffffff, 0x7fffffff, 0x7fffffff);
+                }
+        }
+        const float mt = s0.x, st_ = s0.y, mts = s0.z, sts = s0.w, rm = s1.x, rs = s1.y;
+        const float Mtext = s3_wave_max(mt), Mts = s3_wave_max(mts);
+        if (nsp_r > 0 && publish) {
+            const float RM = s3_wave_max(rm);
+            const float RS = s3_wave_sum((rm > WLX_NEG_INF) ? rs * __expf(rm - RM) : 0.f);
+            if (lane == 0) st.no_speech[item] = __expf(logits[(long)r * ldl + sp.no_speech] - RM) / RS;
+        }
+        const float S_ts = s3_wave_sum((mts > WLX_NEG_INF) ? sts * __expf(mts - Mts) : 0.f);
+        const float lse_ts = (Mts > WLX_NEG_INF) ? Mts + __logf(S_ts) : WLX_NEG_INF;
+        const bool text_masked = ts && (lse_ts > Mtext);
+        float lse_sel;
+        if (text_masked) {
+            lse_sel = lse_ts;
+        } else {
+            const float mx_all = fmaxf(Mtext, Mts);
+            const float a = ((mt > WLX_NEG_INF) ? st_ * __expf(mt - mx_all) : 0.f) +
+                            ((mts > WLX_NEG_INF) ? sts * __expf(mts - mx_all) : 0.f);
+            lse_sel = mx_all + __logf(s3_wave_sum(a));
+        }
+        const bool usable = (lane < nch) && (!text_masked || lane >= nct);
+        const float base = cum_r - lse_sel;
+        int hp = 0;
+        float hv = usable ? L.lv[wave][lane][0] : WLX_NEG_INF;
+        int hi = usable ? L.li[wave][lane][0] : 0x7fffffff;
+#pragma unroll 1
+        for (int k = 0; k < sp.ncand; ++k) {
+            float gv = hv; int gi = hi;
+            s3_wave_argmax(gv, gi);
+            if (lane == 0) {
+                L.cand_s[rb][k] = (gi < V) ? gv + base : WLX_NEG_INF;
+                L.cand_t[rb][k] = (gi < V) ? gi : sp.eot;
+            }
+            if (usable && gi != 0x7fffffff && hi == gi) {
+                ++hp;
+                hv = (hp < sp.ncand) ? L.lv[wave][lane][hp] : WLX_NEG_INF;
+                hi = (hp < sp.ncand) ? L.li[wave][lane][hp] : 0x7fffffff;
+            }
+        }
+    }
+}
+
+template <int NW>
+__device__ __forceinline__ void s3_merge_beams(const SearchParams& sp, int lane, S3MergeLds<NW>& L) {
+    const int b = lane;
+    const bool own = b < sp.beam;
+    int hp = 0;
+#pragma unroll 1
+    for (int k = 0; k < sp.ncand; ++k) {
+        const bool alive = own && hp < sp.ncand;
+        float kv = alive ? L.cand_s[b][hp] : WLX_NEG_INF;
+        int kb = alive ? b : 0x7fffffff;
+        s3_row_argmax(kv, kb);
+        if (lane == 0) L.ord_b[k] = (kb == 0x7fffffff) ? -1 : kb;
+        if (alive && b == kb) { L.ord_s[k] = L.cand_s[b][hp]; L.ord_t[k] = L.cand_t[b][hp]; ++hp; }
+    }
+}
+
+struct S3Class {
+    int bb; float bs; int tok;
+    bool fin_k, act_k;
+    unsigned long long finm, actm;
+    int hidx, aidx;
+};
+template <int NW>
+__device__ __forceinline__ S3Class s3_classify(const SearchParams& sp, int lane, bool is_last, const S3MergeLds<NW>& L) {
+    S3Class c;
+    const int k = lane;
+    const bool in_list = k < sp.ncand;
+    c.bb = in_list ? L.ord_b[k] : -1;
+    c.bs = in_list ? L.ord_s[k] : 0.f;
+    c.tok = in_list ? L.ord_t[k] : 0;
+    const unsigned long long stop = __ballot(!in_list || c.bb < 0);
+    const bool live = k < (int)__builtin_ctzll(stop);
+    c.fin_k = live && (c.tok == sp.eot || is_last);
+    c.act_k = live && !c.fin_k;
+    const unsigned long long below = (1ull << k) - 1ull;
+    c.finm = __ballot(c.fin_k && k < sp.beam);
+    c.actm = __ballot(c.act_k);
+    c.hidx = __builtin_popcountll(c.finm & below); c.aidx = __builtin_popcountll(c.actm & below);
+    return c;
+}
+
+__device__ __forceinline__ bool s3_finished(const SearchParams& sp, const S3Class& c, int n_hyp0, bool is_last, int& nh_new, int& n_active) {
+    int cap = WLX_MAX_HYP - n_hyp0; cap = cap < 16 ? cap : 16; cap = cap > 0 ? cap : 0;
+    nh_new = __builtin_popcountll(c.finm); nh_new = nh_new < cap ? nh_new : cap;
+    n_active = __builtin_popcountll(c.actm); n_active = n_active < sp.beam ? n_active : sp.beam;
+    const bool top_beam_finished = (__ballot(c.fin_k) & 1ull) != 0;
+    const int n_hyp = n_hyp0 + nh_new;
+    bool fin = is_last || n_active == 0;
+    if (sp.allow_early_exit) fin = fin || (top_beam_finished && n_hyp >= sp.num_hyp);
+    else fin = fin || (n_hyp >= sp.max_cand_hyp);
+    return fin;
+}
+
+struct alignas(16) S3BookLds {
+    int4 rule_old[16];
+    short anc_s[16 * WLX_T_TEXT];
+    int parent[16], newtok[16];
+    float newcum[16];
+    int hyp_src[16], hyp_extra[16], hyp_slot[16], hyp_n;
+    int n_active_s, finished_s, n_hyp_s;
+};
+__device__ __forceinline__ void s3_book_stage(const SearchParams& sp, const SearchState& st, int r0, int p, int tid, int nthreads, S3BookLds& B) {
+    for (int i = tid; i < sp.beam * (p + 1); i += nthreads) {
+        const int b = i / (p + 1), q = i - b * (p + 1);
+        B.anc_s[b * WLX_T_TEXT + q] = st.anc[(long)(r0 + b) * WLX_T_TEXT + q];
+    }
+    if (tid < sp.beam) B.rule_old[tid] = *reinterpret_cast<const int4*>(st.rule + 4 * (r0 + tid));
+}
+template <int NW>
+__device__ __forceinline__ void s3_book_select(const SearchParams& sp, const SearchState& st, int item, int lane, int n_hyp0, int ngen, bool is_last,
+                                               const S3MergeLds<NW>& L, S3BookLds& B) {
+    const S3Class c = s3_classify(sp, lane, is_last, L);
+    const int k = lane;
+    int cap = WLX_MAX_HYP - n_hyp0; cap = cap < 16 ? cap : 16; cap = cap > 0 ? cap : 0;
+    if (c.fin_k && k < sp.beam && c.hidx < cap) {
+        const int len = ngen + ((c.tok == sp.eot) ? 0 : 1);
+        const int slot = n_hyp0 + c.hidx;
+        B.hyp_src[c.hidx] = c.bb;
+        B.hyp_extra[c.hidx] = (c.tok == sp.eot) ? -1 : c.tok;
+        B.hyp_slot[c.hidx] = slot;
+        st.hyp_len[item * WLX_MAX_HYP + slot] = len;
+        const float flen = (float)(len > 0 ? len : 1);
+        const float denom = (sp.length_penalty == 1.0f) ? flen : powf(flen, sp.length_penalty);
+        st.hyp_score[item * WLX_MAX_HYP + slot] = c.bs / denom;
+    }
+    if (c.act_k && c.aidx < sp.beam) { B.parent[c.aidx] = c.bb; B.newtok[c.aidx] = c.tok; B.newcum[c.aidx] = c.bs; }
+    int nh_new, n_active;
+    const bool fin = s3_finished(sp, c, n_hyp0, is_last, nh_new, n_active);
+    if (lane == 0) {
+        const int n_hyp = n_hyp0 + nh_new;
+        st.n_hyp[item] = n_hyp; st.n_hyp_host[item] = n_hyp;
+        B.hyp_n = nh_new;
+        B.n_active_s = n_active;
+        B.n_hyp_s = n_hyp;
+        B.finished_s = fin ? 1 : 0;
+    }
+}
+__device__ __forceinline__ bool s3_book_commit(const SearchParams& sp, const SearchState& st, int item, int r0, int p, int plen, int ngen,
+                                               int step_no, int tid, int nthreads, const S3BookLds& B) {
+    for (int hh = 0; hh < B.hyp_n; ++hh) {
+        const int b = B.hyp_src[hh];
+        int* dst = st.hyp_tokens + ((long)item * WLX_MAX_HYP + B.hyp_slot[hh]) * WLX_T_TEXT;
+        for (int j = tid; j < ngen; j += nthreads)
+            dst[j] = st.intok[(long)B.anc_s[b * WLX_T_TEXT + plen + j] * WLX_T_TEXT + plen + j];
+        if (tid == 0 && B.hyp_extra[hh] >= 0) dst[ngen] = B.hyp_extra[hh];
+    }
+    if (B.finished_s) {
+        __syncthreads();
+        if (tid == 0) {
+            if (step_no) step_mirror(st, step_no);
+            finish_item(st, item, sp.items);
+        }
+        return true;
+    }
+    const int na = B.n_active_s;
+    for (int i = tid; i < na * (p + 1); i += nthreads) {
+        const int j = i / (p + 1), q = i - j * (p + 1);
+        st.anc[(long)(r0 + j) * WLX_T_TEXT + q] = B.anc_s[B.parent[j] * WLX_T_TEXT + q];
+    }
+    if (tid < sp.beam) {
+        const int j = tid;
+        st.anc[(long)(r0 + j) * WLX_T_TEXT + p + 1] = (short)(r0 + j);
+        int4 ru = make_int4(0, 1, -1, 0);
+        if (j < na) {
+            const int tok = B.newtok[j];
+            const int4 po = B.rule_old[B.parent[j]];
+            const int is_ts = tok >= sp.ts_begin ? 1 : 0;
+            ru.x = is_ts;
+            ru.y = (ngen + 1 < 2) ? 1 : po.x;
+            ru.z = is_ts ? tok : po.z;
+            st.token[r0 + j] = tok; st.cum[r0 + j] = B.newcum[j];
+        } else { st.token[r0 + j] = sp.eot; st.cum[r0 + j] = WLX_NEG_INF; }
+        *reinterpret_cast<int4*>(st.rule + 4 * (r0 + j)) = ru;
+        st.pos[r0 + j] = p + 1;
+        st.nsp_row[r0 + j] = 0;
+    }
+    if (step_no) step_mirror(st, step_no);
+    return false;
+}
+
+
+#define S3_FOLD_WORDS 64
+#define S3_FOLD_DONE 0
+#define S3_FOLD_IDONE 1
+#define S3_FOLD_POS 2
+#define S3_FOLD_NHYP 3
+#define S3_FOLD_CUM 16
+#define S3_FOLD_TOK 32
+#define S3_FOLD_NW 6
+struct S3FoldLds { S3MergeLds<S3_FOLD_NW> L; S3BookLds B; };
+
+template <class F>
+__device__ __forceinline__ void s3_fold_winners(const SearchParams* __restrict__ spp, const SearchState& st, const int* __restrict__ fold_in, int V,
+                                                int R, int tid, int nw, S3MergeLds<S3_FOLD_NW>& L, int* tok_s, int* pos_s, F after_requests) {
+    const int lane = tid & 63;
+    const int wave = __builtin_amdgcn_readfirstlane(tid >> 6);
+    const int nwv = nw < S3_FOLD_NW ? nw : S3_FOLD_NW;
+    const int done_v = fold_in[S3_FOLD_DONE] | fold_in[S3_FOLD_IDONE];
+    const int p = fold_in[S3_FOLD_POS];
+    const int n_hyp0 = fold_in[S3_FOLD_NHYP];
+    const int plen = st.plen[0];
+    const int old_tok = fold_in[S3_FOLD_TOK + (lane & 15)];
+    const float* cum = reinterpret_cast<const float*>(fold_in + S3_FOLD_CUM);
+    const int rp = wave < R ? wave : R - 1;
+    const int lc = lane < SC_MAXCH ? lane : SC_MAXCH - 1;
+    S3RowFetch pf;
+    s3_merge_request(st, cum, false, rp, lc, pf);
+    const SearchParams sp = *spp;
+    after_requests();
+    bool fin = true;
+    if (!done_v) {
+        int id0_, lim_, nct, nch;
+        s3_chunk(0, sp.ts_begin, V, id0_, lim_, nct, nch);
+        if (wave < nwv) s3_merge_rows<S3_FOLD_NW>(nullptr, 0, V, sp, st, cum, 0, 0, wave, nwv, lane, lc, nct, nch, pf, false, L);
+        __syncthreads();
+        if (wave == 0) {
+            s3_merge_beams<S3_FOLD_NW>(sp, lane, L);
+            const int ngen = p + 1 - plen;
+            const bool is_last = (ngen + 1 >= sp.max_length - plen);
+            const S3Class c = s3_classify(sp, lane, is_last, L);
+            int nh_new, n_active;
+            fin = s3_finished(sp, c, n_hyp0, is_last, nh_new, n_active);
+            if (!fin) {
+                if (lane >= n_active && lane < 16) tok_s[lane] = sp.eot;
+                if (c.act_k && c.aidx < sp.beam) tok_s[c.aidx] = c.tok;
+            }
+        }
+    }
+    if (wave == 0) {
+        if (fin && lane < 16) tok_s[lane] = old_tok;
+        if (lane == 0) *pos_s = fin ? p : p + 1;
+    }
+    __syncthreads();
+}
+
+template <class Lds>
+__device__ __forceinline__ void s3_fold_bookkeep(const float* __restrict__ logits, long ldl, int V, const SearchParams* __restrict__ spp, const SearchState& st,
+                                                 int R, const int* __restrict__ fold_in, int* __restrict__ fold_out, int tid, int nthreads, Lds& F) {
+    const int item = 0, r0 = 0;
+    const int lane = tid & 63;
+    const int wave = __builtin_amdgcn_readfirstlane(tid >> 6);
+    const int nw = nthreads >> 6;
+    const int nwv = nw < S3_FOLD_NW ? nw : S3_FOLD_NW;
+    int fv = tid < S3_FOLD_WORDS ? fold_in[tid] : 0;
+    const int done_v = *st.done;
+    const int idone = st.item_done[item];
+    const int plen = st.plen[item];
+    const int p = st.pos[r0];
+    const int n_hyp0 = st.n_hyp[item];
+    const int rp = r0 + (wave < R ? wave : R - 1);
+    const int lc = lane < SC_MAXCH ? lane : SC_MAXCH - 1;
+    S3RowFetch pf;
+    s3_merge_request(st, st.cum, true, rp, lc, pf);
+    const SearchParams sp = *spp;
+    if (done_v) { if (tid < S3_FOLD_WORDS) fold_out[tid] = fv; return; }
+    int step_no = 0;
+    if (tid == 0) step_no = atomicAdd(st.step, 1) + 1;
+    if (idone) { if (tid < S3_FOLD_WORDS) fold_out[tid] = fv; if (step_no) step_mirror(st, step_no); return; }
+    int id0_, lim_, nct, nch;
+    s3_chunk(0, sp.ts_begin, V, id0_, lim_, nct, nch);
+    s3_book_stage(sp, st, r0, p, tid, nthreads, F.B);
+    if (wave < nwv) s3_merge_rows<S3_FOLD_NW>(logits, ldl, V, sp, st, st.cum, item, r0, wave, nwv, lane, lc, nct, nch, pf, true, F.L);
+    __syncthreads();
+    const int ngen = p + 1 - plen;
+    const bool is_last = (ngen + 1 >= sp.max_length - plen);
+    if (wave == 0) {
+        s3_merge_beams<S3_FOLD_NW>(sp, lane, F.L);
+        s3_book_select<S3_FOLD_NW>(sp, st, item, lane, n_hyp0, ngen, is_last, F.L, F.B);
+    }
+    __syncthreads();
+    if (tid < S3_FOLD_WORDS) {
+        if (F.B.finished_s) {
+            if (tid == S3_FOLD_DONE || tid == S3_FOLD_IDONE) fv = 1;
+        } else {
+            const int na = F.B.n_active_s;
+            if (tid == S3_FOLD_POS) fv = p + 1;
+            if (tid == S3_FOLD_NHYP) fv = F.B.n_hyp_s;
+            const int jc = tid - S3_FOLD_CUM, jt = tid - S3_FOLD_TOK;
+            if (jc >= 0 && jc < sp.beam) fv = __float_as_int(jc < na ? F.B.newcum[jc] : WLX_NEG_INF);
+            if (jt >= 0 && jt < sp.beam) fv = jt < na ? F.B.newtok[jt] : sp.eot;
+        }
+        fold_out[tid] = fv;
+    }
+    (void)s3_book_commit(sp, st, item, r0, p, plen, ngen, step_no, tid, nthreads, F.B);
+}
+
+}
```

After: 1164 xRT (audio s / wall s) (median of 6 runs). No clear change (+0.8%).
